# GlassyWing/yolo_deepsort

Hardware: AMD Instinct MI355X
Metric: end-to-end frames/sec (detect+ReID+assoc), 608x608 (higher is better)
Workload: dtype f16x3

## Files before the change

include/ydsort.h:

```cpp
#ifndef YDSORT_H
#define YDSORT_H

#include <stddef.h>
#include <stdint.h>

#ifdef __cplusplus
extern "C" {
#endif

typedef struct yds_net yds_net;
typedef struct yds_reid yds_reid;
typedef struct yds_trk yds_trk;
typedef struct yds_pipe yds_pipe;
typedef struct yds_zones yds_zones;
typedef struct yds_act yds_act;
typedef struct yds_ident yds_ident;
typedef struct yds_comm yds_comm;

int yds_init(int device_id);
int yds_current_device(void);
int yds_device_pci_bus_id(char *buf, int len);
const char *yds_last_error(void);
int yds_device_count(void);
const char *yds_build_info(void);
void *yds_host_alloc(size_t nbytes);
int yds_host_free(void *host);
void *yds_dev_alloc(size_t nbytes);
int yds_dev_free(void *dev);
int yds_memcpy_h2d(void *dst_dev, const void *src_host, size_t nbytes);
int yds_memcpy_d2h(void *dst_host, const void *src_dev, size_t nbytes);
int yds_memcpy_d2d(void *dst_dev, const void *src_dev, size_t nbytes);
int yds_device_sync(void);

yds_net *yds_darknet_create(const char *cfg_text, int img_h, int img_w, int batch_max);
void yds_darknet_destroy(yds_net *);
int yds_darknet_load_weights(yds_net *, const void *blob_host, size_t nbytes, int cutoff);
int yds_darknet_set_batch_max(yds_net *, int batch_max);
int yds_darknet_batch_max(const yds_net *);
int yds_darknet_set_half(yds_net *, int on);
int yds_darknet_layer_format(const yds_net *, int layer);
int yds_darknet_num_boxes(const yds_net *);
int yds_darknet_num_attrs(const yds_net *);
int yds_darknet_num_layers(const yds_net *);
int yds_darknet_layer_shape(const yds_net *, int layer, int *c, int *h, int *w);
int64_t yds_darknet_conv_flops(const yds_net *);
int yds_darknet_forward_f32(yds_net *, const float *nchw_host, int batch, float *out_host);
int yds_darknet_forward_u8(yds_net *, const uint8_t *rgb_hwc_host, int h, int w, int batch,
                           float *out_host_or_null);
int yds_darknet_forward_u8_dev(yds_net *, const uint8_t *rgb_hwc_dev, int h, int w, int batch);
int yds_darknet_forward_u8_mixed_dev(yds_net *, const uint8_t *rgb_hwc_dev, const uint64_t *frame_off, const int32_t *frame_hw ,
                                     size_t frames_bytes, int batch);
const uint8_t *yds_darknet_last_frames_dev(yds_net *, int *h, int *w, int *batch);
int yds_darknet_layer_output(yds_net *, int layer, int batch, float *nchw_host);
int yds_darknet_get_input(yds_net *, int batch, float *nchw_host);

int yds_nms(yds_net *, int image, float conf_thres, float iou_thres, int frame_h, int frame_w,
            float *out6_host, int cap, int *n_out);
int yds_nms_pred(const float *pred_host, int n_boxes, int attrs, float conf_thres, float iou_thres,
                 float *out6_host, int cap, int *n_out);

int yds_detect_tiled(yds_net *, const uint8_t *rgb_hwc_host, int h, int w, const int32_t *tiles_xyhw, int n_tiles,
                     float conf_thres, float iou_thres, float *out6_host, int cap, int *n_out);
int yds_nms_merge_pred(const float *pred_host, int n_boxes, int attrs, float conf_thres, float iou_thres,
                       float *out6_host, int cap, int *n_out);
int yds_nms_merge_pred_batched(const float *pred_host, int n_frames, int n_boxes, int attrs, float conf_thres, float iou_thres,
                               float *out6_host, int cap, int *n_out);
int yds_nms_ragged_pred(const float *pred_host, size_t total_rows, int attrs, int n_frames, const uint64_t *row0, const int32_t *n_rows,
                        const int32_t *corner_merge, const float *scale, float conf_thres, float iou_thres, float *out6_host, int cap,
                        int *n_out);

yds_reid *yds_reid_create(int max_crops);
void yds_reid_destroy(yds_reid *);
int yds_reid_load_tensor(yds_reid *, const char *name, const float *data_host, const int64_t *shape, int ndim);
int yds_reid_finalize(yds_reid *);
int64_t yds_reid_flops_per_crop(void);
int yds_reid_embed(yds_reid *, const uint8_t *frame_rgb_host, int h, int w, const float *tlwh_host,
                   int D, float *out_host);
int yds_reid_embed_dev(yds_reid *, const uint8_t *frame_rgb_dev, int h, int w, const float *tlwh_host,
                       int D, float *out_host_or_null);
const float *yds_reid_features_dev(yds_reid *);
int yds_reid_preprocess(yds_reid *, const uint8_t *frame_rgb_host, int h, int w, const float *tlwh_host,
                        int D, float *nchw_host);
int yds_reid_preprocess_mixed(yds_reid *, const uint8_t *frames_rgb_dev, const uint64_t *frame_off, const int32_t *frame_hw ,
                              int n_frames, size_t frames_bytes, const float *tlwh_host, const int32_t *frame_of_host, int D, float *nchw_host);
int yds_reid_embed_mixed(yds_reid *, const uint8_t *frames_dev, const uint64_t *frame_off, const int32_t *frame_hw ,
                         int n_frames, size_t frames_bytes, const float *tlwh_host, const int32_t *frame_of_host, int D, int bgr,
                         float *out_host);
int yds_reid_front_fused(yds_reid *);
int yds_reid_front_grid_crops(void);
int yds_reid_forward_f32(yds_reid *, const float *nchw_host, int D, float *out_host);

yds_trk *yds_tracker_create(double max_dist, double max_iou_distance, int max_age, int n_init, int nn_budget);
yds_trk *yds_tracker_create_ex(double max_dist, double max_iou_distance, int max_age, int n_init, int nn_budget, int metric);
void yds_tracker_destroy(yds_trk *);
int yds_tracker_step(yds_trk *, const float *tlwh_host, const float *feats_host, const float *payload_host,
                     int D, int32_t *out6_host, int cap, int *m_out,
                     int32_t *dbg_matches_host, int dbg_cap, int *n_matches);
int yds_tracker_step_dev(yds_trk *, const float *tlwh_host, const float *feats_dev, const float *payload_host,
                         int D, int32_t *out6_host, int cap, int *m_out);
int yds_tracker_step_sel(yds_trk *, const float *tlwh_host, const float *feats, int feats_on_device, const int32_t *feat_rows_host,
                         const float *payload_host, int D, int32_t *out6_host, int cap, int *m_out,
                         int32_t *dbg_matches_host, int dbg_cap, int *n_matches);
int yds_tracker_nms(const float *tlwh_host, const int32_t *order_host, int D, double max_overlap, int32_t *pick_host, int *n_pick);
int yds_tracker_num_tracks(const yds_trk *);
int yds_tracker_get_state(yds_trk *, int32_t *ids, int32_t *state, int32_t *tsu, int32_t *hits,
                          float *mean8, float *cov64, int cap, int *T);
int yds_tracker_gallery_rows(const yds_trk *);
int yds_tracker_get_payload(yds_trk *, float *payload, int cap);
int yds_tracker_get_age(yds_trk *, int32_t *age, int cap);
int yds_tracker_last_unmatched(yds_trk *, int32_t *um_tracks, int cap_t, int *n_t,
                               int32_t *um_dets, int cap_d, int *n_d);
int yds_lsap(const float *cost_host, int nr, int nc, int32_t *rows, int32_t *cols, int *n_out);
int yds_lsap_bench(const float *cost_host, int nr, int nc, int iters, double *avg_us);
int yds_kalman_predict(float *mean_host, float *cov_host, int T);
int yds_kalman_update(float *mean_host, float *cov_host, const float *xyah_host, int M);
int yds_kalman_gating(const float *mean_host, const float *cov_host, int T, const float *xyah_host, int D,
                      float *out_TxD_host);
int yds_kalman_gating_ex(const float *mean_host, const float *cov_host, int T, const float *xyah_host, int D, int only_position,
                         float *out_TxD_host);
int yds_kalman_initiate(const float *xyah_host, int n, float *mean_host, float *cov_host);
int yds_kalman_project(const float *mean_host, const float *cov_host, int n, float *mean4_host, float *cov16_host);
int yds_iou_cost(const float *track_tlwh_host, int T, const float *det_tlwh_host, int D, float *out_TxD_host);
int yds_cosine_min_cost(const float *gallery_host, const int32_t *seg_offsets_host, int T,
                        const float *feats_host, int D, int dim, float *out_TxD_host);
int yds_euclidean_min_cost(const float *gallery_host, const int32_t *seg_offsets_host, int T,
                           const float *feats_host, int D, int dim, float *out_TxD_host);

int yds_gallery_search(yds_trk *const *trks, int n_streams, const float *queries, int queries_on_device, int Q, int state_mask, float max_dist,
                       int top_k, int32_t *n_hits, int32_t *hit_stream, int32_t *hit_id, float *hit_dist);
int yds_gallery_search_dense(yds_trk *const *trks, int n_streams, const float *queries, int queries_on_device, int Q, float *dist_out,
                             int32_t *stream_of, int32_t *track_id, int32_t *state, int cap, int *n_tracks);
int yds_gallery_link(yds_trk *const *trks, int n_streams, int stream, int track_id, int exclude_stream , int state_mask,
                     float max_dist, int top_k, int32_t *n_hits, int32_t *hit_stream, int32_t *hit_id, float *hit_dist);
int yds_tracker_get_gallery(yds_trk *, int track_index, float *rows_out, int cap, int *n_rows);
int yds_tracker_get_slots(yds_trk *, int32_t *slots, int cap);

yds_pipe *yds_pipeline_create(yds_net *, yds_reid *, yds_trk *, float conf_thres, float nms_thres,
                              const int32_t *class_mask, int n_mask);
void yds_pipeline_destroy(yds_pipe *);
int yds_pipeline_step(yds_pipe *, const uint8_t *frames_dev, const uint8_t *next_frames_dev, int h, int w,
                      int batch, int32_t *out6_host, int cap, int32_t *counts_host);
int yds_pipeline_step_host(yds_pipe *, const uint8_t *frames_host, const uint8_t *next_frames_host, int h, int w,
                           int batch, int32_t *out6_host, int cap, int32_t *counts_host);
yds_pipe *yds_pipeline_create_multi(yds_net *, yds_reid *, yds_trk *const *trks, int n_streams, float conf_thres, float nms_thres,
                                    const int32_t *class_mask, int n_mask);
int yds_pipeline_step_multi(yds_pipe *, const uint8_t *frames_dev, const uint8_t *next_frames_dev, int h, int w, int n_frames,
                            const int32_t *stream_of_frame, int32_t *out6_host, int cap, int32_t *counts_host);
int yds_pipeline_step_multi_host(yds_pipe *, const uint8_t *frames_host, const uint8_t *next_frames_host, int h, int w, int n_frames,
                                 const int32_t *stream_of_frame, int32_t *out6_host, int cap, int32_t *counts_host);
int yds_pipeline_step_multi_mixed(yds_pipe *, const uint8_t *frames_dev, const uint8_t *next_frames_dev, const uint64_t *frame_off,
                                  const int32_t *frame_hw , size_t frames_bytes, int n_frames,
                                  const int32_t *stream_of_frame, int32_t *out6_host, int cap, int32_t *counts_host);
int yds_pipeline_step_multi_mixed_host(yds_pipe *, const uint8_t *frames_host, const uint8_t *next_frames_host, const uint64_t *frame_off,
                                       const int32_t *frame_hw , size_t frames_bytes, int n_frames,
                                       const int32_t *stream_of_frame, int32_t *out6_host, int cap, int32_t *counts_host);
int yds_pipeline_prefetch_host(yds_pipe *, const uint8_t *frames_host, int h, int w, int batch);
int yds_pipeline_set_schedule(yds_pipe *, int min_crops);
int yds_pipeline_set_frame_order(yds_pipe *, int bgr);
int yds_pipeline_set_windows(yds_pipe *, int win_w, int win_h, double overlap);
int yds_pipeline_set_stream_windows(yds_pipe *, int stream, int win_w, int win_h, double overlap);
int yds_pipeline_last_schedule(yds_pipe *);
int yds_pipeline_schedule_trial(yds_pipe *, int uploaded, int *decided, double *serialized_s, double *two_stream_s);
int yds_pipeline_stage_us(yds_pipe *, float *us5);
int yds_overlay_tracks(const uint8_t *frames_dev, const int32_t *src_slot_host, int n_out, int h, int w, const int32_t *boxes_host,
                       const int32_t *box_ptr_host, const uint8_t *text_host, int n_text, const int32_t *fps_host,
                       const uint8_t *font_host, int n_glyphs, int thickness, int scale, uint8_t *out_dev, uint8_t *out_host);
int yds_swap_rb(uint8_t *frames_dev, size_t pixels);
int yds_overlay_tracks_bgr(uint8_t *frames_bgr_dev, int n_src, const int32_t *src_slot_host, int n_out, int h, int w, const int32_t *boxes_host,
                           const int32_t *box_ptr_host, const uint8_t *text_host, int n_text, const int32_t *fps_host,
                           const uint8_t *font_host, int n_glyphs, int thickness, int scale, uint8_t *out_host);
int yds_conv_timing(yds_net *, int mode, double *total_us, int64_t *launches, double *flops);
int yds_conv_timing_ex(yds_net *, int mode, double *total_us, int64_t *launches, double *flops, double *bytes, double *attainable_us);
int yds_conv_num_variants(void);
int yds_set_conv_math(int mode);
int yds_get_conv_math(void);
const char *yds_conv_variant_name(int variant);
int yds_conv_bench(int n, int h, int w, int cin, int cout, int ksize, int stride, int act, int with_residual,
                   int iters, double *avg_us, int *variant);
int yds_conv_clock(double *ghz, double *sampled_ms, int reset);
int yds_conv_run(int variant, int n, int h, int w, int cin, int cout, int ksize, int stride, int act, int res_mode,
                 const float *x_nhwc, const float *w_okkc, const float *bias, const float *res_nhwc, float *y_nchw);
int yds_conv_run_view(int variant, int n, int h, int w, int cin, int cout, int ksize, int stride, int act, int res_mode,
                      const int *view, const float *x_nhwc, const float *w_okkc, const float *bias, const float *res_nhwc,
                      float sentinel, float *y_nchw, float *y2_nchw);
int yds_conv_run_half(int variant, int n, int h, int w, int cin, int cout, int ksize, int stride, int act, int res_mode,
                      const int *view, int fmt_x, int fmt_y, const float *x_nhwc, const float *w_okkc, const float *bias,
                      const float *res_nhwc, float sentinel, float *y_nchw, float *y2_nchw);
int yds_conv_run_fused(int kind, int n, int h, int w, int act, int half, int fmt, const float *x_nhwc, const float *w_a,
                       const float *bias_a, const float *w_b, const float *bias_b, float *y_nchw);

enum { YDS_ACT_TAKEOFF = 0, YDS_ACT_LANDING = 1, YDS_ACT_GLIDE = 2, YDS_ACT_FAST_CROSSING = 3, YDS_ACT_BREAK_INTO = 4 };
#define YDS_ACT_MAX_SIZE 16
#define YDS_ACT_MAX_ACTIONS 32
yds_act *yds_actions_create(int n_streams, const int32_t *kind, const int32_t *class_id, const double *param, int n_actions, int max_age,
                            int max_size);
void yds_actions_destroy(yds_act *);
int yds_actions_reset(yds_act *, int stream);
int yds_actions_update(yds_act *, const int32_t *rows6_host, const int32_t *first, const int32_t *stream_of, const double *row_time,
                       int n_frames, int32_t *out4_host, int cap, int *n_out);
int yds_actions_get_orbits(yds_act *, int stream, int32_t *ids, int32_t *ages, int32_t *lens, int cap, int *n);
int yds_actions_set_timing(yds_act *, int on);
int yds_actions_last_us(yds_act *, float *us);
int yds_pipeline_set_actions(yds_pipe *, yds_act *);
int yds_pipeline_set_frame_times(yds_pipe *, const double *t_host, int n);
int yds_pipeline_last_actions(yds_pipe *, int32_t *out4_host, int cap, int *n_out);

enum { YDS_ZONE_ENTER = 0, YDS_ZONE_EXIT = 1, YDS_ZONE_LOST = 2, YDS_ZONE_CROSS_FWD = 3, YDS_ZONE_CROSS_BACK = 4 };
#define YDS_ZONE_MAX_ZONES 32
#define YDS_ZONE_MAX_LINES 32
#define YDS_ZONE_MAX_VERTICES 16
#define YDS_ZONE_COORD_LIMIT (1 << 20)
yds_zones *yds_zones_create(int n_streams, int max_age);
void yds_zones_destroy(yds_zones *);
int yds_zones_set_stream(yds_zones *, int stream, const int32_t *zone_ptr, const int32_t *zone_xy, const int32_t *zone_class,
                         const int32_t *zone_min_sightings, int n_zones, const int32_t *line_xy, const int32_t *line_class, int n_lines);
int yds_zones_reset(yds_zones *, int stream);
int yds_zones_update(yds_zones *, const int32_t *rows6_host, const int32_t *first, const int32_t *stream_of, const double *frame_time,
                     int n_frames, int32_t *ev6_host, double *evt2_host, int cap, int *n_out);
int yds_zones_get_counts(yds_zones *, int stream, int32_t *zone4, int32_t *line2);
int yds_zones_get_tracks(yds_zones *, int stream, int32_t *ids, int32_t *ages, int32_t *inside_mask, int cap, int *n);
int yds_zones_set_timing(yds_zones *, int on);
int yds_zones_last_us(yds_zones *, float *us);
int yds_pipeline_set_zones(yds_pipe *, yds_zones *);
int yds_pipeline_last_zone_events(yds_pipe *, int32_t *ev6_host, double *evt2_host, int cap, int *n_out);

yds_ident *yds_identity_create(yds_trk *const *trks, int n_streams, float max_dist, int max_rows);
void yds_identity_destroy(yds_ident *);
int yds_identity_reset(yds_ident *);
int yds_identity_update(yds_ident *, int *n_linked, int *n_fresh, int *n_deferred);
int yds_identity_get(yds_ident *, int stream, int32_t *track_id, int32_t *global_id, int cap, int *n);
int yds_identity_last_links(yds_ident *, int32_t *stream, int32_t *track_id, int32_t *global_id, float *cost, int cap, int *n);
int yds_identity_last_counts(yds_ident *, int *n_linked, int *n_fresh, int *n_deferred);
int yds_identity_set_timing(yds_ident *, int on);
int yds_identity_last_us(yds_ident *, float *us);
int yds_identity_set_memory(yds_ident *, int max_ids, int rows_per_id, int ttl);
int yds_identity_enrol(yds_ident *, const float *rows, const int32_t *n_rows, int n_arrays, int32_t *global_id_out);
int yds_identity_get_memory(yds_ident *, int32_t *global_id, int32_t *n_rows, int32_t *last_held, int cap, int *n);
int yds_identity_get_memory_rows(yds_ident *, int global_id, float *rows_out, int cap, int *n_rows);
int yds_identity_memory_distances(yds_ident *, const float *queries, int queries_on_device, int Q, float *dist_out, int32_t *global_id_out,
                                  int cap, int *n_entries);
int yds_identity_memory_bench(yds_ident *, const float *queries_dev, int Q, int strip_len, int iters, float *us_out);
int yds_identity_last_relinked(yds_ident *, int32_t *stream, int32_t *track_id, int32_t *global_id, float *cost, int cap, int *n);
int yds_identity_last_memory_counts(yds_ident *, int32_t *counts7);
int yds_pipeline_set_identities(yds_pipe *, yds_ident *);
int yds_pipeline_last_identities(yds_pipe *, int stream, int32_t *track_id, int32_t *global_id, int cap, int *n);

#define YDS_COMM_ID_BYTES 128
#define YDS_COMM_MIN_ROWS 64
int yds_comm_preflight(void);
int yds_comm_unique_id(void *id128_out);
yds_comm *yds_comm_create(const void *id128, int world, int rank);
void yds_comm_destroy(yds_comm *);
int yds_comm_world(const yds_comm *);
int yds_comm_rank(const yds_comm *);
int yds_comm_rccl_version(void);
int yds_comm_allgather(yds_comm *, const void *send_host, size_t bytes, void *recv_host);
int yds_comm_allgather_dev(yds_comm *, const void *send_dev, size_t bytes, void *recv_dev);
int yds_comm_allgather_rows(yds_comm *, const int32_t *out6_host, int cap, const int32_t *counts_host, int batch, int rows_per_block,
                            int32_t *all_host, int *rows_needed);
int yds_comm_allreduce_f64(yds_comm *, double *vals_host, int n, int op);
int yds_comm_barrier(yds_comm *);

int yds_darknet_set_injection(yds_net *, int image, const float *rows_host, int n, float logit);
int yds_darknet_load_injection_sets(yds_net *, const float *rows_host, const int32_t *offsets_host, int n_sets, float logit);
int yds_darknet_select_injection_set(yds_net *, int set);
int yds_pipeline_set_next_injection(yds_pipe *, int set);
int yds_pipeline_slot_pred(yds_pipe *, float *pred_host, size_t cap_rows, size_t *n_rows);
int yds_gallery_search_bench(yds_trk *const *trks, int n_streams, const float *queries_dev, int Q, int state_mask, float max_dist, int top_k,
                             int iters, float *us_out);

#ifdef __cplusplus
}
#endif
#endif
```

yolo_deepsort_amd/_lib.py:

```python

from __future__ import annotations

import ctypes as C
import os

import numpy as np

HERE = os.path.dirname(os.path.abspath(__file__))
_TAG = os.environ.get("YDS_BUILD_TAG", "")
LIB_PATH = os.path.join(HERE, "libydsort" + ("_" + _TAG if _TAG else "") + ".so")


class YdsError(RuntimeError):
    pass


_P = C.c_void_p
_I = C.c_int
_F = C.c_float
_SZ = C.c_size_t
_I64 = C.c_int64

SIGNATURES = {
    "yds_init": (_I, [_I]),
    "yds_last_error": (C.c_char_p, []),
    "yds_device_count": (_I, []),
    "yds_current_device": (_I, []),
    "yds_device_pci_bus_id": (_I, [C.c_char_p, _I]),
    "yds_build_info": (C.c_char_p, []),
    "yds_host_alloc": (_P, [_SZ]),
    "yds_host_free": (_I, [_P]),
    "yds_dev_alloc": (_P, [_SZ]),
    "yds_dev_free": (_I, [_P]),
    "yds_memcpy_h2d": (_I, [_P, _P, _SZ]),
    "yds_memcpy_d2h": (_I, [_P, _P, _SZ]),
    "yds_memcpy_d2d": (_I, [_P, _P, _SZ]),
    "yds_device_sync": (_I, []),
    "yds_darknet_create": (_P, [C.c_char_p, _I, _I, _I]),
    "yds_darknet_destroy": (None, [_P]),
    "yds_darknet_load_weights": (_I, [_P, _P, _SZ, _I]),
    "yds_darknet_set_batch_max": (_I, [_P, _I]),
    "yds_darknet_batch_max": (_I, [_P]),
    "yds_darknet_set_half": (_I, [_P, _I]),
    "yds_darknet_layer_format": (_I, [_P, _I]),
    "yds_darknet_num_boxes": (_I, [_P]),
    "yds_darknet_num_attrs": (_I, [_P]),
    "yds_darknet_num_layers": (_I, [_P]),
    "yds_darknet_layer_shape": (_I, [_P, _I, _P, _P, _P]),
    "yds_darknet_conv_flops": (_I64, [_P]),
    "yds_darknet_forward_f32": (_I, [_P, _P, _I, _P]),
    "yds_darknet_forward_u8": (_I, [_P, _P, _I, _I, _I, _P]),
    "yds_darknet_forward_u8_dev": (_I, [_P, _P, _I, _I, _I]),
    "yds_darknet_last_frames_dev": (_P, [_P, _P, _P, _P]),
    "yds_darknet_layer_output": (_I, [_P, _I, _I, _P]),
    "yds_darknet_get_input": (_I, [_P, _I, _P]),
    "yds_darknet_set_injection": (_I, [_P, _I, _P, _I, _F]),
    "yds_darknet_load_injection_sets": (_I, [_P, _P, _P, _I, _F]),
    "yds_darknet_select_injection_set": (_I, [_P, _I]),
    "yds_conv_variant_name": (C.c_char_p, [_I]),
    "yds_conv_timing_ex": (_I, [_P, _I, _P, _P, _P, _P, _P]),
    "yds_conv_num_variants": (_I, []),
    "yds_conv_clock": (_I, [_P, _P, _I]),
    "yds_set_conv_math": (_I, [_I]),
    "yds_get_conv_math": (_I, []),
    "yds_conv_bench": (_I, [_I, _I, _I, _I, _I, _I, _I, _I, _I, _I, _P, _P]),
    "yds_conv_run": (_I, [_I, _I, _I, _I, _I, _I, _I, _I, _I, _I, _P, _P, _P, _P, _P]),
    "yds_conv_run_view": (_I, [_I, _I, _I, _I, _I, _I, _I, _I, _I, _I, _P, _P, _P, _P, _P, _F, _P, _P]),
    "yds_conv_run_half": (_I, [_I, _I, _I, _I, _I, _I, _I, _I, _I, _I, _P, _I, _I, _P, _P, _P, _P, _F, _P, _P]),
    "yds_conv_run_fused": (_I, [_I, _I, _I, _I, _I, _I, _I, _P, _P, _P, _P, _P, _P]),
    "yds_nms": (_I, [_P, _I, _F, _F, _I, _I, _P, _I, _P]),
    "yds_nms_pred": (_I, [_P, _I, _I, _F, _F, _P, _I, _P]),
    "yds_nms_merge_pred": (_I, [_P, _I, _I, _F, _F, _P, _I, _P]),
    "yds_nms_merge_pred_batched": (_I, [_P, _I, _I, _I, _F, _F, _P, _I, _P]),
    "yds_detect_tiled": (_I, [_P, _P, _I, _I, _P, _I, _F, _F, _P, _I, _P]),
    "yds_reid_create": (_P, [_I]),
    "yds_reid_destroy": (None, [_P]),
    "yds_reid_load_tensor": (_I, [_P, C.c_char_p, _P, _P, _I]),
    "yds_reid_finalize": (_I, [_P]),
    "yds_reid_flops_per_crop": (_I64, []),
    "yds_reid_embed": (_I, [_P, _P, _I, _I, _P, _I, _P]),
    "yds_reid_embed_dev": (_I, [_P, _P, _I, _I, _P, _I, _P]),
    "yds_reid_features_dev": (_P, [_P]),
    "yds_reid_preprocess": (_I, [_P, _P, _I, _I, _P, _I, _P]),
    "yds_reid_forward_f32": (_I, [_P, _P, _I, _P]),
    "yds_tracker_create": (_P, [C.c_double, C.c_double, _I, _I, _I]),
    "yds_tracker_create_ex": (_P, [C.c_double, C.c_double, _I, _I, _I, _I]),
    "yds_tracker_step_sel": (_I, [_P, _P, _P, _I, _P, _P, _I, _P, _I, _P, _P, _I, _P]),
    "yds_tracker_nms": (_I, [_P, _P, _I, C.c_double, _P, _P]),
    "yds_euclidean_min_cost": (_I, [_P, _P, _I, _P, _I, _I, _P]),
    "yds_tracker_destroy": (None, [_P]),
    "yds_tracker_step": (_I, [_P, _P, _P, _P, _I, _P, _I, _P, _P, _I, _P]),
    "yds_tracker_step_dev": (_I, [_P, _P, _P, _P, _I, _P, _I, _P]),
    "yds_tracker_num_tracks": (_I, [_P]),
    "yds_tracker_get_state": (_I, [_P, _P, _P, _P, _P, _P, _P, _I, _P]),
    "yds_comm_unique_id": (_I, [_P]),
    "yds_comm_create": (_P, [_P, _I, _I]),
    "yds_comm_destroy": (None, [_P]),
    "yds_comm_world": (_I, [_P]),
    "yds_comm_rank": (_I, [_P]),
    "yds_comm_rccl_version": (_I, []),
    "yds_comm_allgather": (_I, [_P, _P, _SZ, _P]),
    "yds_comm_allgather_dev": (_I, [_P, _P, _SZ, _P]),
    "yds_comm_allgather_rows": (_I, [_P, _P, _I, _P, _I, _I, _P, _P]),
    "yds_comm_preflight": (_I, []),
    "yds_comm_allreduce_f64": (_I, [_P, _P, _I, _I]),
    "yds_comm_barrier": (_I, [_P]),
    "yds_tracker_get_payload": (_I, [_P, _P, _I]),
    "yds_tracker_get_age": (_I, [_P, _P, _I]),
    "yds_tracker_gallery_rows": (_I, [_P]),
    "yds_kalman_gating_ex": (_I, [_P, _P, _I, _P, _I, _I, _P]),
    "yds_kalman_initiate": (_I, [_P, _I, _P, _P]),
    "yds_kalman_project": (_I, [_P, _P, _I, _P, _P]),
    "yds_tracker_last_unmatched": (_I, [_P, _P, _I, _P, _P, _I, _P]),
    "yds_lsap": (_I, [_P, _I, _I, _P, _P, _P]),
    "yds_lsap_bench": (_I, [_P, _I, _I, _I, _P]),
    "yds_kalman_predict": (_I, [_P, _P, _I]),
    "yds_kalman_update": (_I, [_P, _P, _P, _I]),
    "yds_kalman_gating": (_I, [_P, _P, _I, _P, _I, _P]),
    "yds_iou_cost": (_I, [_P, _I, _P, _I, _P]),
    "yds_cosine_min_cost": (_I, [_P, _P, _I, _P, _I, _I, _P]),
    "yds_pipeline_create": (_P, [_P, _P, _P, _F, _F, _P, _I]),
    "yds_pipeline_destroy": (None, [_P]),
    "yds_pipeline_step": (_I, [_P, _P, _P, _I, _I, _I, _P, _I, _P]),
    "yds_pipeline_step_host": (_I, [_P, _P, _P, _I, _I, _I, _P, _I, _P]),
    "yds_pipeline_create_multi": (_P, [_P, _P, _P, _I, _F, _F, _P, _I]),
    "yds_pipeline_step_multi": (_I, [_P, _P, _P, _I, _I, _I, _P, _P, _I, _P]),
    "yds_pipeline_step_multi_host": (_I, [_P, _P, _P, _I, _I, _I, _P, _P, _I, _P]),
    "yds_pipeline_prefetch_host": (_I, [_P, _P, _I, _I, _I]),
    "yds_pipeline_set_next_injection": (_I, [_P, _I]),
    "yds_pipeline_stage_us": (_I, [_P, _P]),
    "yds_pipeline_set_schedule": (_I, [_P, _I]),
    "yds_pipeline_last_schedule": (_I, [_P]),
    "yds_pipeline_schedule_trial": (_I, [_P, _I, _P, _P, _P]),
    "yds_conv_timing": (_I, [_P, _I, _P, _P, _P]),
    "yds_overlay_tracks": (_I, [_P, _P, _I, _I, _I, _P, _P, _P, _I, _P, _P, _I, _I, _I, _P, _P]),
    "yds_swap_rb": (_I, [_P, _SZ]),
    "yds_overlay_tracks_bgr": (_I, [_P, _I, _P, _I, _I, _I, _P, _P, _P, _I, _P, _P, _I, _I, _I, _P]),
    "yds_pipeline_set_frame_order": (_I, [_P, _I]),
    "yds_pipeline_set_windows": (_I, [_P, _I, _I, C.c_double]),
    "yds_darknet_forward_u8_mixed_dev": (_I, [_P, _P, _P, _P, _SZ, _I]),
    "yds_reid_preprocess_mixed": (_I, [_P, _P, _P, _P, _I, _SZ, _P, _P, _I, _P]),
    "yds_reid_embed_mixed": (_I, [_P, _P, _P, _P, _I, _SZ, _P, _P, _I, _I, _P]),
    "yds_reid_front_fused": (_I, [_P]),
    "yds_reid_front_grid_crops": (_I, []),
    "yds_pipeline_step_multi_mixed": (_I, [_P, _P, _P, _P, _P, _SZ, _I, _P, _P, _I, _P]),
    "yds_pipeline_step_multi_mixed_host": (_I, [_P, _P, _P, _P, _P, _SZ, _I, _P, _P, _I, _P]),
    "yds_nms_ragged_pred": (_I, [_P, _SZ, _I, _I, _P, _P, _P, _P, _F, _F, _P, _I, _P]),
    "yds_pipeline_set_stream_windows": (_I, [_P, _I, _I, _I, C.c_double]),
    "yds_pipeline_slot_pred": (_I, [_P, _P, _SZ, _P]),
    "yds_gallery_search": (_I, [_P, _I, _P, _I, _I, _I, _F, _I, _P, _P, _P, _P]),
    "yds_gallery_search_dense": (_I, [_P, _I, _P, _I, _I, _P, _P, _P, _P, _I, _P]),
    "yds_gallery_link": (_I, [_P, _I, _I, _I, _I, _I, _F, _I, _P, _P, _P, _P]),
    "yds_tracker_get_gallery": (_I, [_P, _I, _P, _I, _P]),
    "yds_tracker_get_slots": (_I, [_P, _P, _I]),
    "yds_actions_create": (_P, [_I, _P, _P, _P, _I, _I, _I]),
    "yds_actions_destroy": (None, [_P]),
    "yds_actions_reset": (_I, [_P, _I]),
    "yds_actions_update": (_I, [_P, _P, _P, _P, _P, _I, _P, _I, _P]),
    "yds_actions_get_orbits": (_I, [_P, _I, _P, _P, _P, _I, _P]),
    "yds_actions_set_timing": (_I, [_P, _I]),
    "yds_actions_last_us": (_I, [_P, _P]),
    "yds_pipeline_set_actions": (_I, [_P, _P]),
    "yds_pipeline_set_frame_times": (_I, [_P, _P, _I]),
    "yds_pipeline_last_actions": (_I, [_P, _P, _I, _P]),
    "yds_gallery_search_bench": (_I, [_P, _I, _P, _I, _I, _F, _I, _I, _P]),
    "yds_identity_create": (_P, [_P, _I, _F, _I]),
    "yds_identity_destroy": (None, [_P]),
    "yds_identity_reset": (_I, [_P]),
    "yds_identity_update": (_I, [_P, _P, _P, _P]),
    "yds_identity_get": (_I, [_P, _I, _P, _P, _I, _P]),
    "yds_identity_last_links": (_I, [_P, _P, _P, _P, _P, _I, _P]),
    "yds_identity_last_counts": (_I, [_P, _P, _P, _P]),
    "yds_identity_set_timing": (_I, [_P, _I]),
    "yds_identity_last_us": (_I, [_P, _P]),
    "yds_identity_set_memory": (_I, [_P, _I, _I, _I]),
    "yds_identity_enrol": (_I, [_P, _P, _P, _I, _P]),
    "yds_identity_get_memory": (_I, [_P, _P, _P, _P, _I, _P]),
    "yds_identity_get_memory_rows": (_I, [_P, _I, _P, _I, _P]),
    "yds_identity_memory_distances": (_I, [_P, _P, _I, _I, _P, _P, _I, _P]),
    "yds_identity_memory_bench": (_I, [_P, _P, _I, _I, _I, _P]),
    "yds_identity_last_relinked": (_I, [_P, _P, _P, _P, _P, _I, _P]),
    "yds_identity_last_memory_counts": (_I, [_P, _P]),
    "yds_pipeline_set_identities": (_I, [_P, _P]),
    "yds_pipeline_last_identities": (_I, [_P, _I, _P, _P, _I, _P]),
    "yds_zones_create": (_P, [_I, _I]),
    "yds_zones_destroy": (None, [_P]),
    "yds_zones_set_stream": (_I, [_P, _I, _P, _P, _P, _P, _I, _P, _P, _I]),
    "yds_zones_reset": (_I, [_P, _I]),
    "yds_zones_update": (_I, [_P, _P, _P, _P, _P, _I, _P, _P, _I, _P]),
    "yds_zones_get_counts": (_I, [_P, _I, _P, _P]),
    "yds_zones_get_tracks": (_I, [_P, _I, _P, _P, _P, _I, _P]),
    "yds_zones_set_timing": (_I, [_P, _I]),
    "yds_zones_last_us": (_I, [_P, _P]),
    "yds_pipeline_set_zones": (_I, [_P, _P]),
    "yds_pipeline_last_zone_events": (_I, [_P, _P, _P, _I, _P]),
}

_lib = None
MISSING = []


def load():
    global _lib
    if _lib is not None:
        return _lib
    if not os.path.exists(LIB_PATH):
        raise YdsError(f"{LIB_PATH} not found: build it with `python -m yolo_deepsort_amd.build` "
                       "(the product has no CPU fallback)")
    lib = C.CDLL(LIB_PATH)
    for name, (res, args) in SIGNATURES.items():
        try:
            fn = getattr(lib, name)
        except AttributeError:
            MISSING.append(name)
            continue
        fn.restype = res
        fn.argtypes = args
    _lib = lib
    return lib


def last_error():
    return load().yds_last_error().decode("utf-8", "replace")


def check(rc):
    if rc != 0:
        raise YdsError(last_error())


def check_ptr(p):
    if not p:
        raise YdsError(last_error())
    return p


_bound = None


VISIBILITY_MASKS = ("HIP_VISIBLE_DEVICES", "ROCR_VISIBLE_DEVICES", "CUDA_VISIBLE_DEVICES", "GPU_DEVICE_ORDINAL")


def default_device(n_visible=None):
    v = os.environ.get("YDS_DEVICE")
    if v not in (None, ""):
        return int(v)
    v = os.environ.get("LOCAL_RANK")
    if v in (None, ""):
        return 0
    masked = any(os.environ.get(k) not in (None, "") for k in VISIBILITY_MASKS)
    if masked:
        n = load().yds_device_count() if n_visible is None else n_visible
        if n == 1:
            return 0
    return int(v)


def init(device=None):
    global _bound
    if _bound is not None:
        if device is not None and int(device) != _bound:
            raise YdsError(f"this process is bound to device {_bound}; one process drives one GPU (requested {int(device)})")
        return _bound
    dev = default_device() if device is None else int(device)
    check(load().yds_init(dev))
    _bound = dev
    return dev


def current_device():
    return _bound


def pci_bus_id():
    buf = C.create_string_buffer(64)
    check(load().yds_device_pci_bus_id(buf, 64))
    return buf.value.decode()


def ptr(a):
    if a is None:
        return None
    assert a.flags["C_CONTIGUOUS"], "array must be C-contiguous"
    return a.ctypes.data_as(C.c_void_p)


def as_f32(a):
    return np.ascontiguousarray(a, dtype=np.float32)


class PinnedArray:

    def __init__(self, shape, dtype=np.uint8):
        self.shape, self.dtype = tuple(int(v) for v in shape), np.dtype(dtype)
        self.nbytes = int(np.prod(self.shape)) * self.dtype.itemsize
        self.ptr = check_ptr(load().yds_host_alloc(self.nbytes))
        buf = (C.c_uint8 * self.nbytes).from_address(self.ptr)
        self.array = np.frombuffer(buf, dtype=self.dtype).reshape(self.shape)

    @classmethod
    def from_array(cls, a):
        a = np.asarray(a)
        p = cls(a.shape, a.dtype)
        np.copyto(p.array, a)
        return p

    def free(self):
        if self.ptr:
            self.array = None
            load().yds_host_free(self.ptr)
            self.ptr = None

    def __del__(self):
        try:
            self.free()
        except Exception:
            pass


class DeviceBuffer:

    def __init__(self, nbytes):
        self.nbytes = int(nbytes)
        self.ptr = check_ptr(load().yds_dev_alloc(self.nbytes))

    @classmethod
    def from_array(cls, a):
        a = np.ascontiguousarray(a)
        buf = cls(a.nbytes)
        check(load().yds_memcpy_h2d(buf.ptr, ptr(a), a.nbytes))
        return buf

    def offset(self, nbytes):
        return C.c_void_p(self.ptr + int(nbytes))

    def free(self):
        if self.ptr:
            load().yds_dev_free(self.ptr)
            self.ptr = None

    def __del__(self):
        try:
            self.free()
        except Exception:
            pass
```

yolo_deepsort_amd/csrc/common.h:

```cpp
#pragma once
#include <hip/hip_runtime.h>
#include <stdint.h>
#include <stdio.h>
#include <string>
#include <vector>
#include <stdexcept>

#include "slot_plan.h"

namespace yds {

void set_error(const std::string &msg);
struct Error : std::runtime_error {
    explicit Error(const std::string &m) : std::runtime_error(m) {}
};
[[noreturn]] void fail(const char *fmt, ...);
int bound_device();
void bind_thread();
hipStream_t make_stream(bool latency_role);

#define YDS_HIP(expr)                                                                          \
    do {                                                                                       \
        hipError_t _e = (expr);                                                                \
        if (_e != hipSuccess)                                                                  \
            ::yds::fail("%s failed: %s (%s:%d)", #expr, hipGetErrorString(_e), __FILE__, __LINE__); \
    } while (0)

#define YDS_API_BEGIN try { ::yds::bind_thread();
#define YDS_API_END                                                                            \
    }                                                                                          \
    catch (const std::exception &e) {                                                          \
        ::yds::set_error(e.what());                                                            \
        return -1;                                                                             \
    }                                                                                          \
    return 0;
#define YDS_API_END_PTR                                                                        \
    }                                                                                          \
    catch (const std::exception &e) {                                                          \
        ::yds::set_error(e.what());                                                            \
        return nullptr;                                                                        \
    }

template <typename T> struct DevBuf {
    T *p = nullptr;
    size_t n = 0;
    DevBuf() = default;
    explicit DevBuf(size_t count) { alloc(count); }
    DevBuf(const DevBuf &) = delete;
    DevBuf &operator=(const DevBuf &) = delete;
    DevBuf(DevBuf &&o) noexcept : p(o.p), n(o.n) { o.p = nullptr; o.n = 0; }
    DevBuf &operator=(DevBuf &&o) noexcept {
        if (this != &o) { release(); p = o.p; n = o.n; o.p = nullptr; o.n = 0; }
        return *this;
    }
    ~DevBuf() { release(); }
    void alloc(size_t count) {
        release();
        if (count == 0) return;
        YDS_HIP(hipMalloc((void **)&p, count * sizeof(T)));
        n = count;
    }
    void ensure(size_t count) { if (count > n) alloc(count); }
    void release() { if (p) { (void)hipFree(p); p = nullptr; n = 0; } }
    void upload(const T *src, size_t count, hipStream_t s = nullptr) {
        ensure(count);
        if (count) YDS_HIP(hipMemcpyAsync(p, src, count * sizeof(T), hipMemcpyHostToDevice, s));
    }
};

struct View {
    float *p = nullptr;
    int n = 0, h = 0, w = 0, c = 0, ld = 0;
    int fmt = 0;
    size_t pixels() const { return (size_t)n * h * w; }
};

enum Act { ACT_LINEAR = 0, ACT_LEAKY = 1, ACT_MISH = 2, ACT_RELU = 3 };
enum ResMode { RES_NONE = 0, RES_AFTER_ACT = 1, RES_BEFORE_ACT = 2 };

struct ConvArgs {
    View x, y;
    const float *w = nullptr, *bias = nullptr;
    const void *w16 = nullptr;
    View res;
    int ksize = 1, stride = 1, pad = 0, kpad = 0;
    int act = ACT_LINEAR, res_mode = RES_NONE;
    int terms = 3;
    View y2;
    int n_split = 0;
    int tile_gn = 0;
};
enum ConvVariant {
    VAR_F32_128x128_K32, VAR_F32_128x64_K32, VAR_F32_64x64_K32, VAR_F32_128x32_K32, VAR_F32_128x128_K16, VAR_F32_128x64_K16, VAR_F32_64x128_K16,
    VAR_STAGED_128x128, VAR_STAGED_64x128, VAR_STAGED_128x64, VAR_STAGED_64x64,
    VAR_DMA_128x128_NS2, VAR_DMA_256x128_NS3, VAR_DMA_128x256_NS3, VAR_DMA_128x128_NS3, VAR_WIN_256x128, VAR_WIN_256x64, VAR_WIN_128x64,
    VAR_DMA_128x64_NS2, VAR_DMA_64x128_NS2, VAR_WIN2_128x128, VAR_SPLITK_64x128, VAR_SPLITK_128x128, VAR_DIRECT_RGB, kConvVariants
};
static_assert(VAR_STAGED_128x128 == 7 && VAR_WIN_256x128 == 15 && VAR_SPLITK_64x128 == 21 && kConvVariants == 24, "variant ids are fixed");
int launch_conv(const ConvArgs &a, hipStream_t s, int variant = -1);
constexpr int kVariantMask = 0xff, kTileGnShift = 8;
bool conv_presplit_input(const ConvArgs &a);
bool launch_conv_maxpool3s2(const ConvArgs &a, hipStream_t s);
int conv_autotune(const ConvArgs &a, hipStream_t s, float *best_us);
std::vector<int> conv_candidates(const ConvArgs &a);
enum ConvMath { MATH_F32 = 0, MATH_F16X3 = 1 };
int conv_math();
void set_conv_math(int m);
void pack_weights_f16x3(const float *w, int cout, int kpad, std::vector<uint16_t> &out);
const char *conv_variant_name(int v);
double conv_flops(const ConvArgs &a);
double conv_bytes_io(const View &v);
double conv_bytes(const ConvArgs &a);

void launch_maxpool(const View &x, const View &y, int k, int stride, int pad, bool zero_pad_br, hipStream_t s);
void launch_upsample(const View &x, const View &y, int stride, hipStream_t s);
void launch_copy(const View &x, const View &y, hipStream_t s);
void launch_add(const View &a, const View &b, const View &y, hipStream_t s);
void launch_nchw_to_nhwc(const float *src_nchw, const View &y, int c_src, hipStream_t s);
void launch_nhwc_to_nchw(const View &x, float *dst_nchw, hipStream_t s);
void nhwc_to_host(const View &x, float *dst_nchw_host, hipStream_t s);
void launch_pack_h16(const float *src_f32, const View &y, hipStream_t s);
void launch_yolo_decode(const View &head, float *out, int total_boxes, int box_off, int num_classes,
                        const float *anchors_wh , int A, int img_h, int img_w, hipStream_t s);
void launch_inject(const View &head, int image, const float *rows_dev, int n, int head_index, int num_classes,
                   float logit, hipStream_t s);
void launch_inject_batch(const View &head, int batch, const float *table_dev, const int *offsets_dev, int max_rows, int head_index,
                         int num_classes, float logit, hipStream_t s);
void launch_resize_u8(const uint8_t *frames, int n, int h, int w, const View &y, hipStream_t s, bool bgr = false);
std::vector<FrameGeom> checked_layout(const uint64_t *frame_off, const int32_t *frame_hw, int n, size_t frames_bytes);
void launch_slot_resize(const uint8_t *frames, const SlotRec *slots, int n, const View &y, hipStream_t s, bool bgr);
void launch_slot_boxes(const float *pred, int n_boxes, int attrs, const SlotRec *slots, int n, float *dst, hipStream_t s);
struct ReidFront {
    const uint8_t *frames = nullptr;
    const FrameGeom *geom = nullptr;
    const int *boxes = nullptr;
    int h = 0, w = 0, bgr = 0;
};
void launch_crop_resize(const ReidFront &f, int D, const View &y, hipStream_t s);
void launch_reid_stem(const ReidFront &f, int D, const float *w, int kpad, const float *bias, const View &pooled, hipStream_t s);
constexpr int kReidStemUnitsPerCrop = 4;
int reid_stem_grid();
void launch_avgpool_l2norm(const View &x, float *out, hipStream_t s);

}
```

yolo_deepsort_amd/csrc/conv_common.h:

```cpp
#pragma once
#include "common.h"
#include "h16.h"

#include <algorithm>
#include <stdlib.h>
#include <type_traits>

namespace yds {

typedef float f32x16 __attribute__((ext_vector_type(16)));
typedef float f32x4 __attribute__((ext_vector_type(4)));

typedef _Float16 h8 __attribute__((ext_vector_type(8)));
typedef _Float16 h4 __attribute__((ext_vector_type(4)));
constexpr float A_SCALE = 1.f / 256.f, LO_SCALE = 2048.f;
typedef __attribute__((address_space(3))) void lds_void_t;
typedef __attribute__((address_space(1))) const void glb_void_t;
template <int N> __device__ __forceinline__ void wait_vmcnt() { asm volatile("s_waitcnt vmcnt(%0)" ::"n"(N) : "memory"); }

struct ConvKernelArgs {
    const float *x, *w, *bias, *res;
    float *y;
    int H, W, Cin, ldx;
    int Ho, Wo, Cout, ldy, ldr;
    int ksize, stride, pad;
    int K, Kpad, M;
    int act, res_mode;
    int fmt_x, fmt_y, fmt_r;
    int terms;
    int ksplit = 1;
    float *y2 = nullptr;
    int ldy2 = 0, n_split = 0;
    int tiles_m, tiles_n, xm, rm, rn;
    int gn = 1;
    int gn_req = 0;
};

constexpr int KALIGN = 32;
constexpr int STAGGER = 24;

template <int ACT> __device__ __forceinline__ float apply_act(float v) {
    if (ACT == ACT_LEAKY) return v > 0.f ? v : v * 0.1f;
    if (ACT == ACT_RELU) return v > 0.f ? v : 0.f;
    if (ACT == ACT_MISH) {
        const float e = __builtin_amdgcn_exp2f(fminf(v, 20.f) * 1.44269504088896341f);
        const float n = e * (e + 2.f);
        const float m = v * (n * __builtin_amdgcn_rcpf(n + 2.f));
        return v > 20.f ? v : m;
    }
    return v;
}

__device__ __forceinline__ bool tile_of_block(const ConvKernelArgs &p, int &tm, int &tn) {
    const int b = blockIdx.x, xcd = b & 7, idx = b >> 3;
    int lm, ln;
    if (p.gn <= 1) {
        lm = idx % p.rm;
        ln = idx / p.rm;
    } else {
        const int per = p.rm * p.gn, grp = idx / per, w = idx - grp * per;
        const int g = min(p.gn, p.rn - grp * p.gn);
        lm = w / g;
        ln = grp * p.gn + (w - lm * g);
    }
    tm = (xcd % p.xm) * p.rm + lm;
    tn = (xcd / p.xm) * p.rn + ln;
    return tm < p.tiles_m && tn < p.tiles_n;
}

inline int plan_tile_map(ConvKernelArgs &k, int BM, int BN) {
    k.tiles_m = (k.M + BM - 1) / BM;
    k.tiles_n = (k.Cout + BN - 1) / BN;
    long best = -1;
    for (int xm = 1; xm <= 8; xm *= 2) {
        int xn = 8 / xm;
        int rm = (k.tiles_m + xm - 1) / xm, rn = (k.tiles_n + xn - 1) / xn;
        long waste = (long)rm * rn * 8 - (long)k.tiles_m * k.tiles_n;
        long cost = ((long)rm * BM + (long)rn * BN) * 64 + waste * (BM + BN);
        if (best < 0 || cost < best) { best = cost; k.xm = xm; k.rm = rm; k.rn = rn; }
    }
    k.gn = std::max(1, std::min(k.gn_req, k.rn));
    return 8 * k.rm * k.rn;
}

struct FlatRows {
    int m0;
    __device__ __forceinline__ int operator()(int row) const { return m0 + row; }
};
template <int BM, int BN, int WM, int WN, int ACT, int RES, int NT, class RowMap, bool ONE_PASS, class Store>
__device__ __forceinline__ void conv_epilogue_core(const ConvKernelArgs &p, Store store, float *stage, RowMap rows, int n0, int tid) {
    constexpr int ROWS = BM / WM, LD = BN + 4, C4 = BN / 4;
    constexpr int RSTEP = NT / C4;
    static_assert(NT % C4 == 0 && C4 % 2 == 0 && ROWS % RSTEP == 0, "tile width must divide the workgroup; lane pairs share a row");
    const int wave = tid >> 6, wm = wave / WN;
    const int c4 = tid % C4, rr = tid / C4;
    const int n = n0 + c4 * 4;
    const bool n_vec = n + 3 < p.Cout;
    const bool second = p.n_split > 0 && n >= p.n_split;
    float *const y_base = second ? p.y2 : p.y;
    const int y_ld = second ? p.ldy2 : p.ldy, ny = second ? n - p.n_split : n;
    float4 bias4 = make_float4(0.f, 0.f, 0.f, 0.f);
    if (n_vec) bias4 = *reinterpret_cast<const float4 *>(p.bias + n);
    else {
        if (n < p.Cout) bias4.x = p.bias[n];
        if (n + 1 < p.Cout) bias4.y = p.bias[n + 1];
        if (n + 2 < p.Cout) bias4.z = p.bias[n + 2];
    }
    constexpr int PER_PASS = ROWS / RSTEP, NRES = RES != RES_NONE ? WM * PER_PASS : 1;
    auto sweep = [&](auto yf_c, auto rf_c) {
        constexpr int YF = decltype(yf_c)::value, RF = decltype(rf_c)::value;
        constexpr bool YH = YF == FMT_H16, RH = RF == FMT_H16, YS = YF == FMT_F16, RS = RF == FMT_F16;
        float4 rraw[NRES];
        if (RES != RES_NONE) {
#pragma unroll
            for (int q = 0; q < NRES; ++q) {
                const int m = rows((q / PER_PASS) * ROWS + rr + (q % PER_PASS) * RSTEP);
                rraw[q] = make_float4(0.f, 0.f, 0.f, 0.f);
                if (m >= 0 && m < p.M && n < p.Cout) {
                    const float *rp = p.res + (size_t)m * p.ldr;
                    if (RH) {
                        const char *g = reinterpret_cast<const char *>(rp + (n & ~31)) + (n & 31) * 2;
                        const float2 hi = *reinterpret_cast<const float2 *>(g), lo = *reinterpret_cast<const float2 *>(g + 64);
                        rraw[q] = make_float4(hi.x, hi.y, lo.x, lo.y);
                    } else if (RS) {
                        const float2 h = *reinterpret_cast<const float2 *>(reinterpret_cast<const char *>(rp) + n * 2);
                        rraw[q] = make_float4(h.x, h.y, 0.f, 0.f);
                    } else if (n_vec) {
                        rraw[q] = *reinterpret_cast<const float4 *>(rp + n);
                    } else {
                        rraw[q].x = rp[n];
                        if (n + 1 < p.Cout) rraw[q].y = rp[n + 1];
                        if (n + 2 < p.Cout) rraw[q].z = rp[n + 2];
                    }
                }
            }
        }
#pragma unroll
        for (int pass = 0; pass < WM; ++pass) {
            if (ONE_PASS ? pass == 0 : wm == pass) store(stage + (ONE_PASS ? wm * ROWS * LD : 0));
            if (!ONE_PASS || pass == 0) __syncthreads();
#pragma unroll
            for (int k2 = 0; k2 < PER_PASS; ++k2) {
                const int r = rr + k2 * RSTEP;
                const int m = rows(pass * ROWS + r);
                const bool live = m >= 0 && m < p.M && n < p.Cout;
                float4 v = *reinterpret_cast<const float4 *>(stage + (ONE_PASS ? pass * ROWS * LD : 0) + r * LD + c4 * 4);
                float rs[4] = {0.f, 0.f, 0.f, 0.f};
                if (RES != RES_NONE) {
                    const float4 t = rraw[RES != RES_NONE ? pass * PER_PASS + k2 : 0];
                    if (RH) {
                        union { float2 f; h16x4 h; } uh, ul;
                        uh.f = make_float2(t.x, t.y);
                        ul.f = make_float2(t.z, t.w);
                        h16_decode4(uh.h, ul.h, rs);
                    } else if (RS) {
                        union { float2 f; h16x4 h; } uh;
                        uh.f = make_float2(t.x, t.y);
#pragma unroll
                        for (int k = 0; k < 4; ++k) rs[k] = (float)uh.h[k] * (1.f / H16_A_SCALE);
                    } else { rs[0] = t.x; rs[1] = t.y; rs[2] = t.z; rs[3] = t.w; }
                }
                float o[4] = {v.x + bias4.x, v.y + bias4.y, v.z + bias4.z, v.w + bias4.w};
#pragma unroll
                for (int k = 0; k < 4; ++k) {
                    if (RES == RES_BEFORE_ACT) o[k] += rs[k];
                    o[k] = apply_act<ACT>(o[k]);
                    if (RES == RES_AFTER_ACT) o[k] += rs[k];
                }
                float *yp = y_base + (size_t)m * y_ld;
                if (YH) {
                    h16x4 hi, lo;
                    h16_encode4(o, hi, lo);
                    const bool odd = c4 & 1;
                    union { h16x4 h; int i[2]; } send, recv;
                    send.h = odd ? hi : lo;
                    recv.i[0] = __builtin_amdgcn_update_dpp(send.i[0], send.i[0], 0xB1, 0xF, 0xF, false);
                    recv.i[1] = __builtin_amdgcn_update_dpp(send.i[1], send.i[1], 0xB1, 0xF, 0xF, false);
                    union { h16x4 h[2]; float4 f; } out;
                    out.h[0] = odd ? recv.h : hi;
                    out.h[1] = odd ? lo : recv.h;
                    const int nq = ny & ~7;
                    char *g = reinterpret_cast<char *>(yp + (nq & ~31)) + (nq & 31) * 2 + (odd ? 64 : 0);
                    if (live) *reinterpret_cast<float4 *>(g) = out.f;
                } else if (YS) {
                    union { h16x4 h; int i[2]; } mine, other;
#pragma unroll
                    for (int k = 0; k < 4; ++k) mine.h[k] = (_Float16)(o[k] * H16_A_SCALE);
                    other.i[0] = __builtin_amdgcn_update_dpp(mine.i[0], mine.i[0], 0xB1, 0xF, 0xF, false);
                    other.i[1] = __builtin_amdgcn_update_dpp(mine.i[1], mine.i[1], 0xB1, 0xF, 0xF, false);
                    union { h16x4 h[2]; float4 f; } out;
                    out.h[0] = mine.h;
                    out.h[1] = other.h;
                    if (live && !(c4 & 1)) *reinterpret_cast<float4 *>(reinterpret_cast<char *>(yp) + ny * 2) = out.f;
                } else if (live) {
                    if (n_vec) *reinterpret_cast<float4 *>(yp + ny) = make_float4(o[0], o[1], o[2], o[3]);
                    else { yp[ny] = o[0]; if (n + 1 < p.Cout) yp[ny + 1] = o[1]; if (n + 2 < p.Cout) yp[ny + 2] = o[2]; }
                }
            }
            if (!ONE_PASS && pass + 1 < WM) __syncthreads();
        }
    };
    using F32c = std::integral_constant<int, FMT_F32>;
    using H16c = std::integral_constant<int, FMT_H16>;
    using F16c = std::integral_constant<int, FMT_F16>;
    const bool yh = p.fmt_y == FMT_H16, rh = RES != RES_NONE && p.fmt_r == FMT_H16;
    if (p.fmt_y == FMT_F16) {
        sweep(F16c{}, F16c{});
    } else if (yh) {
        if (rh) sweep(H16c{}, H16c{});
        else sweep(H16c{}, F32c{});
    } else {
        if (rh) sweep(F32c{}, H16c{});
        else sweep(F32c{}, F32c{});
    }
}
constexpr size_t conv_stage_bytes(int BM, int BN) { return (size_t)BM * (BN + 4) * sizeof(float); }

template <int BM, int BN, int WM, int WN, int ACT, int RES, int TM, int TN, int NT = 256, class RowMap = FlatRows, bool ONE_PASS = false>
__device__ __forceinline__ void conv_epilogue_rows(const ConvKernelArgs &p, f32x16 (&acc)[TM][TN], float *stage, RowMap rows, int n0, int tid) {
    constexpr int LD = BN + 4;
    const int lane = tid & 63, wn = (tid >> 6) % WN;
    const int col = lane & 31, rsel = (lane >> 5) * 4;
    auto store = [&](float *st) {
#pragma unroll
        for (int i = 0; i < TM; ++i)
#pragma unroll
            for (int j = 0; j < TN; ++j)
#pragma unroll
                for (int e = 0; e < 16; ++e)
                    st[(i * 32 + rsel + (e & 3) + 8 * (e >> 2)) * LD + wn * (BN / WN) + j * 32 + col] = acc[i][j][e];
    };
    conv_epilogue_core<BM, BN, WM, WN, ACT, RES, NT, RowMap, ONE_PASS>(p, store, stage, rows, n0, tid);
}

template <int BM, int BN, int WM, int WN, int ACT, int RES, int TM, int TN, int NT = 256, class RowMap = FlatRows, bool ONE_PASS = false>
__device__ __forceinline__ void conv_epilogue16_rows(const ConvKernelArgs &p, f32x4 (&acc)[TM][TN], float *stage, RowMap rows, int n0, int tid) {
    constexpr int LD = BN + 4;
    const int lane = tid & 63, wn = (tid >> 6) % WN;
    const int col = lane & 15, rsel = (lane >> 4) * 4;
    auto store = [&](float *st) {
#pragma unroll
        for (int i = 0; i < TM; ++i)
#pragma unroll
            for (int j = 0; j < TN; ++j)
#pragma unroll
                for (int e = 0; e < 4; ++e)
                    st[(i * 16 + rsel + e) * LD + wn * (BN / WN) + j * 16 + col] = acc[i][j][e];
    };
    conv_epilogue_core<BM, BN, WM, WN, ACT, RES, NT, RowMap, ONE_PASS>(p, store, stage, rows, n0, tid);
}
template <int BM, int BN, int WM, int WN, int ACT, int RES, int TM, int TN, int NT = 256, bool ONE_PASS = false>
__device__ __forceinline__ void conv_epilogue16(const ConvKernelArgs &p, f32x4 (&acc)[TM][TN], float *stage, int m0, int n0, int tid) {
    conv_epilogue16_rows<BM, BN, WM, WN, ACT, RES, TM, TN, NT, FlatRows, ONE_PASS>(p, acc, stage, FlatRows{m0}, n0, tid);
}

template <int BM, int BN, int WM, int WN, int ACT, int RES, int TM, int TN, int NT = 256, bool ONE_PASS = false>
__device__ __forceinline__ void conv_epilogue(const ConvKernelArgs &p, f32x16 (&acc)[TM][TN], float *stage, int m0, int n0, int tid) {
    conv_epilogue_rows<BM, BN, WM, WN, ACT, RES, TM, TN, NT, FlatRows, ONE_PASS>(p, acc, stage, FlatRows{m0}, n0, tid);
}

ConvKernelArgs make_conv_args(const ConvArgs &a);
bool conv_stem2_applicable(const ConvKernelArgs &k0, const ConvKernelArgs &k1);
void launch_conv_stem2(const ConvKernelArgs &k0, const ConvKernelArgs &k1, hipStream_t s);
bool conv_block1_applicable(const ConvKernelArgs &k2, const ConvKernelArgs &k3);
void launch_conv_block1(const ConvKernelArgs &k2, const ConvKernelArgs &k3, hipStream_t s);

template <class F> void dispatch_act_res(const ConvKernelArgs &k, F f) {
    using Linear = std::integral_constant<int, ACT_LINEAR>;
    using Leaky = std::integral_constant<int, ACT_LEAKY>;
    using Mish = std::integral_constant<int, ACT_MISH>;
    using Relu = std::integral_constant<int, ACT_RELU>;
    using None = std::integral_constant<int, RES_NONE>;
    using After = std::integral_constant<int, RES_AFTER_ACT>;
    using Before = std::integral_constant<int, RES_BEFORE_ACT>;
    switch (k.act * 4 + k.res_mode) {
        case ACT_LINEAR * 4 + RES_NONE: f(Linear{}, None{}); break;
        case ACT_LEAKY * 4 + RES_NONE: f(Leaky{}, None{}); break;
        case ACT_LEAKY * 4 + RES_AFTER_ACT: f(Leaky{}, After{}); break;
        case ACT_MISH * 4 + RES_NONE: f(Mish{}, None{}); break;
        case ACT_MISH * 4 + RES_AFTER_ACT: f(Mish{}, After{}); break;
        case ACT_RELU * 4 + RES_NONE: f(Relu{}, None{}); break;
        case ACT_RELU * 4 + RES_BEFORE_ACT: f(Relu{}, Before{}); break;
        default: fail("conv: unsupported activation/residual combination (%d, %d)", k.act, k.res_mode);
    }
}

template <auto KERN, class... Args>
void launch_conv_tiles(ConvKernelArgs k, int BM, int BN, int grid_y, int threads, size_t smem, hipStream_t s, Args... args) {
    static size_t attr_set = 0;
    if (smem > attr_set) {
        YDS_HIP(hipFuncSetAttribute(reinterpret_cast<const void *>(KERN), hipFuncAttributeMaxDynamicSharedMemorySize, (int)smem));
        attr_set = smem;
    }
    dim3 grid(plan_tile_map(k, BM, BN), grid_y);
    hipLaunchKernelGGL(KERN, grid, dim3(threads), smem, s, k, args...);
    YDS_HIP(hipGetLastError());
}

bool conv_direct_applicable(const ConvKernelArgs &k);
void launch_conv_direct(const ConvKernelArgs &k, hipStream_t s);
bool conv_pool_applicable(const ConvKernelArgs &k);
void launch_conv_pool(const ConvKernelArgs &k, hipStream_t s);

void launch_conv_f16x3_staged(ConvKernelArgs k, int tile, hipStream_t s);
void launch_conv_f16x3_dma(ConvKernelArgs k, int tile, hipStream_t s);
void launch_conv_f16x3_win(ConvKernelArgs k, int tile, hipStream_t s);
void launch_conv_f16x3_splitk(ConvKernelArgs k, int tile, hipStream_t s);
bool conv_splitk_applicable(const ConvKernelArgs &k, int tile);
bool conv_splitk_preferred(const ConvKernelArgs &k);
bool conv_win2_applicable(const ConvKernelArgs &k);
void launch_conv_win2(ConvKernelArgs k, hipStream_t s);
bool conv_win_applicable(const ConvKernelArgs &k);
void launch_conv_win(ConvKernelArgs k, int shape, hipStream_t s);
void conv_win_clock(unsigned long long *cycles_ticks, bool reset);
void conv_win16_clock(unsigned long long *cycles_ticks, bool reset);
bool conv_win16_small_applicable(const ConvKernelArgs &k);
void launch_conv_win16(ConvKernelArgs k, int shape, hipStream_t s);
void conv_win2_clock(unsigned long long *cycles_ticks, bool reset);

}
```

yolo_deepsort_amd/csrc/conv_stem2.hip:

```cpp
#include "conv_common.h"

#include <algorithm>


namespace yds {

namespace {

typedef float f32x2 __attribute__((ext_vector_type(2)));

constexpr int TH = 8, TW = 16;
constexpr int BM = TH * TW, BN = 64, WM = 4, WN = 2, NW = 8, NT = NW * 64;
constexpr int PR = 2 * TH + 1, PC = 2 * TW + 1;
constexpr int EVEN_COLS = TW + 1, ODD_COLS = TW;
constexpr int ODD_BASE = PR * EVEN_COLS;
constexpr int PATCH_ROWS = PR * PC;
constexpr int RR = PR + 2, RC = PC + 2;
constexpr int W_BYTES = 9 * BN * 128, PATCH_BYTES = PATCH_ROWS * 128, RGB_BYTES = RR * RC * 16;
constexpr int SMEM = W_BYTES + PATCH_BYTES + RGB_BYTES;

struct StemRows {
    int img, oy0, ox0, Ho, Wo;
    __device__ __forceinline__ int operator()(int row) const {
        const int oy = oy0 + row / TW, ox = ox0 + row % TW;
        return oy < Ho && ox < Wo ? (img * Ho + oy) * Wo + ox : -1;
    }
};

__device__ __forceinline__ int patch_row(int ry, int rc) {
    return (rc & 1) ? ODD_BASE + ry * ODD_COLS + (rc >> 1) : ry * EVEN_COLS + (rc >> 1);
}

template <int ACT0, int ACT1, bool HALF>
__global__ __launch_bounds__(NT, 1) void conv_stem2_f16x3(ConvKernelArgs p0, ConvKernelArgs p1, int tiles_y, int tiles_x, int n_tiles) {
    fp16_saturate_on();
    extern __shared__ __attribute__((aligned(16))) char smem[];
    char *wreg = smem, *patch = smem + W_BYTES;
    float4 *rgb = reinterpret_cast<float4 *>(smem + W_BYTES + PATCH_BYTES);
    const int tid = threadIdx.x, lane = tid & 63, wave = tid >> 6, wm = wave / WN, wn = wave % WN;

    for (int i = tid; i < 9 * BN * 8; i += NT) {
        const int row = i >> 3, pos = i & 7, tap = row / BN, co = row - tap * BN;
        const int c = pos ^ ((row >> 1) & 7);
        const f32x4 v = *reinterpret_cast<const f32x4 *>(reinterpret_cast<const char *>(p1.w) + ((size_t)min(co, p1.Cout - 1) * 9 + tap) * 128 + c * 16);
        *reinterpret_cast<f32x4 *>(wreg + row * 128 + pos * 16) = v;
    }
    const int kb0 = lane >> 5;
    h8 w0h[3], w0l[3];
#pragma unroll
    for (int sb = 0; sb < 3; ++sb)
#pragma unroll
        for (int e = 0; e < 8; ++e) {
            const int t = 4 * sb + 2 * kb0 + (e >> 2), c = e & 3;
            const float x = (t < 9 && c < 3) ? p0.w[(size_t)(lane & 31) * p0.Kpad + t * 4 + c] : (t == 4 && c == 3 ? p0.bias[lane & 31] : 0.f);
            const _Float16 h = (_Float16)x;
            w0h[sb][e] = h;
            w0l[sb][e] = (_Float16)((x - (float)h) * LO_SCALE);
        }
    const int kb = lane >> 5, r = wm * 32 + (lane & 31), py = r / TW, px = r - py * TW;
    const int brow = wn * 32 + (lane & 31);

    constexpr int LOADS = (RR * RC + NT - 1) / NT;
    float4 nxt[LOADS];
    auto fetch = [&](int tl) {
        const int img = tl / (tiles_y * tiles_x), rem = tl - img * (tiles_y * tiles_x);
        const int iy0 = 2 * ((rem / tiles_x) * TH) - 2, ix0 = 2 * ((rem % tiles_x) * TW) - 2;
#pragma unroll
        for (int l = 0; l < LOADS; ++l) {
            const int i = tid + l * NT, rr = i / RC, cc = i - rr * RC;
            const int iy = iy0 + rr, ix = ix0 + cc;
            nxt[l] = make_float4(0.f, 0.f, 0.f, 0.f);
            if (i < RR * RC && tl < n_tiles && (unsigned)iy < (unsigned)p0.H && (unsigned)ix < (unsigned)p0.W) {
                nxt[l] = *reinterpret_cast<const float4 *>(p0.x + ((size_t)(img * p0.H + iy) * p0.W + ix) * p0.ldx);
                nxt[l].w = 1.f;
            }
        }
    };
    fetch(blockIdx.x);
    for (int tl = blockIdx.x; tl < n_tiles; tl += gridDim.x) {
        const int img = tl / (tiles_y * tiles_x), rem = tl - img * (tiles_y * tiles_x);
        const int oy0 = (rem / tiles_x) * TH, ox0 = (rem % tiles_x) * TW;
        const int ly0 = 2 * oy0 - 1, lx0 = 2 * ox0 - 1;
        __syncthreads();
#pragma unroll
        for (int l = 0; l < LOADS; ++l) {
            const int i = tid + l * NT;
            if (i < RR * RC) {
                const float v[4] = {nxt[l].x, nxt[l].y, nxt[l].z, nxt[l].w};
                union { h16x4 h[2]; float4 f; } sp;
                h16_encode4(v, sp.h[0], sp.h[1]);
                rgb[i] = sp.f;
            }
        }
        __syncthreads();
        fetch(tl + gridDim.x);
#pragma unroll 1
        for (int fr = wave; fr < (PATCH_ROWS + 31) / 32; fr += NW) {
            const int pix = fr * 32 + (lane & 31), pc = min(pix, PATCH_ROWS - 1);
            const int ry = pc / PC, rc = pc - ry * PC;
            f32x16 c1, c2;
#pragma unroll
            for (int e = 0; e < 16; ++e) { c1[e] = 0.f; c2[e] = 0.f; }
#pragma unroll
            for (int sb = 0; sb < 3; ++sb) {
                union { h16x4 q[2]; h8 v; } xh, xl;
#pragma unroll
                for (int u = 0; u < 2; ++u) {
                    const int t = 4 * sb + 2 * kb0 + u;
                    union { float4 f; h16x4 h[2]; } px4;
                    px4.f = make_float4(0.f, 0.f, 0.f, 0.f);
                    if (t < 9) px4.f = rgb[(ry + t / 3) * RC + rc + t % 3];
                    xh.q[u] = px4.h[0];
                    xl.q[u] = px4.h[1];
                }
                c1 = __builtin_amdgcn_mfma_f32_32x32x16_f16(w0h[sb], xh.v, c1, 0, 0, 0);
                if (!HALF) {
                    c2 = __builtin_amdgcn_mfma_f32_32x32x16_f16(w0h[sb], xl.v, c2, 0, 0, 0);
                    c2 = __builtin_amdgcn_mfma_f32_32x32x16_f16(w0l[sb], xh.v, c2, 0, 0, 0);
                }
            }
            const bool inside = (unsigned)(ly0 + ry) < (unsigned)p0.H && (unsigned)(lx0 + rc) < (unsigned)p0.W;
            const int j = patch_row(ry, rc), jsw = (j >> 1) & 7;
            if (pix < PATCH_ROWS) {
                if (inside) {
#pragma unroll
                    for (int g = 0; g < 4; ++g) {
                        float v[4];
#pragma unroll
                        for (int c = 0; c < 4; ++c) {
                            const int e = g * 4 + c;
                            const float os = HALF ? c1[e] : c1[e] + c2[e] * (1.f / LO_SCALE);
                            v[c] = ACT0 == ACT_LEAKY ? fmaxf(os, os * 0.1f) : apply_act<ACT0>(os * (1.f / A_SCALE)) * A_SCALE;
                        }
                        h16x4 hi, lo;
                        if (HALF) {
#pragma unroll
                            for (int c = 0; c < 4; ++c) hi[c] = (_Float16)v[c];
                        } else {
                            h16_encode4_scaled(v, hi, lo);
                        }
                        *reinterpret_cast<h16x4 *>(patch + j * 128 + ((g ^ jsw) << 4) + kb0 * 8) = hi;
                        if (!HALF) *reinterpret_cast<h16x4 *>(patch + j * 128 + (((4 + g) ^ jsw) << 4) + kb0 * 8) = lo;
                    }
                } else {
                    const h16x4 z = {(_Float16)0.f, (_Float16)0.f, (_Float16)0.f, (_Float16)0.f};
#pragma unroll
                    for (int g = 0; g < (HALF ? 4 : 8); ++g) *reinterpret_cast<h16x4 *>(patch + j * 128 + ((g ^ jsw) << 4) + kb0 * 8) = z;
                }
            }
        }
        __syncthreads();
        f32x16 acc1[1][1], acc2[1][1];
#pragma unroll
        for (int e = 0; e < 16; ++e) { acc1[0][0][e] = 0.f; acc2[0][0][e] = 0.f; }
#pragma unroll
        for (int t = 0; t < 9; ++t) {
            const int dy = t / 3, dx = t % 3;
            const int j = (dx & 1) ? ODD_BASE + (2 * py + dy) * ODD_COLS + px : (2 * py + dy) * EVEN_COLS + px + (dx >> 1);
            const int jsw = (j >> 1) & 7, wrow = t * BN + brow, wsw = (wrow >> 1) & 7;
            const char *ap = patch + j * 128, *bp = wreg + wrow * 128;
#pragma unroll
            for (int s = 0; s < 2; ++s) {
                const h8 ah = *reinterpret_cast<const h8 *>(ap + (((2 * s + kb) ^ jsw) << 4));
                const h8 bh = *reinterpret_cast<const h8 *>(bp + (((2 * s + kb) ^ wsw) << 4));
                acc1[0][0] = __builtin_amdgcn_mfma_f32_32x32x16_f16(ah, bh, acc1[0][0], 0, 0, 0);
                if (!HALF) {
                    const h8 al = *reinterpret_cast<const h8 *>(ap + (((4 + 2 * s + kb) ^ jsw) << 4));
                    const h8 bl = *reinterpret_cast<const h8 *>(bp + (((4 + 2 * s + kb) ^ wsw) << 4));
                    acc2[0][0] = __builtin_amdgcn_mfma_f32_32x32x16_f16(ah, bl, acc2[0][0], 0, 0, 0);
                    acc2[0][0] = __builtin_amdgcn_mfma_f32_32x32x16_f16(al, bh, acc2[0][0], 0, 0, 0);
                }
            }
        }
#pragma unroll
        for (int e = 0; e < 16; ++e) acc1[0][0][e] = (HALF ? acc1[0][0][e] : acc1[0][0][e] + acc2[0][0][e] * (1.f / LO_SCALE)) * (1.f / A_SCALE);
        __syncthreads();
        conv_epilogue_rows<BM, BN, WM, WN, ACT1, RES_NONE, 1, 1, NT, StemRows, true>(p1, acc1, reinterpret_cast<float *>(patch),
                                                                                       StemRows{img, oy0, ox0, p1.Ho, p1.Wo}, 0, tid);
    }
}

template <int ACT0, int ACT1, bool HALF> void launch_inst(const ConvKernelArgs &k0, const ConvKernelArgs &k1, hipStream_t s) {
    static_assert(BM * (BN + 4) * 4 <= PATCH_BYTES, "whole-tile epilogue staging must fit the layer-0 patch");
    const int n_img = k0.M / (k0.H * k0.W);
    const int tiles_y = (k1.Ho + TH - 1) / TH, tiles_x = (k1.Wo + TW - 1) / TW, n_tiles = n_img * tiles_y * tiles_x;
    static bool attr_set = false;
    auto kern = conv_stem2_f16x3<ACT0, ACT1, HALF>;
    if (!attr_set) {
        YDS_HIP(hipFuncSetAttribute(reinterpret_cast<const void *>(kern), hipFuncAttributeMaxDynamicSharedMemorySize, SMEM));
        attr_set = true;
    }
    hipLaunchKernelGGL(kern, dim3(std::min(n_tiles, 256)), dim3(NT), SMEM, s, k0, k1, tiles_y, tiles_x, n_tiles);
    YDS_HIP(hipGetLastError());
}

}

bool conv_stem2_applicable(const ConvKernelArgs &k0, const ConvKernelArgs &k1) {
    return k0.Cin == 4 && k0.ksize == 3 && k0.stride == 1 && k0.pad == 1 && k0.Cout == 32 && k0.res_mode == RES_NONE && k0.fmt_x == FMT_F32 &&
           k1.Cin == 32 && k1.ksize == 3 && k1.stride == 2 && k1.pad == 1 && k1.Cout == 64 && k1.res_mode == RES_NONE && k1.K == 288 &&
           k1.H == k0.Ho && k1.W == k0.Wo && k0.act == k1.act && (k0.act == ACT_LEAKY || k0.act == ACT_MISH);
}

void launch_conv_stem2(const ConvKernelArgs &k0, const ConvKernelArgs &k1, hipStream_t s) {
    if (!conv_stem2_applicable(k0, k1)) fail("conv: the fused stem takes a 3x3/s1 RGB->32 conv followed by a 3x3/s2 32->64 conv");
    const bool half = k1.terms == 1;
    if (k0.act == ACT_LEAKY) { if (half) launch_inst<ACT_LEAKY, ACT_LEAKY, true>(k0, k1, s); else launch_inst<ACT_LEAKY, ACT_LEAKY, false>(k0, k1, s); }
    else { if (half) launch_inst<ACT_MISH, ACT_MISH, true>(k0, k1, s); else launch_inst<ACT_MISH, ACT_MISH, false>(k0, k1, s); }
}

}
```

yolo_deepsort_amd/csrc/darknet.cpp:

```cpp
#include "engine.h"
#include "h16.h"
#include "conv_common.h"

#include <math.h>
#include <stdlib.h>
#include <string.h>
#include <map>
#include <sstream>

namespace yds {

std::vector<CfgBlock> parse_cfg(const std::string &text) {
    std::vector<CfgBlock> blocks;
    std::istringstream in(text);
    std::string line;
    auto strip = [](std::string s) {
        size_t a = s.find_first_not_of(" \t\r\n"), b = s.find_last_not_of(" \t\r\n");
        return a == std::string::npos ? std::string() : s.substr(a, b - a + 1);
    };
    while (std::getline(in, line)) {
        if (line.empty() || line[0] == '#') continue;
        line = strip(line);
        if (line.empty()) fail("cfg: whitespace-only line (the reference parser rejects it too)");
        if (line[0] == '[') {
// ... 178 lines not shown
                storage[r].into = i;
                storage[r].coff = off;
            } else {
                l.copies.push_back({j, off});
            }
            off += s.c;
        }
        if (l.groups) fail("cfg: grouped multi-source routes are not supported");
    }
    math = conv_math();
    std::vector<char> h16_ok(L, math == MATH_F16X3 ? 1 : 0);
    for (int j = 0; j < L; ++j) {
        if (layers[j].type == L_YOLO) continue;
        int off = 0, o = owner_of(j, off);
        if (off % 32 || layers[j].c % 32) h16_ok[o] = 0;
    }
    for (int pass = 0; pass < 2; ++pass)
        for (int i = 0; i < L; ++i)
            for (auto &cp : layers[i].copies) {
                int off = 0, o = owner_of(cp.first, off);
                if (o >= 0 && h16_ok[o] != h16_ok[i]) h16_ok[o] = h16_ok[i] = 0;
            }
    for (int i = 0; i < L; ++i) {
        Layer &l = layers[i];
        bool owns = (is_producer(i) && !storage[i].redirected) || l.concat();
        if (!owns) continue;
        if (storage[i].ld == 0) storage[i].ld = (l.c + 3) / 4 * 4;
        storage[i].fmt = (h16_ok[i] && storage[i].ld % 32 == 0) ? FMT_H16 : FMT_F32;
        storage[i].owns = true;
    }
    const bool no_merge = getenv("YDS_NO_CSP_MERGE") != nullptr;
    for (int i = 1; i + 2 < L && !no_merge; ++i) {
        Layer &a = layers[i];
        const Layer &r = layers[i + 1];
        Layer &b = layers[i + 2];
        if (a.type != L_CONV || b.type != L_CONV || r.type != L_ROUTE || r.refs.size() != 1 || r.groups) continue;
        if (a.src < 0 || r.refs[0] != a.src || b.src != i + 1) continue;
        if (a.cw.ksize != 1 || b.cw.ksize != 1 || a.cw.stride != 1 || b.cw.stride != 1 || a.act != b.act || a.fused_res >= 0 || b.fused_res >= 0) continue;
        if (a.merged_into >= 0 || a.merge_next >= 0 || a.cw.cin != b.cw.cin) continue;
        if ((int)i == block1_at || (int)i + 2 == block1_at || i + 2 == (int)block1_at + 1) continue;
        int oa = 0, ob = 0;
        const int sa = owner_of(i, oa), sb = owner_of(i + 2, ob);
        if (storage[sa].fmt != storage[sb].fmt || a.c % 4 || b.c % 4) continue;
        if (storage[sa].fmt == FMT_H16 && (a.c % 32 || b.c % 32)) continue;
        a.merge_next = i + 2;
        b.merged_into = i;
    }
    plan_half_formats();
    allocate_buffers();
}

int Darknet::owner_of(int j, int &off) const {
    const Layer &l = layers[j];
    if (l.concat()) { off = 0; return j; }
    int r = l.root;
    if (storage[r].redirected) { off = storage[r].coff + l.coff; return storage[r].into; }
    off = l.coff;
    return r;
}

void Darknet::plan_half_formats() {
    const int L = (int)layers.size();
    for (Storage &st : storage) st.fmt_half = st.fmt;
    const bool off = getenv("YDS_HALF_H16") != nullptr;
    if (!half_mode || off || math != MATH_F16X3) return;
    std::vector<char> ok(L, 0);
    for (int i = 0; i < L; ++i) ok[i] = storage[i].owns && storage[i].fmt == FMT_H16 && storage[i].ld % 64 == 0;
    auto own = [&](int j) { int off = 0; return owner_of(j, off); };
    for (int j = 0; j < L; ++j) {
        if (layers[j].type == L_YOLO) continue;
        int off = 0, o = owner_of(j, off);
        if (o >= 0 && (off % 64 || layers[j].c % 64)) ok[o] = 0;
    }
    if (block1_at >= 0) ok[own(block1_at)] = 0;
    for (int pass = 0; pass < L; ++pass) {
        bool changed = false;
        auto tie = [&](int a, int b) {
            if (a >= 0 && b >= 0 && ok[a] != ok[b]) { ok[a] = ok[b] = 0; changed = true; }
        };
        for (int i = 0; i < L; ++i) {
            const Layer &l = layers[i];
            for (auto &cp : l.copies) tie(own(cp.first), i);
            if (l.type == L_CONV && l.fused_res >= 0) tie(own(i), own(l.fused_res));
            if (l.type == L_CONV && l.merge_next >= 0) tie(own(i), own(l.merge_next));
            if (l.type == L_UPSAMPLE) tie(own(i), own(l.src));
            if (i == block1_at && l.src >= 0) tie(own(l.src), own(i + 1));
        }
        if (!changed) break;
    }
    for (int i = 0; i < L; ++i)
        if (ok[i]) storage[i].fmt_half = FMT_F16;
}

void Darknet::set_half(bool on) {
    if (on == half_mode) return;
    YDS_HIP(hipStreamSynchronize(stream));
    half_mode = on;
    plan_half_formats();
    ++plan_epoch;
}

void Darknet::allocate_buffers() {
    for (size_t i = 0; i < layers.size(); ++i) {
        if (!storage[i].owns) continue;
        const Layer &l = layers[i];
        size_t n = (size_t)batch_max * l.h * l.w * storage[i].ld;
        storage[i].buf.alloc(n);
        YDS_HIP(hipMemsetAsync(storage[i].buf.p, 0, n * sizeof(float), stream));
    }
    input.alloc((size_t)batch_max * img_h * img_w * 4);
    out.alloc((size_t)batch_max * total_boxes * attrs);
    stage_f32.alloc((size_t)batch_max * img_h * img_w * 4);
    YDS_HIP(hipStreamSynchronize(stream));
    inject_rows.clear();
    inject_rows.resize(batch_max);
    inject_n.assign(batch_max, 0);
    inject_active = false;
    inject_offsets.clear();
    inject_set = -1;
    ++plan_epoch;
    stage_n = 0;
}

void Darknet::set_batch_max(int b) {
    if (b < 1) fail("set_batch_max: %d", b);
    if (b == batch_max) return;
    YDS_HIP(hipStreamSynchronize(stream));
    batch_max = b;
    allocate_buffers();
}

Darknet::~Darknet() {
    for (const ConvTimeRec &r : conv_pending) { (void)hipEventDestroy(r.e0); (void)hipEventDestroy(r.e1); }
    for (hipEvent_t e : ev_pool) (void)hipEventDestroy(e);
    if (stream) (void)hipStreamDestroy(stream);
}

View Darknet::view(int i, int batch, int first) const {
    const Layer &l = layers[i];
    int r = l.root;
    View v;
    v.n = batch; v.h = l.h; v.w = l.w; v.c = l.c;
    if (l.concat()) {
        v.fmt = half_mode ? storage[i].fmt_half : storage[i].fmt;
        v.p = storage[i].buf.p; v.ld = fmt_slots(v.fmt, storage[i].ld);
        v.p += (size_t)first * l.h * l.w * v.ld;
        return v;
    }
    const Storage &st = storage[r];
    if (st.redirected) {
        const Storage &dst = storage[st.into];
        v.fmt = half_mode ? dst.fmt_half : dst.fmt;
        v.p = dst.buf.p + fmt_slots(v.fmt, st.coff + l.coff);
        v.ld = fmt_slots(v.fmt, dst.ld);
    } else {
        v.fmt = half_mode ? st.fmt_half : st.fmt;
        v.p = st.buf.p + fmt_slots(v.fmt, l.coff);
        v.ld = fmt_slots(v.fmt, st.ld);
    }
    v.p += (size_t)first * l.h * l.w * v.ld;
    return v;
}

View Darknet::input_view(int batch, int first) const {
    View v;
    v.p = input.p + (size_t)first * img_h * img_w * 4; v.n = batch; v.h = img_h; v.w = img_w; v.c = 4; v.ld = 4;
    return v;
}

void Darknet::load_weights(const void *blob, size_t nbytes, int cutoff) {
    if (nbytes < 20) fail("weights: blob shorter than the 20-byte header");
    const float *w = reinterpret_cast<const float *>(static_cast<const char *>(blob) + 20);
    size_t avail = (nbytes - 20) / 4, ptr = 0;
    ++plan_epoch;
    for (Layer &l : layers) l.cw_merged.release();
    for (int i = 0; i < (int)layers.size(); ++i) {
        Layer &l = layers[i];
        if (l.type != L_CONV) continue;
        if (cutoff >= 0 && i >= cutoff) { l.cw.release(); continue; }
        const int co = l.c;
        const size_t nw = (size_t)co * l.cw.cin_file * l.cw.ksize * l.cw.ksize, need = (size_t)(l.bn ? 4 : 1) * co + nw;
        if (ptr + need > avail) fail("weights: file too short at layer %d (need %zu more floats, have %zu)", i, need, avail - ptr);
        std::vector<double> scale(co, 1.0);
        std::vector<float> bias(co);
        if (l.bn) {
            const float *beta = w + ptr, *gamma = beta + co, *mean = gamma + co, *var = mean + co;
            for (int o = 0; o < co; ++o) {
                scale[o] = (double)gamma[o] / sqrt((double)var[o] + 1e-5);
                bias[o] = (float)((double)beta[o] - (double)mean[o] * scale[o]);
            }
        } else {
            for (int o = 0; o < co; ++o) bias[o] = w[ptr + o];
        }
        ptr += (size_t)(l.bn ? 4 : 1) * co;
        l.cw.upload(w + ptr, scale.data(), bias.data(), stream);
        ptr += nw;
    }
    for (Layer &a : layers) {
        if (a.merge_next < 0) continue;
        const Layer &b = layers[a.merge_next];
        if (a.cw.loaded() && b.cw.loaded()) a.cw_merged = ConvWeights::concat(a.cw, b.cw, stream);
    }
}

ConvArgs Darknet::conv_args(int i, int batch, int first, bool merged) const {
    const Layer &l = layers[i];
    ConvArgs a;
    a.x = l.src < 0 ? input_view(batch, first) : view(l.src, batch, first);
    a.y = view(i, batch, first);
    l.cw.fill(a);
    a.act = l.act;
    if (l.fused_res >= 0) { a.res = view(l.fused_res, batch, first); a.res_mode = RES_AFTER_ACT; }
    a.terms = half_mode ? 1 : 3;
    if (merged) {
        a.y2 = view(l.merge_next, batch, first);
        a.n_split = a.y.c;
        a.y.c = a.y.c + a.y2.c;
        l.cw_merged.fill(a);
    }
    return a;
}

const LaunchPlan &Darknet::plan(int batch) {
    LaunchPlan &p = plan_;
    if (p.batch == batch && p.math == conv_math() && p.epoch == plan_epoch) return p;
    p.batch = batch; p.math = conv_math(); p.epoch = plan_epoch;
    p.steps.clear();
    p.produced_by.assign(layers.size(), -1);
    static const bool no_stem = getenv("YDS_NO_STEM_FUSE") != nullptr, no_block = getenv("YDS_NO_BLOCK_FUSE") != nullptr;
    const bool f16x3 = p.math == MATH_F16X3;
    auto has_w = [&](int i) { return layers[i].cw.loaded(); };
    auto kargs = [&](int i) { return make_conv_args(conv_args(i, batch)); };
    const bool stem = !no_stem && stem_fusable && f16x3 && has_w(0) && has_w(1) && view(1, batch).fmt != FMT_F32 &&
                      conv_stem2_applicable(kargs(0), kargs(1));
    const bool block1 = !no_block && block1_at >= 0 && f16x3 && has_w(block1_at) && has_w(block1_at + 1) &&
                        conv_block1_applicable(kargs(block1_at), kargs(block1_at + 1));
    int heads = 0;
    auto add = [&](Step::Kind kind, int layer) -> Step & {
        p.produced_by[layer] = (int)p.steps.size();
        p.steps.push_back(Step{kind, layer});
        return p.steps.back();
    };
    for (int i = 0; i < (int)layers.size(); ++i) {
        const Layer &l = layers[i];
        switch (l.type) {
        case L_CONV:
            if (l.merged_into >= 0 && layers[l.merged_into].cw_merged.loaded()) p.produced_by[i] = p.produced_by[l.merged_into];
            else if ((i == 0 && stem) || (i == block1_at && block1)) break;
            else if (i == 1 && stem) add(Step::CONV_STEM2, i);
            else if (i == block1_at + 1 && block1) add(Step::CONV_BLOCK1, i);
            else add(l.cw_merged.loaded() ? Step::CONV_MERGED : Step::CONV, i);
            break;
        case L_MAXPOOL: {
            Step &st = add(Step::MAXPOOL, i);
            st.src = l.src; st.ksize = l.ksize; st.stride = l.stride; st.pad = l.pad; st.zero_br = l.zero_br;
            if (l.stride != 1 || l.zero_br || l.ksize < 9 || l.pad != (l.ksize - 1) / 2) break;
            for (int j = i - 1; j >= 0; --j) {
                const Layer &q = layers[j];
                if (q.type == L_MAXPOOL && q.stride == 1 && !q.zero_br && q.ksize == l.ksize - 4 && q.pad == (q.ksize - 1) / 2 && q.c == l.c &&
                    layers[q.src].root == layers[l.src].root && layers[q.src].coff == layers[l.src].coff) {
                    st.src = j; st.ksize = 5; st.pad = 2;
                    break;
                }
            }
            break;
        }
        case L_UPSAMPLE: add(Step::UPSAMPLE, i); break;
        case L_ROUTE:
            for (auto &cp : l.copies) {
                Step &st = add(Step::COPY, i);
                st.src = cp.first; st.arg = cp.second;
            }
            break;
        case L_SHORTCUT:
            if (!l.fused) add(Step::ADD, i);
            break;
        case L_YOLO: add(Step::YOLO, i).arg = heads++; break;
        }
    }
    return p;
}

void Darknet::autotune(int batch) {
    const int mode = conv_math() + (half_mode ? 10 : 0);
    auto tune = [&](int i, bool merged) {
        Layer &l = layers[i];
        if (!l.cw.loaded() || (l.tuned_batch == batch && l.tuned_math == mode)) return;
        l.variant = conv_autotune(conv_args(i, batch, 0, merged), stream, nullptr);
        l.tuned_batch = batch;
        l.tuned_math = mode;
    };
    for (const Step &st : plan(batch).steps) {
        if (st.kind > Step::CONV_BLOCK1) continue;
        if (st.kind == Step::CONV_STEM2 || st.kind == Step::CONV_BLOCK1) tune(st.layer - 1, false);
        tune(st.layer, st.kind == Step::CONV_MERGED);
    }
}

void Darknet::check_pass(int batch) const {
    if (batch < 1 || batch > batch_max) fail("forward: batch %d outside [1,%d]", batch, batch_max);
    if (math != conv_math()) fail("forward: this network was planned for conv math %d, current mode is %d (re-create it)", math, conv_math());
}

void Darknet::run_graph(int batch) {
    check_pass(batch);
    int lanes = getenv("YDS_DET_LANES") ? atoi(getenv("YDS_DET_LANES")) : 1;
    while (lanes > 1 && batch / lanes < 4) --lanes;
    if (lanes < 1) lanes = 1;
    if (lanes == 1) { run_lane(0, batch, stream); return; }
    while ((int)lane_streams.size() < lanes - 1) {
        hipStream_t st; hipEvent_t ev;
        YDS_HIP(hipStreamCreateWithFlags(&st, hipStreamNonBlocking));
        YDS_HIP(hipEventCreateWithFlags(&ev, hipEventDisableTiming));
        lane_streams.push_back(st); lane_done.push_back(ev);
    }
    if (!lane_fork) YDS_HIP(hipEventCreateWithFlags(&lane_fork, hipEventDisableTiming));
    const int per = (batch + lanes - 1) / lanes;
    YDS_HIP(hipEventRecord(lane_fork, stream));
    for (int k = 0; k < lanes; ++k) {
        const int first = k * per, cnt = std::min(per, batch - first);
        if (cnt <= 0) break;
        hipStream_t st = (k == 0 || time_convs) ? stream : lane_streams[k - 1];
        if (st != stream) YDS_HIP(hipStreamWaitEvent(st, lane_fork, 0));
        run_lane(first, cnt, st);
        if (st != stream) {
            YDS_HIP(hipEventRecord(lane_done[k - 1], st));
            YDS_HIP(hipStreamWaitEvent(stream, lane_done[k - 1], 0));
        }
    }
}

int Darknet::head_layers() const {
    double total = 0, acc = 0;
    for (int i = 0; i < (int)layers.size(); ++i)
        if (layers[i].type == L_CONV) total += conv_flops(conv_args(i, 1));
    for (int i = 0; i < (int)layers.size(); ++i) {
        if (layers[i].type != L_CONV) continue;
        acc += conv_flops(conv_args(i, 1));
        if (acc >= 0.06 * total) return i + 1;
    }
    return (int)layers.size();
}

bool Darknet::forward_resized_part(int batch, int part) {
    check_pass(batch);
    if (getenv("YDS_DET_LANES") && atoi(getenv("YDS_DET_LANES")) > 1) return false;
    const int cut = head_layers();
    if (part == 0) run_lane(0, batch, stream, 0, cut);
    else run_lane(0, batch, stream, cut, -1);
    return true;
}

void Darknet::enqueue_conv(const Step &st, int first, int batch, hipStream_t stream) {
    const int i = st.layer;
    const Layer &l = layers[i];
    if (!l.cw.loaded()) fail("forward: layer %d has no weights (call load_darknet_weights)", i);
    const ConvArgs a = conv_args(i, batch, first, st.kind == Step::CONV_MERGED);
    ConvTimeRec rec;
    if (time_convs) { rec.e0 = timing_event(); rec.e1 = timing_event(); YDS_HIP(hipEventRecord(rec.e0, stream)); }
    int variant;
    double extra_flops = 0, extra_bytes = 0;
    if (st.kind == Step::CONV_STEM2) {
        const ConvArgs a0 = conv_args(i - 1, batch, first);
        ConvKernelArgs k0 = make_conv_args(a0), k1 = make_conv_args(a);
        k1.w = reinterpret_cast<const float *>(a.w16);
        launch_conv_stem2(k0, k1, stream);
        variant = VAR_DIRECT_RGB;
        extra_flops = conv_flops(a0);
        extra_bytes = conv_bytes(a0) - conv_bytes_io(a0.y) - conv_bytes_io(a.x);
    } else if (st.kind == Step::CONV_BLOCK1) {
        const ConvArgs a2 = conv_args(i - 1, batch, first);
        ConvKernelArgs k2 = make_conv_args(a2), k3 = make_conv_args(a);
        k2.w = reinterpret_cast<const float *>(a2.w16);
        k3.w = reinterpret_cast<const float *>(a.w16);
        launch_conv_block1(k2, k3, stream);
        variant = VAR_WIN_256x128;
        extra_flops = conv_flops(a2);
        extra_bytes = conv_bytes(a2) - conv_bytes_io(a2.y) - conv_bytes_io(a.x) - (a.res.p ? conv_bytes_io(a.res) : 0.0);
    } else {
        variant = launch_conv(a, stream, l.variant);
    }
    if (time_convs) {
        YDS_HIP(hipEventRecord(rec.e1, stream));
        rec.variant = variant;
        rec.flops = conv_flops(a) + extra_flops;
        rec.bytes = conv_bytes(a) + extra_bytes;
        const double peak = conv_math() == MATH_F32 ? 157.3e12 : (a.terms == 1 ? 2500e12 : 2500e12 / 3);
        rec.attain_us = std::max(rec.flops / peak, rec.bytes / 6.29e12) * 1e6;
        conv_pending.push_back(rec);
    }
}

void Darknet::run_lane(int first, int batch, hipStream_t stream, int l0, int l1) {
    autotune(batch);
    if (l1 < 0) l1 = (int)layers.size();
    auto v = [&](int layer) { return view(layer, batch, first); };
    for (const Step &st : plan(batch).steps) {
        const int i = st.layer;
        if (i < l0) continue;
        if (i >= l1) break;
        const Layer &l = layers[i];
        switch (st.kind) {
        case Step::CONV: case Step::CONV_MERGED: case Step::CONV_STEM2: case Step::CONV_BLOCK1:
            enqueue_conv(st, first, batch, stream);
            break;
        case Step::MAXPOOL: launch_maxpool(v(st.src), v(i), st.ksize, st.stride, st.pad, st.zero_br, stream); break;
        case Step::UPSAMPLE: launch_upsample(v(l.src), v(i), l.stride, stream); break;
        case Step::COPY: {
            View d = v(i);
            d.p += fmt_slots(d.fmt, st.arg);
            launch_copy(v(st.src), d, stream);
            break;
        }
        case Step::ADD: launch_add(v(l.refs[0]), v(l.refs[1]), v(i), stream); break;
        case Step::YOLO: {
            const View head = v(l.src);
            const int hidx = st.arg;
            if (inject_active && inject_set >= 0) {
                launch_inject_batch(head, batch, inject_table.p, inject_offsets_dev.p + (size_t)inject_set * batch_max + first, inject_max_rows, hidx,
                                    l.classes, inject_logit, stream);
            } else {
                for (int b = 0; b < batch && inject_active; ++b)
                    launch_inject(head, b, inject_rows[first + b].p, inject_n[first + b], hidx, l.classes, inject_logit, stream);
            }
            launch_yolo_decode(head, out.p + (size_t)first * total_boxes * attrs, total_boxes, l.box_off, l.classes, l.anchors.data(), (int)l.anchors.size() / 2, img_h, img_w, stream);
            break;
        }
        }
    }
}

void Darknet::forward_f32_host(const float *nchw, int batch, float *out_host) {
    size_t n = (size_t)batch * in_channels * img_h * img_w;
    YDS_HIP(hipMemcpyAsync(stage_f32.p, nchw, n * sizeof(float), hipMemcpyHostToDevice, stream));
    launch_nchw_to_nhwc(stage_f32.p, input_view(batch), in_channels, stream);
    run_graph(batch);
    if (out_host) YDS_HIP(hipMemcpyAsync(out_host, out.p, (size_t)batch * total_boxes * attrs * sizeof(float), hipMemcpyDeviceToHost, stream));
    YDS_HIP(hipStreamSynchronize(stream));
}

void Darknet::forward_u8_dev(const uint8_t *frames_dev, int h, int w, int batch) {
    if (in_channels != 3) fail("forward_u8: network expects %d channels", in_channels);
    check_pass(batch);
    launch_resize_u8(frames_dev, batch, h, w, input_view(batch), stream);
    run_graph(batch);
}

void Darknet::forward_u8_frames_dev(const uint8_t *frames_dev, const std::vector<FrameGeom> &geom) {
    const int batch = (int)geom.size();
    if (in_channels != 3) fail("forward_u8: network expects %d channels", in_channels);
    check_pass(batch);
    std::vector<SlotRec> slots;
    for (const FrameGeom &g : geom) slots.push_back(plain_slot(g.off, g.h, g.w));
    slot_tab.upload(slots.data(), slots.size(), stream);
    YDS_HIP(hipStreamSynchronize(stream));
    launch_slot_resize(frames_dev, slot_tab.p, batch, input_view(batch), stream, false);
    run_graph(batch);
}

void Darknet::forward_u8_host(const uint8_t *frames, int h, int w, int batch, float *out_host) {
    size_t n = (size_t)batch * h * w * 3;
    stage_u8.ensure(n);
    YDS_HIP(hipMemcpyAsync(stage_u8.p, frames, n, hipMemcpyHostToDevice, stream));
    stage_h = h; stage_w = w; stage_n = batch;
    forward_u8_dev(stage_u8.p, h, w, batch);
    if (out_host) YDS_HIP(hipMemcpyAsync(out_host, out.p, (size_t)batch * total_boxes * attrs * sizeof(float), hipMemcpyDeviceToHost, stream));
    YDS_HIP(hipStreamSynchronize(stream));
}

void Darknet::forward_slots(const uint8_t *frames_dev, const SlotRec *slots, int n_slots, float *pred, bool bgr) {
    for (int slot0 = 0; slot0 < n_slots; slot0 += batch_max) {
        const int nb = std::min(batch_max, n_slots - slot0);
        launch_slot_resize(frames_dev, slots + slot0, nb, input_view(nb), stream, bgr);
        run_graph(nb);
        launch_slot_boxes(out.p, total_boxes, attrs, slots + slot0, nb, pred + (size_t)slot0 * total_boxes * attrs, stream);
    }
}

void Darknet::forward_tiles_host(const uint8_t *frame, int h, int w, const int *tiles_xyhw, int n_tiles) {
    if (in_channels != 3) fail("forward_tiles: network expects %d channels", in_channels);
    if (n_tiles < 1) fail("forward_tiles: no windows");
    for (int t = 0; t < n_tiles; ++t) {
        const int x = tiles_xyhw[t * 4], y = tiles_xyhw[t * 4 + 1], th = tiles_xyhw[t * 4 + 2], tw = tiles_xyhw[t * 4 + 3];
        if (x < 0 || y < 0 || th < 1 || tw < 1 || x + tw > w || y + th > h) fail("forward_tiles: window %d (%d,%d,%d,%d) outside the %dx%d frame", t, x, y, th, tw, w, h);
    }
    const size_t nbytes = (size_t)h * w * 3;
    stage_u8.ensure(nbytes);
    tiled_pred.ensure((size_t)n_tiles * total_boxes * attrs);
    YDS_HIP(hipMemcpyAsync(stage_u8.p, frame, nbytes, hipMemcpyHostToDevice, stream));
    stage_h = h; stage_w = w; stage_n = 1;
    std::vector<SlotRec> slots;
    for (int t = 0; t < n_tiles; ++t)
        slots.push_back(window_slot(0, w, tiles_xyhw[t * 4], tiles_xyhw[t * 4 + 1], tiles_xyhw[t * 4 + 2], tiles_xyhw[t * 4 + 3], img_h, img_w));
    slot_tab.upload(slots.data(), slots.size(), stream);
    forward_slots(stage_u8.p, slot_tab.p, n_tiles, tiled_pred.p, false);
    YDS_HIP(hipStreamSynchronize(stream));
}

void Darknet::layer_output_host(int i, int batch, float *nchw) {
    if (i < 0 || i >= (int)layers.size()) fail("layer_output: no layer %d", i);
    const Layer &l = layers[i];
    if (l.type == L_CONV && l.cw.loaded() && plan(batch).produced_by[i] < 0) (void)launch_conv(conv_args(i, batch), stream, l.variant);
    if (l.type == L_YOLO) fail("layer_output: yolo layers are read through the forward output");
    if (l.fused_res >= 0) fail("layer_output: layer %d is fused with the following shortcut", i);
    nhwc_to_host(view(i, batch), nchw, stream);
}

void Darknet::get_input_host(int batch, float *nchw) {
    View v = input_view(batch);
    v.c = in_channels;
    nhwc_to_host(v, nchw, stream);
}

void Darknet::set_injection(int image, const float *rows, int n, float logit) {
    if (image < 0 || image >= batch_max) fail("inject: image %d outside batch", image);
    inject_n[image] = n;
    if (n > 0) inject_rows[image].upload(rows, (size_t)n * 9, stream);
    YDS_HIP(hipStreamSynchronize(stream));
    inject_logit = logit;
    inject_active = false;
    for (int b = 0; b < batch_max; ++b) inject_active |= inject_n[b] > 0;
}

void Darknet::load_injection_sets(const float *rows, const int *offsets, int n_sets, float logit) {
    if (n_sets <= 0) { inject_set = -1; inject_active = false; inject_offsets.clear(); return; }
    inject_offsets.assign(offsets, offsets + (size_t)n_sets * batch_max + 1);
    inject_table.ensure((size_t)inject_offsets.back() * 9 + 9);
    inject_table.upload(rows, (size_t)inject_offsets.back() * 9, stream);
    inject_offsets_dev.ensure(inject_offsets.size());
    inject_offsets_dev.upload(inject_offsets.data(), inject_offsets.size(), stream);
    inject_max_rows = 0;
    for (size_t i = 0; i + 1 < inject_offsets.size(); ++i) inject_max_rows = std::max(inject_max_rows, inject_offsets[i + 1] - inject_offsets[i]);
    YDS_HIP(hipStreamSynchronize(stream));
    inject_logit = logit;
    inject_set = 0;
    inject_active = true;
}

void Darknet::select_injection_set(int set) {
    if (inject_offsets.empty()) fail("inject: no sets loaded");
    int n_sets = (int)(inject_offsets.size() - 1) / batch_max;
    if (set < 0 || set >= n_sets) fail("inject: set %d outside [0,%d)", set, n_sets);
    inject_set = set;
}

int64_t Darknet::flops_per_image() const {
    int64_t f = 0;
    for (const Layer &l : layers)
        if (l.type == L_CONV) f += 2ll * l.h * l.w * l.c * l.cw.ksize * l.cw.ksize * l.cw.cin_file;
    return f;
}

void Darknet::enable_conv_timing(bool on) {
    if (!on) resolve_conv_timing();
    time_convs = on;
}

hipEvent_t Darknet::timing_event() {
    if (!ev_pool.empty()) { hipEvent_t e = ev_pool.back(); ev_pool.pop_back(); return e; }
    hipEvent_t e;
    YDS_HIP(hipEventCreate(&e));
    return e;
}

void Darknet::resolve_conv_timing() {
    if (conv_pending.empty()) return;
    YDS_HIP(hipStreamSynchronize(stream));
    for (const ConvTimeRec &r : conv_pending) {
        float ms = 0;
        YDS_HIP(hipEventElapsedTime(&ms, r.e0, r.e1));
        conv_us[r.variant] += ms * 1e3;
        conv_launches[r.variant]++;
        conv_flops_acc[r.variant] += r.flops;
        conv_bytes_acc[r.variant] += r.bytes;
        conv_attain_us[r.variant] += r.attain_us;
        ev_pool.push_back(r.e0);
        ev_pool.push_back(r.e1);
    }
    conv_pending.clear();
}

}

using yds::Darknet;

extern "C" {

yds_net *yds_darknet_create(const char *cfg_text, int img_h, int img_w, int batch_max) {
    YDS_API_BEGIN
    if (!cfg_text) yds::fail("cfg_text is NULL");
    if (img_h <= 0 || img_w <= 0 || batch_max <= 0) yds::fail("bad geometry %dx%d batch %d", img_h, img_w, batch_max);
    auto *n = new yds_net{new Darknet(cfg_text, img_h, img_w, batch_max)};
    return n;
    YDS_API_END_PTR
}
void yds_darknet_destroy(yds_net *n) {
    if (n) { delete n->d; delete n; }
}
int yds_darknet_load_weights(yds_net *n, const void *blob, size_t nbytes, int cutoff) {
    YDS_API_BEGIN
    n->d->load_weights(blob, nbytes, cutoff);
    YDS_API_END
}
int yds_darknet_set_batch_max(yds_net *n, int batch_max) {
    YDS_API_BEGIN
    n->d->set_batch_max(batch_max);
    YDS_API_END
}
int yds_darknet_batch_max(const yds_net *n) { return n->d->batch_max; }
int yds_darknet_set_half(yds_net *n, int on) {
    YDS_API_BEGIN
    if (on && n->d->math != yds::MATH_F16X3) yds::fail("half mode needs the split-fp16 tensor formats (conv math f16x3)");
    n->d->set_half(on != 0);
    YDS_API_END
}
int yds_darknet_layer_format(const yds_net *n, int layer) {
    if (!n || layer < 0 || layer >= (int)n->d->layers.size() || n->d->layers[layer].type == yds::L_YOLO) return -1;
    return n->d->view(layer, 1).fmt;
}
int yds_darknet_num_boxes(const yds_net *n) { return n->d->total_boxes; }
int yds_darknet_num_attrs(const yds_net *n) { return n->d->attrs; }
int yds_darknet_num_layers(const yds_net *n) { return (int)n->d->layers.size(); }
int yds_darknet_layer_shape(const yds_net *n, int layer, int *c, int *h, int *w) {
    YDS_API_BEGIN
    if (layer < 0 || layer >= (int)n->d->layers.size()) yds::fail("no layer %d", layer);
    const auto &l = n->d->layers[layer];
    *c = l.c; *h = l.h; *w = l.w;
    YDS_API_END
}
int64_t yds_darknet_conv_flops(const yds_net *n) { return n->d->flops_per_image(); }
int yds_darknet_forward_f32(yds_net *n, const float *nchw_host, int batch, float *out_host) {
    YDS_API_BEGIN
    n->d->forward_f32_host(nchw_host, batch, out_host);
    YDS_API_END
}
int yds_darknet_forward_u8(yds_net *n, const uint8_t *rgb, int h, int w, int batch, float *out_host) {
    YDS_API_BEGIN
    n->d->forward_u8_host(rgb, h, w, batch, out_host);
    YDS_API_END
}
const uint8_t *yds_darknet_last_frames_dev(yds_net *n, int *h, int *w, int *batch) {
    if (!n || !n->d->stage_n) return nullptr;
    *h = n->d->stage_h; *w = n->d->stage_w; *batch = n->d->stage_n;
    return n->d->stage_u8.p;
}
int yds_darknet_forward_u8_dev(yds_net *n, const uint8_t *rgb_dev, int h, int w, int batch) {
    YDS_API_BEGIN
    n->d->forward_u8_dev(rgb_dev, h, w, batch);
    YDS_API_END
}
int yds_darknet_forward_u8_mixed_dev(yds_net *n, const uint8_t *rgb_dev, const uint64_t *frame_off, const int32_t *frame_hw, size_t frames_bytes,
                                     int batch) {
    YDS_API_BEGIN
    if (!rgb_dev) yds::fail("forward_u8: NULL frames");
    n->d->forward_u8_frames_dev(rgb_dev, yds::checked_layout(frame_off, frame_hw, batch, frames_bytes));
    YDS_API_END
}
int yds_darknet_layer_output(yds_net *n, int layer, int batch, float *nchw_host) {
    YDS_API_BEGIN
    n->d->layer_output_host(layer, batch, nchw_host);
    YDS_API_END
}
int yds_darknet_get_input(yds_net *n, int batch, float *nchw_host) {
    YDS_API_BEGIN
    n->d->get_input_host(batch, nchw_host);
    YDS_API_END
}
int yds_darknet_set_injection(yds_net *n, int image, const float *rows, int cnt, float logit) {
    YDS_API_BEGIN
    n->d->set_injection(image, rows, cnt, logit);
    YDS_API_END
}
int yds_conv_timing_ex(yds_net *n, int mode, double *total_us, int64_t *launches, double *flops, double *bytes, double *attainable_us) {
    YDS_API_BEGIN
    Darknet *d = n->d;
    if (mode == 2) d->enable_conv_timing(false);
    else d->resolve_conv_timing();
    for (int v = 0; v < yds::kConvVariants; ++v) {
        if (total_us) total_us[v] = d->conv_us[v];
        if (launches) launches[v] = d->conv_launches[v];
        if (flops) flops[v] = d->conv_flops_acc[v];
        if (bytes) bytes[v] = d->conv_bytes_acc[v];
        if (attainable_us) attainable_us[v] = d->conv_attain_us[v];
    }
    if (mode == 1) {
        for (int v = 0; v < yds::kConvVariants; ++v) {
            d->conv_us[v] = 0; d->conv_launches[v] = 0; d->conv_flops_acc[v] = 0; d->conv_bytes_acc[v] = 0; d->conv_attain_us[v] = 0;
        }
        d->enable_conv_timing(true);
    }
    YDS_API_END
}
int yds_conv_timing(yds_net *n, int mode, double *total_us4, int64_t *launches4, double *flops4) {
    return yds_conv_timing_ex(n, mode, total_us4, launches4, flops4, nullptr, nullptr);
}
const char *yds_conv_variant_name(int v) { return yds::conv_variant_name(v); }
int yds_conv_num_variants(void) { return yds::kConvVariants; }
int yds_set_conv_math(int mode) { yds::set_conv_math(mode); return 0; }
int yds_get_conv_math(void) { return yds::conv_math(); }
int yds_conv_clock(double *ghz, double *sampled_ms, int reset) {
    YDS_API_BEGIN
    double g = 0, ms = 0;
#ifdef YDS_CLOCK_PROBE
    YDS_HIP(hipDeviceSynchronize());
    unsigned long long a[2], b[2], c[2];
    yds::conv_win_clock(a, reset != 0);
    yds::conv_win2_clock(b, reset != 0);
    yds::conv_win16_clock(c, reset != 0);
    const double cycles = (double)a[0] + (double)b[0] + (double)c[0], ticks = (double)a[1] + (double)b[1] + (double)c[1];
    g = ticks > 0 ? cycles / ticks * 0.1 : 0.0;
    ms = ticks * 1e-5;
#else
    (void)reset;
#endif
    if (ghz) *ghz = g;
    if (sampled_ms) *sampled_ms = ms;
    YDS_API_END
}
int yds_darknet_load_injection_sets(yds_net *n, const float *rows_host, const int32_t *offsets_host, int n_sets, float logit) {
    YDS_API_BEGIN
    n->d->load_injection_sets(rows_host, offsets_host, n_sets, logit);
    YDS_API_END
}
int yds_darknet_select_injection_set(yds_net *n, int set) {
    YDS_API_BEGIN
    n->d->select_injection_set(set);
    YDS_API_END
}

}
```

yolo_deepsort_amd/csrc/engine.h:

```cpp
#pragma once
#include "common.h"
#include "conv_weights.h"

#include <map>
#include <memory>
#include <string>
#include <utility>
#include <vector>

namespace yds {

struct CfgBlock {
    std::string type;
    std::map<std::string, std::string> kv;
};
std::vector<CfgBlock> parse_cfg(const std::string &text);

enum LayerType { L_CONV, L_MAXPOOL, L_UPSAMPLE, L_ROUTE, L_SHORTCUT, L_YOLO };

struct Layer {
    LayerType type = L_CONV;
    int c = 0, h = 0, w = 0;
    int root = -1, coff = 0;
    int src = -1;
    std::vector<int> refs;
    std::vector<std::pair<int, int>> copies;
    bool concat() const { return type == L_ROUTE && refs.size() > 1; }
    int bn = 0, act = ACT_LINEAR;
    ConvWeights cw;
    int fused_res = -1;
    int variant = -1, tuned_batch = 0, tuned_math = -1;
    int merge_next = -1, merged_into = -1;
    ConvWeights cw_merged;
    int ksize = 1, stride = 1, pad = 0;
    bool fused = false, zero_br = false;
    int groups = 0, group_id = 0;
    std::vector<float> anchors;
    int classes = 0, box_off = 0;
};

struct Step {
    enum Kind { CONV, CONV_MERGED, CONV_STEM2, CONV_BLOCK1, MAXPOOL, UPSAMPLE, COPY, ADD, YOLO };
    Kind kind;
    int layer;
    int src = -1;
    int arg = 0;
    int ksize = 1, stride = 1, pad = 0;
    bool zero_br = false;
};
struct LaunchPlan {
    std::vector<Step> steps;
    std::vector<int> produced_by;
    int batch = -1, math = -1, epoch = -1;
};

struct Storage {
    DevBuf<float> buf;
    int ld = 0;
    int fmt = 0;
    int fmt_half = 0;
    bool owns = false;
    bool redirected = false;
    int into = -1, coff = 0;
};

class Darknet {
public:
    Darknet(const std::string &cfg_text, int img_h, int img_w, int batch_max);
    ~Darknet();
    void load_weights(const void *blob, size_t nbytes, int cutoff);
    void set_batch_max(int b);
    void forward_f32_host(const float *nchw, int batch, float *out_host);
    void forward_u8_host(const uint8_t *frames, int h, int w, int batch, float *out_host);
    void forward_u8_dev(const uint8_t *frames_dev, int h, int w, int batch);
    void forward_u8_frames_dev(const uint8_t *frames_dev, const std::vector<FrameGeom> &geom);
    void forward_resized(int batch) { run_graph(batch); }
    bool forward_resized_part(int batch, int part);
    int head_layers() const;
    void forward_tiles_host(const uint8_t *frame, int h, int w, const int *tiles_xyhw, int n_tiles);
    void forward_slots(const uint8_t *frames_dev, const SlotRec *slots, int n_slots, float *pred, bool bgr);
    void layer_output_host(int layer, int batch, float *nchw);
    void get_input_host(int batch, float *nchw);
    void set_injection(int image, const float *rows, int n, float logit);
    void load_injection_sets(const float *rows, const int *offsets, int n_sets, float logit);
    void select_injection_set(int set);
    void enable_conv_timing(bool on);
    void autotune(int batch);
    int64_t flops_per_image() const;
    View view(int layer, int batch, int first = 0) const;
    View input_view(int batch, int first = 0) const;
    ConvArgs conv_args(int layer, int batch, int first = 0, bool merged = false) const;

    int img_h, img_w, batch_max, in_channels = 3;
    int math = 0;
    bool half_mode = false;
    void set_half(bool on);
    void plan_half_formats();
    int owner_of(int layer, int &off) const;
    int total_boxes = 0, attrs = 0;
    std::vector<Layer> layers;
    std::vector<Storage> storage;
    std::vector<int> yolo_layers;
    DevBuf<float> input, out, stage_f32;
    DevBuf<uint8_t> stage_u8;
    DevBuf<SlotRec> slot_tab;
    int stage_h = 0, stage_w = 0, stage_n = 0;
    DevBuf<float> tiled_pred;
    hipStream_t stream = nullptr;
    std::vector<DevBuf<float>> inject_rows;
    std::vector<int> inject_n;
    bool inject_active = false;
    DevBuf<float> inject_table;
    std::vector<int> inject_offsets;
    DevBuf<int> inject_offsets_dev;
    int inject_max_rows = 0;
    int inject_set = -1;
    float inject_logit = 6.f;
    struct ConvTimeRec { hipEvent_t e0 = nullptr, e1 = nullptr; int variant = 0; double flops = 0, bytes = 0, attain_us = 0; };
    bool time_convs = false;
    std::vector<ConvTimeRec> conv_pending;
    std::vector<hipEvent_t> ev_pool;
    hipEvent_t timing_event();
    void resolve_conv_timing();
    double conv_us[kConvVariants] = {}, conv_flops_acc[kConvVariants] = {}, conv_bytes_acc[kConvVariants] = {}, conv_attain_us[kConvVariants] = {};
    int64_t conv_launches[kConvVariants] = {};

private:
    void allocate_buffers();
    void check_pass(int batch) const;
    void run_graph(int batch);
    void run_lane(int first, int batch, hipStream_t st, int l0 = 0, int l1 = -1);
    void enqueue_conv(const Step &st, int first, int batch, hipStream_t s);
    const LaunchPlan &plan(int batch);
    LaunchPlan plan_;
    int plan_epoch = 0;
    bool stem_fusable = false;
    int block1_at = -1;
    std::vector<hipStream_t> lane_streams;
    std::vector<hipEvent_t> lane_done;
    hipEvent_t lane_fork = nullptr;
};

struct NmsUniform { int32_t n_boxes, corner, merge; float sx, sy; };
class NmsWorkspace {
public:
    explicit NmsWorkspace(int max_candidates = 16384, int frames = 1);
    ~NmsWorkspace();
    NmsWorkspace(const NmsWorkspace &) = delete;
    void launch(const float *pred_dev, const NmsUniform &u, int n_frames, int attrs, float conf_thres, float iou_thres, int cap, hipStream_t s);
    void launch(const float *pred_dev, const NmsFrame *fr, int n_frames, int max_rows, size_t total_rows, int attrs, float conf_thres,
                float iou_thres, int cap, hipStream_t s);
    int collect(int frame, float *out6_host, int cap);
    void resize(int max_candidates, int n_frames);
    int needed(int n_frames) const;
    static constexpr int kMaxCandidates = 1 << 18;
    int run(const float *pred_dev, int n_boxes, int attrs, float conf_thres, float iou_thres, float sx, float sy,
            float *out6_host, int cap, hipStream_t s);
    int run_merge(const float *pred_dev, int n_boxes, int attrs, float conf_thres, float iou_thres, float *out6_host, int cap, hipStream_t s);
    int max_cand, frames;
    DevBuf<float> cand;
    DevBuf<float> sorted;
    DevBuf<int> counts;
    DevBuf<int> box_count;
    DevBuf<unsigned long long> mask;
    DevBuf<float> kept;
    int *h_counts = nullptr;
    float *h_kept = nullptr;
};

class ReidNet {
public:
    explicit ReidNet(int max_crops);
    ~ReidNet();
    void load_tensor(const std::string &name, const float *data, const int64_t *shape, int ndim);
    void finalize();
    void embed_dev(const uint8_t *frame_dev, int h, int w, const float *tlwh_host, int D, float *out_host);
    void embed_multi_dev(const uint8_t *frames_dev, int h, int w, const float *tlwh_host, const int *frame_of, int D, bool bgr = false,
                         const FrameGeom *geom = nullptr, int n_geom = 0);
    void preprocess_frames_dev(const uint8_t *frames_dev, const std::vector<FrameGeom> &geom, const float *tlwh_host, const int *frame_of, int D,
                               float *nchw_host);
    void embed_host(const uint8_t *frame_host, int h, int w, const float *tlwh_host, int D, float *out_host);
    void preprocess_host(const uint8_t *frame_host, int h, int w, const float *tlwh_host, int D, float *nchw_host);
    void forward_f32_host(const float *nchw, int D, float *out_host);
    void forward(int D, const ReidFront *front = nullptr);
    void reserve(int D);
    float *in_buf();
    void crop_into_in(const ReidFront &f, int D);
    ReidFront stage_crops(const uint8_t *frames_dev, int h, int w, const float *tlwh_host, const int *frame_of, int D, bool bgr,
                          const FrameGeom *geom, int n_geom);
    void allocate_buffers();
    static int64_t flops_per_crop();

    int max_crops;
    std::map<std::string, std::vector<float>> raw;
    std::map<std::string, std::vector<int64_t>> raw_shape;
    bool ready = false;
    std::vector<ConvWeights> convs;
    std::vector<DevBuf<float>> bufs;
    DevBuf<float> in, feat, stage_f32;
    DevBuf<uint8_t> stage_u8;
    DevBuf<int> boxes_dev;
    std::vector<int> boxes_host;
    int *boxes_pin[2] = {nullptr, nullptr};
    size_t boxes_pin_cap[2] = {0, 0};
    int boxes_pin_turn = 0;
    hipStream_t sync_before_regrow = nullptr;
    std::map<int, std::pair<int, int>> tuned;
    int tuned_math = -1;
    hipStream_t stream = nullptr;
    double conv_flops_last = 0;
    bool front_fused_last = false;
};

struct ActFrame {
    const int32_t *rows6;
    const int32_t *n_rows_p;
    int n_rows, stream, tag;
    double t;
    const double *row_time;
};
struct ActionsIface {
    virtual ~ActionsIface() {}
    virtual int streams() const = 0;
    virtual void enqueue(const ActFrame *fr, int n, hipStream_t s) = 0;
    virtual void collect() = 0;
    std::vector<int32_t> rows4, first;
};

struct ZonesIface {
    virtual ~ZonesIface() {}
    virtual int streams() const = 0;
    virtual void enqueue(const ActFrame *fr, int n, hipStream_t s) = 0;
    virtual void collect() = 0;
    std::vector<int32_t> ev6, first;
    std::vector<double> evt2;
};

struct GalleryView {
    const float *gallery;
    const int *slot, *id, *state, *n_feat;
    int budget, n_tracks, metric;
    double max_dist;
    const int *n_tracks_dev;
    int capacity, unbounded;
    const int *hits;
};
struct TrackerIface {
    virtual ~TrackerIface() {}
    virtual GalleryView gallery_view() const = 0;
    virtual int step(const float *tlwh_host, const float *feats, bool feats_on_device, const float *payload_host, int D,
                     int32_t *out6_host, int cap) = 0;
    virtual int num_tracks() const = 0;
};
struct IdentityIface {
    virtual ~IdentityIface() {}
    virtual bool bound_to(TrackerIface *const *trk, int S) const = 0;
    virtual void enqueue_collect(hipStream_t s) = 0;
    virtual void finish(hipStream_t s) = 0;
    virtual void get(int stream, int32_t *track_id, int32_t *global_id, int cap, int *n) const = 0;
    std::shared_ptr<void *> user;
    bool (*user_busy)(void *) = nullptr;
};

struct TrackerGroupIface {
    virtual ~TrackerGroupIface() {}
    virtual void set_identities(IdentityIface *ident) = 0;
    virtual void set_actions(ActionsIface *act, const double *frame_times) = 0;
    virtual void set_zones(ZonesIface *zones, const double *frame_times) = 0;
    virtual void step_batch(TrackerIface *const *trk, int S, int n, const int *stream_of, const float *tlwh_host, const int *first,
                            const float *feats_dev, const float *payload_host, const char *skip, int32_t *out6_host, int cap, int32_t *counts) = 0;
    virtual void wait_for(hipEvent_t ev) = 0;
};
TrackerGroupIface *make_tracker_group();

}

struct yds_net { yds::Darknet *d; };
struct yds_reid { yds::ReidNet *r; };
struct yds_trk { yds::TrackerIface *t; };
struct yds_act { yds::ActionsIface *a; };
struct yds_ident { yds::IdentityIface *i; };
struct yds_zones { yds::ZonesIface *z; };
```

yolo_deepsort_amd/csrc/layers.hip:

```cpp
#include "common.h"

#include <algorithm>
#include "h16.h"
#include "resize_dev.h"

namespace yds {

static inline int grid_for(size_t work, int block = 256) {
    size_t g = (work + block - 1) / block;
    if (g > 8192) g = 8192;
    if (g < 1) g = 1;
    return (int)g;
}

__global__ void maxpool_kernel(const float *x, float *y, int N, int H, int W, int C, int ldx, int Ho, int Wo, int ldy,
                               int k, int stride, int pad, int zero_br, int fmt_in, int fmt_out) {
    fp16_saturate_on();
    const int C4 = C >> 2;
    const size_t total = (size_t)N * Ho * Wo * C4;
    for (size_t idx = blockIdx.x * (size_t)blockDim.x + threadIdx.x; idx < total; idx += (size_t)gridDim.x * blockDim.x) {
        int c4 = idx % C4;
        size_t pix = idx / C4;
        int ox = pix % Wo;
        size_t t = pix / Wo;
        int oy = t % Ho;
        int n = t / Ho;
        float4 m = make_float4(-INFINITY, -INFINITY, -INFINITY, -INFINITY);
        for (int dy = 0; dy < k; ++dy) {
            int iy = oy * stride - pad + dy;
            for (int dx = 0; dx < k; ++dx) {
                int ix = ox * stride - pad + dx;
                float v[4] = {0.f, 0.f, 0.f, 0.f};
                if ((unsigned)iy < (unsigned)H && (unsigned)ix < (unsigned)W)
                    load4(x + ((size_t)(n * H + iy) * W + ix) * ldx, c4 * 4, fmt_in, v);
                else if (!zero_br)
                    continue;
                m.x = fmaxf(m.x, v[0]); m.y = fmaxf(m.y, v[1]); m.z = fmaxf(m.z, v[2]); m.w = fmaxf(m.w, v[3]);
            }
        }
        const float o[4] = {m.x, m.y, m.z, m.w};
        store4(y + pix * ldy, c4 * 4, fmt_out, o);
    }
}

void launch_maxpool(const View &x, const View &y, int k, int stride, int pad, bool zero_pad_br, hipStream_t s) {
    if (x.c % 4 || x.ld % 4 || y.ld % 4) fail("maxpool: channels must be a multiple of 4");
    size_t total = y.pixels() * (x.c / 4);
    hipLaunchKernelGGL(maxpool_kernel, dim3(grid_for(total)), dim3(256), 0, s, x.p, y.p, x.n, x.h, x.w, x.c, x.ld, y.h, y.w,
                       y.ld, k, stride, pad, zero_pad_br ? 1 : 0, x.fmt, y.fmt);
    YDS_HIP(hipGetLastError());
}

__global__ void upsample_kernel(const float *x, float *y, int N, int H, int W, int C, int ldx, int ldy, int s) {
    const int C4 = C >> 2, Ho = H * s, Wo = W * s;
    const size_t total = (size_t)N * Ho * Wo * C4;
    for (size_t idx = blockIdx.x * (size_t)blockDim.x + threadIdx.x; idx < total; idx += (size_t)gridDim.x * blockDim.x) {
        int c4 = idx % C4;
        size_t pix = idx / C4;
        int ox = pix % Wo;
        size_t t = pix / Wo;
        int oy = t % Ho;
        int n = t / Ho;
        *reinterpret_cast<float4 *>(y + pix * ldy + c4 * 4) =
            *reinterpret_cast<const float4 *>(x + ((size_t)(n * H + oy / s) * W + ox / s) * ldx + c4 * 4);
    }
}

void launch_upsample(const View &x, const View &y, int stride, hipStream_t s) {
    if (x.c % 4 || x.ld % 4 || y.ld % 4) fail("upsample: channels must be a multiple of 4");
    if (x.fmt != y.fmt) fail("upsample: source and destination formats differ");
    const int slots = fmt_slots(x.fmt, x.c);
    if (slots % 4) fail("upsample: channels must fill whole 16-byte pieces");
    size_t total = y.pixels() * (slots / 4);
    hipLaunchKernelGGL(upsample_kernel, dim3(grid_for(total)), dim3(256), 0, s, x.p, y.p, x.n, x.h, x.w, slots, x.ld, y.ld, stride);
    YDS_HIP(hipGetLastError());
}

__global__ void copy_kernel(const float *x, float *y, size_t pixels, int C, int ldx, int ldy) {
    const int C4 = C >> 2;
    const size_t total = pixels * C4;
    for (size_t idx = blockIdx.x * (size_t)blockDim.x + threadIdx.x; idx < total; idx += (size_t)gridDim.x * blockDim.x) {
        int c4 = idx % C4;
        size_t pix = idx / C4;
        *reinterpret_cast<float4 *>(y + pix * ldy + c4 * 4) = *reinterpret_cast<const float4 *>(x + pix * ldx + c4 * 4);
    }
}
__global__ void copy_scalar_kernel(const float *x, float *y, size_t pixels, int C, int ldx, int ldy) {
    const size_t total = pixels * C;
    for (size_t idx = blockIdx.x * (size_t)blockDim.x + threadIdx.x; idx < total; idx += (size_t)gridDim.x * blockDim.x) {
        int c = idx % C;
        size_t pix = idx / C;
        y[pix * ldy + c] = x[pix * ldx + c];
    }
}

void launch_copy(const View &x, const View &y, hipStream_t s) {
    if (x.fmt != y.fmt) fail("copy: source and destination formats differ");
    const int slots = fmt_slots(x.fmt, x.c);
    bool vec = !(slots % 4 || x.ld % 4 || y.ld % 4 || ((uintptr_t)x.p & 15) || ((uintptr_t)y.p & 15));
    if (vec)
        hipLaunchKernelGGL(copy_kernel, dim3(grid_for(x.pixels() * (slots / 4))), dim3(256), 0, s, x.p, y.p, x.pixels(), slots, x.ld, y.ld);
    else
        hipLaunchKernelGGL(copy_scalar_kernel, dim3(grid_for(x.pixels() * slots)), dim3(256), 0, s, x.p, y.p, x.pixels(), slots, x.ld, y.ld);
    YDS_HIP(hipGetLastError());
}

__global__ void add_kernel(const float *a, const float *b, float *y, size_t pixels, int C, int lda, int ldb, int ldy, int fa, int fb, int fy) {
    fp16_saturate_on();
    const int C4 = C >> 2;
    const size_t total = pixels * C4;
    for (size_t idx = blockIdx.x * (size_t)blockDim.x + threadIdx.x; idx < total; idx += (size_t)gridDim.x * blockDim.x) {
        int c4 = idx % C4;
        size_t pix = idx / C4;
        float u[4], v[4];
        load4(a + pix * lda, c4 * 4, fa, u);
        load4(b + pix * ldb, c4 * 4, fb, v);
        const float o[4] = {u[0] + v[0], u[1] + v[1], u[2] + v[2], u[3] + v[3]};
        store4(y + pix * ldy, c4 * 4, fy, o);
    }
}

void launch_add(const View &a, const View &b, const View &y, hipStream_t s) {
    if (a.c % 4 || a.ld % 4 || b.ld % 4 || y.ld % 4) fail("add: channels must be a multiple of 4");
    hipLaunchKernelGGL(add_kernel, dim3(grid_for(a.pixels() * (a.c / 4))), dim3(256), 0, s, a.p, b.p, y.p, a.pixels(), a.c, a.ld, b.ld, y.ld,
                       a.fmt, b.fmt, y.fmt);
    YDS_HIP(hipGetLastError());
}

__global__ void nchw_to_nhwc_kernel(const float *src, float *y, int N, int C, int H, int W, int ldy, int Cdst) {
    const size_t total = (size_t)N * H * W * Cdst;
    for (size_t idx = blockIdx.x * (size_t)blockDim.x + threadIdx.x; idx < total; idx += (size_t)gridDim.x * blockDim.x) {
        int c = idx % Cdst;
        size_t pix = idx / Cdst;
        int xw = pix % W;
        size_t t = pix / W;
        int yh = t % H;
        int n = t / H;
        y[pix * ldy + c] = c < C ? src[((size_t)(n * C + c) * H + yh) * W + xw] : 0.f;
    }
}
void launch_nchw_to_nhwc(const float *src_nchw, const View &y, int c_src, hipStream_t s) {
    hipLaunchKernelGGL(nchw_to_nhwc_kernel, dim3(grid_for(y.pixels() * y.c)), dim3(256), 0, s, src_nchw, y.p, y.n, c_src, y.h, y.w, y.ld, y.c);
    YDS_HIP(hipGetLastError());
}

__global__ void nhwc_to_nchw_kernel(const float *x, float *dst, int N, int C, int H, int W, int ldx, int fmt) {
    const size_t total = (size_t)N * C * H * W;
    for (size_t idx = blockIdx.x * (size_t)blockDim.x + threadIdx.x; idx < total; idx += (size_t)gridDim.x * blockDim.x) {
        int xw = idx % W;
        size_t t = idx / W;
        int yh = t % H;
        t /= H;
        int c = t % C;
        int n = t / C;
        const float *pixel = x + ((size_t)(n * H + yh) * W + xw) * ldx;
        if (fmt == FMT_H16 || fmt == FMT_F16) {
            float v[4];
            load4(pixel, c & ~3, fmt, v);
            dst[idx] = v[c & 3];
        } else {
            dst[idx] = pixel[c];
        }
    }
}
__global__ void pack_h16_kernel(const float *src, float *y, size_t pixels, int C, int ldy) {
    fp16_saturate_on();
    const int C4 = C >> 2;
    const size_t total = pixels * C4;
    for (size_t idx = blockIdx.x * (size_t)blockDim.x + threadIdx.x; idx < total; idx += (size_t)gridDim.x * blockDim.x) {
        int c4 = idx % C4;
        size_t pix = idx / C4;
        float4 t = *reinterpret_cast<const float4 *>(src + pix * C + c4 * 4);
        const float v[4] = {t.x, t.y, t.z, t.w};
        h16_store4(y + pix * ldy, c4 * 4, v);
    }
}
void launch_pack_h16(const float *src_f32, const View &y, hipStream_t s) {
    if (y.c % 32 || y.ld % 32) fail("pack_h16: channels must be a multiple of 32");
    hipLaunchKernelGGL(pack_h16_kernel, dim3(grid_for(y.pixels() * (y.c / 4))), dim3(256), 0, s, src_f32, y.p, y.pixels(), y.c, y.ld);
    YDS_HIP(hipGetLastError());
}

void launch_nhwc_to_nchw(const View &x, float *dst_nchw, hipStream_t s) {
    hipLaunchKernelGGL(nhwc_to_nchw_kernel, dim3(grid_for(x.pixels() * x.c)), dim3(256), 0, s, x.p, dst_nchw, x.n, x.c, x.h, x.w, x.ld, x.fmt);
    YDS_HIP(hipGetLastError());
}

struct YoloParams {
    float aw[8], ah[8];
    float s0, s1;
};

__global__ void yolo_decode_kernel(const float *head, float *out, int N, int H, int W, int ld, int A, int attrs, int total_boxes,
                                   int box_off, YoloParams yp) {
    const int HW = H * W, n = blockIdx.y, per_cell = A * attrs;
    (void)N;
    const int lane = threadIdx.x & 63;
    const int wave0 = __builtin_amdgcn_readfirstlane((int)((blockIdx.x * blockDim.x + threadIdx.x) >> 6));
    const int nwaves = (int)((gridDim.x * blockDim.x) >> 6);
    for (int cell = wave0; cell < HW; cell += nwaves) {
        const int gy = cell / W, gx = cell - gy * W;
        const float *src = head + ((size_t)(n * H + gy) * W + gx) * ld;
        float *dst = out + ((size_t)n * total_boxes + box_off + cell) * attrs;
        for (int i = lane; i < per_cell; i += 64) {
            int a = 0;
#pragma unroll
            for (int k = 1; k < 8; ++k) a += (k < A && i >= k * attrs) ? 1 : 0;
            const int t = i - a * attrs;
            const float v = src[i];
            float r;
            if (t == 0) r = __fmul_rn(__fadd_rn(1.f / (1.f + expf(-v)), (float)gx), yp.s0);
            else if (t == 1) r = __fmul_rn(__fadd_rn(1.f / (1.f + expf(-v)), (float)gy), yp.s1);
            else if (t == 2) r = __fmul_rn(__fmul_rn(expf(v), yp.aw[a]), yp.s0);
            else if (t == 3) r = __fmul_rn(__fmul_rn(expf(v), yp.ah[a]), yp.s1);
            else r = 1.f / (1.f + expf(-v));
            dst[(size_t)a * HW * attrs + t] = r;
        }
    }
}

void launch_yolo_decode(const View &head, float *out, int total_boxes, int box_off, int num_classes, const float *anchors_wh,
                        int A, int img_h, int img_w, hipStream_t s) {
    if (A > 8) fail("yolo: at most 8 anchors per head");
    YoloParams yp;
    yp.s0 = (float)((double)img_h / head.h);
    yp.s1 = (float)((double)img_w / head.w);
    for (int a = 0; a < A; ++a) {
        yp.aw[a] = anchors_wh[2 * a] / yp.s0;
        yp.ah[a] = anchors_wh[2 * a + 1] / yp.s1;
    }
    int attrs = num_classes + 5;
    if (head.c != A * attrs) fail("yolo: head has %d channels, expected %d", head.c, A * attrs);
    const size_t per_img = (size_t)A * head.h * head.w * attrs;
    if (per_img >= (1ull << 31)) fail("yolo: head too large for 32-bit indexing");
    const unsigned cells = (unsigned)head.h * head.w;
    hipLaunchKernelGGL(yolo_decode_kernel, dim3(std::min((cells + 3) / 4, 2048u), head.n), dim3(256), 0, s, head.p, out, head.n, head.h, head.w,
                       head.ld, A, attrs, total_boxes, box_off, yp);
    YDS_HIP(hipGetLastError());
}

__global__ void inject_clear_kernel(float *head, int image, int H, int W, int ld, int A, int attrs, float logit) {
    int total = H * W * A;
    for (int idx = blockIdx.x * blockDim.x + threadIdx.x; idx < total; idx += gridDim.x * blockDim.x) {
        int a = idx % A, cell = idx / A;
        head[((size_t)image * H * W + cell) * ld + a * attrs + 4] = -logit;
    }
}
__device__ __forceinline__ bool inject_row_superseded(const float *rows, int r, int n) {
    const float *row = rows + (size_t)r * 9;
    for (int j = r + 1; j < n; ++j) {
        const float *o = rows + (size_t)j * 9;
        if (o[0] == row[0] && o[1] == row[1] && o[2] == row[2] && o[3] == row[3]) return true;
    }
    return false;
}
__global__ void inject_rows_kernel(float *head, int image, int H, int W, int ld, int attrs, const float *rows, int n, int head_index,
                                   float logit) {
    int r = blockIdx.x;
    if (r >= n) return;
    const float *row = rows + r * 9;
    if ((int)row[0] != head_index) return;
    if (inject_row_superseded(rows, r, n)) return;
    int a = (int)row[1], gy = (int)row[2], gx = (int)row[3], cls = (int)row[8];
    float *cell = head + ((size_t)(image * H + gy) * W + gx) * ld + a * attrs;
    for (int t = threadIdx.x; t < attrs; t += blockDim.x) {
        float v;
        if (t < 4) v = row[4 + t];
        else if (t == 4) v = logit;
        else v = (t - 5 == cls) ? logit : -logit;
        cell[t] = v;
    }
}
void launch_inject(const View &head, int image, const float *rows_dev, int n, int head_index, int num_classes, float logit,
                   hipStream_t s) {
    int attrs = num_classes + 5, A = head.c / attrs;
    hipLaunchKernelGGL(inject_clear_kernel, dim3(grid_for((size_t)head.h * head.w * A)), dim3(256), 0, s, head.p, image, head.h, head.w,
                       head.ld, A, attrs, logit);
    if (n > 0)
        hipLaunchKernelGGL(inject_rows_kernel, dim3(n), dim3(128), 0, s, head.p, image, head.h, head.w, head.ld, attrs, rows_dev, n,
                           head_index, logit);
    YDS_HIP(hipGetLastError());
}

__global__ void inject_clear_batch_kernel(float *head, int H, int W, int ld, int A, int attrs, float logit) {
    const int total = H * W * A, image = blockIdx.y;
    for (int idx = blockIdx.x * blockDim.x + threadIdx.x; idx < total; idx += gridDim.x * blockDim.x) {
        int a = idx % A, cell = idx / A;
        head[((size_t)image * H * W + cell) * ld + a * attrs + 4] = -logit;
    }
}
__global__ void inject_rows_batch_kernel(float *head, int H, int W, int ld, int attrs, const float *table, const int *offsets, int head_index,
                                         float logit) {
    const int image = blockIdx.y, o0 = offsets[image], n = offsets[image + 1] - o0, r = blockIdx.x;
    if (r >= n) return;
    const float *row = table + (size_t)(o0 + r) * 9;
    if ((int)row[0] != head_index) return;
    if (inject_row_superseded(table + (size_t)o0 * 9, r, n)) return;
    int a = (int)row[1], gy = (int)row[2], gx = (int)row[3], cls = (int)row[8];
    float *cell = head + ((size_t)(image * H + gy) * W + gx) * ld + a * attrs;
    for (int t = threadIdx.x; t < attrs; t += blockDim.x) {
        float v;
        if (t < 4) v = row[4 + t];
        else if (t == 4) v = logit;
        else v = (t - 5 == cls) ? logit : -logit;
        cell[t] = v;
    }
}
void launch_inject_batch(const View &head, int batch, const float *table_dev, const int *offsets_dev, int max_rows, int head_index,
                         int num_classes, float logit, hipStream_t s) {
    int attrs = num_classes + 5, A = head.c / attrs;
    hipLaunchKernelGGL(inject_clear_batch_kernel, dim3(min(grid_for((size_t)head.h * head.w * A), 64), batch), dim3(256), 0, s, head.p, head.h,
                       head.w, head.ld, A, attrs, logit);
    if (max_rows > 0)
        hipLaunchKernelGGL(inject_rows_batch_kernel, dim3(max_rows, batch), dim3(128), 0, s, head.p, head.h, head.w, head.ld, attrs, table_dev,
                           offsets_dev, head_index, logit);
    YDS_HIP(hipGetLastError());
}


__global__ void resize_u8_kernel(const uint8_t *frames, int N, int H, int W, float *y, int Ho, int Wo, int ldy, int bgr) {
    const size_t total = (size_t)N * Ho * Wo;
    for (size_t idx = blockIdx.x * (size_t)blockDim.x + threadIdx.x; idx < total; idx += (size_t)gridDim.x * blockDim.x) {
        int ox = idx % Wo;
        size_t t = idx / Wo;
        int oy = t % Ho;
        int n = t / Ho;
        float o[3];
        resize_px(frames + (size_t)n * H * W * 3, (size_t)W * 3, H, W, Ho, Wo, oy, ox, o);
        if (bgr) { const float t = o[0]; o[0] = o[2]; o[2] = t; }
        *reinterpret_cast<float4 *>(y + idx * ldy) = make_float4(__fdiv_rn(o[0], 255.f), __fdiv_rn(o[1], 255.f), __fdiv_rn(o[2], 255.f), 0.f);
    }
}

void launch_resize_u8(const uint8_t *frames, int n, int h, int w, const View &y, hipStream_t s, bool bgr) {
    if (y.c != 4 || y.ld != 4) fail("resize: destination must be NHWC4");
    hipLaunchKernelGGL(resize_u8_kernel, dim3(grid_for((size_t)n * y.h * y.w)), dim3(256), 0, s, frames, n, h, w, y.p, y.h, y.w, y.ld, bgr ? 1 : 0);
    YDS_HIP(hipGetLastError());
}

__global__ void slot_resize_kernel(const uint8_t *frames, const SlotRec *slots, float *y, int Ho, int Wo, int bgr) {
    const SlotRec g = slots[blockIdx.y];
    const int per = Ho * Wo;
    float *dst = y + (size_t)blockIdx.y * per * 4;
    for (int idx = blockIdx.x * blockDim.x + threadIdx.x; idx < per; idx += gridDim.x * blockDim.x) {
        const int oy = idx / Wo, ox = idx - oy * Wo;
        float o[3];
        resize_px(frames + g.off, (size_t)g.stride, g.th, g.tw, Ho, Wo, oy, ox, o);
        if (bgr) { const float v = o[0]; o[0] = o[2]; o[2] = v; }
        *reinterpret_cast<float4 *>(dst + (size_t)idx * 4) = make_float4(__fdiv_rn(o[0], 255.f), __fdiv_rn(o[1], 255.f), __fdiv_rn(o[2], 255.f), 0.f);
    }
}

void launch_slot_resize(const uint8_t *frames, const SlotRec *slots, int n, const View &y, hipStream_t s, bool bgr) {
    if (y.c != 4 || y.ld != 4) fail("resize: destination must be NHWC4");
    if (n < 1 || n > 65535) fail("resize: %d slots", n);
    const int per_slot = grid_for((size_t)y.h * y.w), gx = std::min(per_slot, std::max(1, 8192 / n));
    hipLaunchKernelGGL(slot_resize_kernel, dim3(gx, n), dim3(256), 0, s, frames, slots, y.p, y.h, y.w, bgr ? 1 : 0);
    YDS_HIP(hipGetLastError());
}

__global__ void slot_boxes_kernel(const float *pred, int n_boxes, int attrs, const SlotRec *slots, int n, float *dst) {
    const size_t total = (size_t)n * n_boxes;
    for (size_t row = blockIdx.x * (size_t)(blockDim.x / 32) + threadIdx.x / 32; row < total; row += (size_t)gridDim.x * (blockDim.x / 32)) {
        const SlotRec &g = slots[row / n_boxes];
        const int lane = threadIdx.x % 32;
        const float *p = pred + row * attrs;
        float *d = dst + row * attrs;
        for (int j = 4 + lane; j < attrs; j += 32) d[j] = p[j];
        if (lane < 4) {
            float v = p[lane];
            if (g.window) {
                const float half = __fdiv_rn(p[2 + (lane & 1)], 2.f);
                v = lane < 2 ? __fsub_rn(p[lane & 1], half) : __fadd_rn(p[lane & 1], half);
                v = __fmul_rn(v, lane & 1 ? g.sy : g.sx);
                v = __fadd_rn(v, (float)(lane & 1 ? g.y0 : g.x0));
            }
            d[lane] = v;
        }
    }
}

void launch_slot_boxes(const float *pred, int n_boxes, int attrs, const SlotRec *slots, int n, float *dst, hipStream_t s) {
    hipLaunchKernelGGL(slot_boxes_kernel, dim3(grid_for((size_t)n * n_boxes * 32)), dim3(256), 0, s, pred, n_boxes, attrs, slots, n, dst);
    YDS_HIP(hipGetLastError());
}

__global__ void crop_resize_kernel(ReidFront f, int D, float *y, int Ho, int Wo) {
    const size_t total = (size_t)D * Ho * Wo;
    for (size_t idx = blockIdx.x * (size_t)blockDim.x + threadIdx.x; idx < total; idx += (size_t)gridDim.x * blockDim.x) {
        int ox = idx % Wo;
        size_t t = idx / Wo;
        int oy = t % Ho;
        int d = t / Ho;
        const int *b = f.boxes + (size_t)d * 5;
        int x1 = b[0], y1 = b[1], cw = b[2] - x1, ch = b[3] - y1, fi = b[4];
        size_t off = (size_t)fi * f.h * f.w * 3;
        int W = f.w;
        if (f.geom) { const FrameGeom g = f.geom[fi]; off = g.off; W = g.w; }
        const float mean[3] = {0.485f, 0.456f, 0.406f}, stdv[3] = {0.229f, 0.224f, 0.225f};
        float o[3];
        resize_px(f.frames + off + ((size_t)y1 * W + x1) * 3, (size_t)W * 3, ch, cw, Ho, Wo, oy, ox, o);
        if (f.bgr) { const float t = o[0]; o[0] = o[2]; o[2] = t; }
#pragma unroll
        for (int c = 0; c < 3; ++c) o[c] = __fdiv_rn(__fsub_rn(__fdiv_rn(o[c], 255.f), mean[c]), stdv[c]);
        *reinterpret_cast<float4 *>(y + idx * 4) = make_float4(o[0], o[1], o[2], 0.f);
    }
}

void launch_crop_resize(const ReidFront &f, int D, const View &y, hipStream_t s) {
    if (D == 0) return;
    hipLaunchKernelGGL(crop_resize_kernel, dim3(grid_for((size_t)D * y.h * y.w)), dim3(256), 0, s, f, D, y.p, y.h, y.w);
    YDS_HIP(hipGetLastError());
}

__global__ void avgpool_l2norm_kernel(const float *x, float *out, int P, int C, int ld, int fmt) {
    __shared__ float red[8];
    const int d = blockIdx.x;
    float v[2], ss = 0.f;
#pragma unroll
    for (int j = 0; j < 2; ++j) {
        int c = threadIdx.x + j * blockDim.x;
        float sum = 0.f;
        for (int p = 0; p < P; ++p) {
            const float *pixel = x + ((size_t)d * P + p) * ld;
            if (fmt == FMT_H16) {
                float q[4];
                h16_load4(pixel, c & ~3, q);
                sum += q[c & 3];
            } else {
                sum += pixel[c];
            }
        }
        v[j] = sum / (float)P;
        ss += v[j] * v[j];
    }
    for (int o = 32; o > 0; o >>= 1) ss += __shfl_down(ss, o, 64);
    if ((threadIdx.x & 63) == 0) red[threadIdx.x >> 6] = ss;
    __syncthreads();
    float tot = 0.f;
    for (int i = 0; i < (int)(blockDim.x >> 6); ++i) tot += red[i];
    float nrm = sqrtf(tot);
#pragma unroll
    for (int j = 0; j < 2; ++j) out[(size_t)d * C + threadIdx.x + j * blockDim.x] = v[j] / nrm;
}

void launch_avgpool_l2norm(const View &x, float *out, hipStream_t s) {
    if (x.n == 0) return;
    if (x.c != 512) fail("avgpool: expected 512 channels");
    hipLaunchKernelGGL(avgpool_l2norm_kernel, dim3(x.n), dim3(256), 0, s, x.p, out, x.h * x.w, x.c, x.ld, x.fmt);
    YDS_HIP(hipGetLastError());
}

}
```

yolo_deepsort_amd/csrc/pipeline.cpp:

```cpp
#include "engine.h"

#include <limits.h>
#include <stdlib.h>
#include <string.h>

#include <algorithm>
#include <chrono>
#include <utility>

namespace yds {

struct DetSlot {
    std::unique_ptr<NmsWorkspace> nms;
    hipEvent_t e0, e1, e2, e_nms;
    hipEvent_t e_r0, e_r1;
    bool reid_in_pass = false;
    DetSlot() { for (hipEvent_t *e : {&e0, &e1, &e2, &e_nms, &e_r0, &e_r1}) YDS_HIP(hipEventCreate(e)); }
    ~DetSlot() {
        for (hipEvent_t e : {e0, e1, e2, e_nms, e_r0, e_r1}) (void)hipEventDestroy(e);
        if (plan_tab) (void)hipHostFree(plan_tab);
    }
    void *plan_tab = nullptr;
    size_t plan_bytes = 0, plan_slots_n = 0;
    const SlotRec *plan_slots() const { return static_cast<const SlotRec *>(plan_tab); }
    const NmsFrame *plan_frames() const { return reinterpret_cast<const NmsFrame *>(plan_slots() + plan_slots_n); }
    void write_plan(const SlotPlan &pl) {
        YDS_HIP(hipEventSynchronize(e1));
        YDS_HIP(hipEventSynchronize(e_nms));
        const size_t need = pl.slots.size() * sizeof(SlotRec) + pl.frames.size() * sizeof(NmsFrame);
        if (plan_bytes < need) {
            if (plan_tab) (void)hipHostFree(plan_tab);
            plan_tab = nullptr;
            plan_bytes = 0;
            YDS_HIP(hipHostMalloc(&plan_tab, std::max<size_t>(need, 4096), hipHostMallocDefault));
            plan_bytes = std::max<size_t>(need, 4096);
        }
        plan_slots_n = pl.slots.size();
        memcpy(plan_tab, pl.slots.data(), pl.slots.size() * sizeof(SlotRec));
        memcpy(const_cast<NmsFrame *>(plan_frames()), pl.frames.data(), pl.frames.size() * sizeof(NmsFrame));
    }
};

struct Geometry {
    int h = 0, w = 0;
    std::vector<FrameGeom> frames;
    bool mixed() const { return !frames.empty(); }
    bool operator==(const Geometry &o) const {
        if (h != o.h || w != o.w || frames.size() != o.frames.size()) return false;
        for (size_t n = 0; n < frames.size(); ++n)
            if (frames[n].off != o.frames[n].off || frames[n].h != o.frames[n].h || frames[n].w != o.frames[n].w) return false;
        return true;
    }
};

struct Pass {
    const uint8_t *frames = nullptr;
    Geometry geo;
    SlotPlan plan;
    int batch = 0;
    int slot = 0;
    enum { NOTHING, HEAD, WHOLE } done = NOTHING;
    bool split = false;
    bool open() const { return frames && done != WHOLE; }
    bool is_whole(const uint8_t *f, int n, const Geometry &g, const SlotPlan &pl) const {
        return frames == f && batch == n && geo == g && plan == pl && done == WHOLE;
    }
};

class FrameStager {
public:
    enum Reader { DET, REID };
    FrameStager(hipStream_t det_stream, hipStream_t reid_stream) : det_stream(det_stream), reid_stream(reid_stream) {
        YDS_HIP(hipStreamCreateWithFlags(&copy_stream, hipStreamNonBlocking));
    }
    ~FrameStager() { (void)hipStreamDestroy(copy_stream); }
    int find(const uint8_t *host) const {
        for (int k = 0; k < N; ++k)
            if (host && slots[k].host == host) return k;
        return -1;
    }
    int slot_of(const uint8_t *dev) const {
        for (int k = 0; k < N; ++k)
            if (slots[k].dev.p && dev == slots[k].dev.p) return k;
        return -1;
    }
    const uint8_t *dev(int k) const { return slots[k].dev.p; }
    int upload(const uint8_t *host, size_t bytes, int ttl, int keep_a = -1, int keep_b = -1) {
        int k = -1;
        for (int pass = 0; pass < 2 && k < 0; ++pass)
            for (int t = 1; t <= N; ++t) {
                const int c = (turn + t) % N;
                if (c == keep_a || c == keep_b || (pass == 0 && slots[c].host)) continue;
                k = c;
                break;
            }
        if (k < 0) fail("pipeline: no staging buffer free");
        turn = k;
        Slot &s = slots[k];
        for (Read &r : s.rd)
            if (r.set) { YDS_HIP(hipStreamWaitEvent(copy_stream, r.ev, 0)); r.set = false; }
        if (s.dev.n < bytes) {
            YDS_HIP(hipStreamSynchronize(det_stream));
            YDS_HIP(hipStreamSynchronize(reid_stream));
        }
        s.dev.ensure(bytes);
        s.ttl = ttl;
        YDS_HIP(hipMemcpyAsync(s.dev.p, host, bytes, hipMemcpyHostToDevice, copy_stream));
        YDS_HIP(hipEventRecord(s.up_done, copy_stream));
        s.host = host;
        s.up_pending = true;
        return k;
    }
    void wait_uploaded(const uint8_t *dev, hipStream_t stream) {
        if (const int k = slot_of(dev); k >= 0 && hipEventQuery(slots[k].up_done) != hipSuccess)
            YDS_HIP(hipStreamWaitEvent(stream, slots[k].up_done, 0));
    }
    void mark_read(const uint8_t *dev, hipStream_t stream, Reader who) {
        if (const int k = slot_of(dev); k >= 0) { YDS_HIP(hipEventRecord(slots[k].rd[who].ev, stream)); slots[k].rd[who].set = true; }
    }
    void end_of_step(int consumed) {
        for (Slot &s : slots)
            if (s.up_pending) { YDS_HIP(hipEventSynchronize(s.up_done)); s.up_pending = false; }
        slots[consumed].host = nullptr;
        for (int k = 0; k < N; ++k)
            if (k != consumed && slots[k].host && --slots[k].ttl <= 0) slots[k].host = nullptr;
        cur = -1;
    }
    int cur = -1, next = -1;

private:
    static constexpr int N = 3;
    struct Read { hipEvent_t ev = nullptr; bool set = false; };
    struct Slot {
        DevBuf<uint8_t> dev;
        const uint8_t *host = nullptr;
        bool up_pending = false;
        int ttl = 0;
        hipEvent_t up_done = nullptr;
        Read rd[2];
        Slot() { for (hipEvent_t *e : {&up_done, &rd[DET].ev, &rd[REID].ev}) YDS_HIP(hipEventCreateWithFlags(e, hipEventDisableTiming)); }
        ~Slot() { for (hipEvent_t e : {up_done, rd[DET].ev, rd[REID].ev}) (void)hipEventDestroy(e); }
    };
    Slot slots[N];
    int turn = 0;
    hipStream_t copy_stream = nullptr, det_stream, reid_stream;
};

class Pipeline {
public:
    Pipeline(Darknet *net, ReidNet *reid, std::vector<TrackerIface *> trks, bool multi, float conf, float nms_iou, const int32_t *mask, int n_mask)
        : net(net), reid(reid), trks(std::move(trks)), group(make_tracker_group()), multi(multi), conf(conf), nms_thres(nms_iou),
          class_mask(mask, mask + n_mask), deep_min(getenv("YDS_PIPE_DEEP_MIN") ? atoi(getenv("YDS_PIPE_DEEP_MIN")) : 64),
          stager(net->stream, reid->stream) {
        for (DetSlot &s : det) s.nms.reset(new NmsWorkspace(4096, net->batch_max));
        YDS_HIP(hipEventCreateWithFlags(&ev_feat, hipEventDisableTiming));
        YDS_HIP(hipEventCreateWithFlags(&ev_reid_done, hipEventDisableTiming));
    }
    ~Pipeline() {
        *self = nullptr;
        (void)hipEventDestroy(ev_feat);
        (void)hipEventDestroy(ev_reid_done);
    }

    void prefetch_host(const uint8_t *frames_host, int h, int w, int batch) {
        if (stager.find(frames_host) >= 0) return;
        stager.upload(frames_host, (size_t)batch * h * w * 3, 3, stager.cur, stager.next);
    }
    void step_host(const uint8_t *frames_host, const uint8_t *next_host, const Geometry &geo, size_t bytes, int batch, int32_t *out6, int cap,
                   int32_t *counts) {
        check_step(geo, batch);
        stager.cur = stager.find(frames_host);
        if (stager.cur < 0) stager.cur = stager.upload(frames_host, bytes, 1, stager.find(next_host));
        stager.next = next_host ? stager.find(next_host) : -1;
        if (next_host && stager.next < 0) stager.next = stager.upload(next_host, bytes, 2, stager.cur);
        step(stager.dev(stager.cur), stager.next >= 0 ? stager.dev(stager.next) : nullptr, geo, batch, out6, cap, counts, true);
        stager.end_of_step(stager.cur);
    }

    void launch_detector(Pass &p, bool split = false) {
        if (p.done == Pass::NOTHING) launch_detector_head(p, split);
        if (p.done == Pass::HEAD) launch_detector_tail(p);
    }
    void launch_detector_head(Pass &p, bool split) {
        DetSlot &s = det[p.slot];
        s.reid_in_pass = false;
        stager.wait_uploaded(p.frames, net->stream);
        YDS_HIP(hipEventRecord(s.e0, net->stream));
        p.done = Pass::HEAD;
        p.split = false;
        if (!p.plan.empty()) s.write_plan(p.plan);
        if (p.plan.windowed) {
            YDS_HIP(hipEventRecord(s.e1, net->stream));
            return;
        }
        if (p.plan.direct()) launch_slot_resize(p.frames, s.plan_slots(), p.batch, net->input_view(p.batch), net->stream, frames_bgr);
        else launch_resize_u8(p.frames, p.batch, p.geo.h, p.geo.w, net->input_view(p.batch), net->stream, frames_bgr);
        YDS_HIP(hipEventRecord(s.e1, net->stream));
        stager.mark_read(p.frames, net->stream, FrameStager::DET);
        p.split = split && net->forward_resized_part(p.batch, 0);
    }
    void launch_detector_tail(Pass &p) {
        DetSlot &s = det[p.slot];
        const size_t per_slot = (size_t)net->total_boxes * net->attrs, n_slots = p.plan.slots.size();
        if (p.plan.windowed) {
            if (win_pred.n < n_slots * per_slot) {
                YDS_HIP(hipStreamSynchronize(net->stream));
                win_pred.alloc(n_slots * per_slot);
            }
            pred_rows = n_slots * net->total_boxes;
            net->forward_slots(p.frames, s.plan_slots(), (int)n_slots, win_pred.p, frames_bgr);
            stager.mark_read(p.frames, net->stream, FrameStager::DET);
        } else if (p.split) {
            (void)net->forward_resized_part(p.batch, 1);
        } else {
            net->forward_resized(p.batch);
        }
        YDS_HIP(hipEventRecord(s.e2, net->stream));
        if (p.plan.empty()) {
            const float sx = box_scale(p.geo.w, net->img_w), sy = box_scale(p.geo.h, net->img_h);
            s.nms->launch(net->out.p, NmsUniform{net->total_boxes, 0, 0, sx, sy}, p.batch, net->attrs, conf, nms_thres, 300, net->stream);
        } else {
            s.nms->launch(p.plan.windowed ? win_pred.p : net->out.p, s.plan_frames(), p.batch, p.plan.max_rows, n_slots * net->total_boxes,
                          net->attrs, conf, nms_thres, 300, net->stream);
        }
        YDS_HIP(hipEventRecord(s.e_nms, net->stream));
        p.done = Pass::WHOLE;
    }

    void set_windows(int ww, int wh, double overlap) {
        if (pending.frames || ahead.reid_in_flight) fail("pipeline: set_windows while a look-ahead pass is in flight (consume it with a step first)");
        if (ww > 0 && wh <= 0) fail("pipeline: window %d x %d", ww, wh);
        if (ww > 0 && !(overlap >= 0)) fail("pipeline: window overlap %g", overlap);
        if (ww > 0 && any_stream_windows()) fail("pipeline: set_windows while a stream holds a window setting of its own (set_stream_windows): one or the other");
        win_w = ww > 0 ? ww : 0; win_h = ww > 0 ? wh : 0; win_overlap = overlap;
    }
    bool any_stream_windows() const {
        for (const WindowSetting &sw : stream_win)
            if (sw.w > 0) return true;
        return false;
    }
    void set_stream_windows(int stream, int ww, int wh, double overlap) {
        if (!multi) fail("pipeline: created by yds_pipeline_create: it has no streams (window mode: yds_pipeline_set_windows)");
        if (stream < 0 || stream >= (int)trks.size()) fail("pipeline: stream %d outside [0,%zu)", stream, trks.size());
        if (ww > 0 && wh <= 0) fail("pipeline: window %d x %d", ww, wh);
        if (ww > 0 && !(overlap >= 0)) fail("pipeline: window overlap %g", overlap);
        if (pending.frames || ahead.reid_in_flight)
            fail("pipeline: set_stream_windows while a look-ahead pass is in flight (consume it with a step first)");
        if (win_w > 0) fail("pipeline: set_stream_windows while window mode is on for all streams (yds_pipeline_set_windows): one or the other");
        stream_win.resize(trks.size());
        stream_win[stream] = ww > 0 ? WindowSetting{ww, wh, overlap} : WindowSetting();
    }
    SlotPlan make_plan(const Geometry &geo, int batch) const {
        std::vector<WindowSetting> win;
        if (win_w > 0) win.push_back(WindowSetting{win_w, win_h, win_overlap});
        else if (multi && any_stream_windows())
            for (int b = 0; b < batch; ++b) win.push_back(stream_win[stream_of[b]]);
        return build_slot_plan(batch, geo.h, geo.w, geo.mixed() ? geo.frames.data() : nullptr, win, net->img_h, net->img_w, net->total_boxes);
    }

    struct Dets {
        std::vector<float> tlwh, payload;
        std::vector<int> frame_of, first, n_det;
        const uint8_t *frames = nullptr;
        Geometry geo;
        SlotPlan plan;
        int batch = 0;
        bool reid_in_flight = false;
        hipStream_t reid_on = nullptr;
    };

    void finish_detector(Dets &d, const Pass &p) {
        DetSlot &s = det[p.slot];
        const int batch = p.batch;
        YDS_HIP(hipEventSynchronize(s.e_nms));
        if (s.nms->needed(batch) > s.nms->max_cand) {
            YDS_HIP(hipStreamSynchronize(net->stream));
            s.nms->resize(s.nms->needed(batch), s.nms->frames);
            Pass redo{p.frames, p.geo, p.plan, batch, p.slot};
            launch_detector(redo);
            if (pending.done == Pass::HEAD) pending.done = Pass::NOTHING;
            YDS_HIP(hipEventSynchronize(s.e_nms));
        }
        float ms01 = 0, ms12 = 0;
        YDS_HIP(hipEventElapsedTime(&ms01, s.e0, s.e1));
        YDS_HIP(hipEventElapsedTime(&ms12, s.e1, s.e2));
        if (s.reid_in_pass) {
            float msr = 0;
            YDS_HIP(hipEventElapsedTime(&msr, s.e_r0, s.e_r1));
            ms12 -= msr;
            s.reid_in_pass = false;
        }
        stage_us[0] = ms01 * 1e3f; stage_us[1] = ms12 * 1e3f;
        std::vector<float> det_rows(300 * 6);
        d.tlwh.clear(); d.payload.clear(); d.frame_of.clear();
        d.first.assign(batch + 1, 0); d.n_det.assign(batch, 0);
        d.frames = p.frames; d.geo = p.geo; d.plan = p.plan; d.batch = batch; d.reid_in_flight = false;
        for (int b = 0; b < batch; ++b) {
            d.n_det[b] = s.nms->collect(b, det_rows.data(), 300);
            for (int i = 0; i < d.n_det[b]; ++i) {
                const float *r = &det_rows[i * 6];
                bool keep = class_mask.empty();
                for (int m : class_mask) keep |= (r[5] == (float)m);
                if (!keep) continue;
                d.tlwh.push_back(r[0]); d.tlwh.push_back(r[1]); d.tlwh.push_back(r[2] - r[0]); d.tlwh.push_back(r[3] - r[1]);
                d.payload.push_back(r[5]);
                d.frame_of.push_back(b);
            }
            d.first[b + 1] = (int)d.payload.size();
        }
    }
    void launch_reid(Dets &d, hipStream_t on = nullptr, const Pass *inside = nullptr) {
        d.reid_on = on ? on : reid->stream;
        if (!d.payload.empty()) {
            struct Swap { hipStream_t &s; hipStream_t keep; ~Swap() { s = keep; } } swap{reid->stream, reid->stream};
            if (reid_last_on && reid_last_on != d.reid_on) YDS_HIP(hipStreamWaitEvent(d.reid_on, ev_reid_done, 0));
            reid->stream = d.reid_on;
            if (reid_last_on && reid_last_on != d.reid_on) reid->sync_before_regrow = reid_last_on;
            if (inside) YDS_HIP(hipEventRecord(det[inside->slot].e_r0, d.reid_on));
            reid->embed_multi_dev(d.frames, d.geo.h, d.geo.w, d.tlwh.data(), d.frame_of.data(), (int)d.payload.size(), frames_bgr,
                                  d.geo.mixed() ? d.geo.frames.data() : nullptr, (int)d.geo.frames.size());
            reid->sync_before_regrow = nullptr;
            if (inside) { YDS_HIP(hipEventRecord(det[inside->slot].e_r1, d.reid_on)); det[inside->slot].reid_in_pass = true; }
            YDS_HIP(hipEventRecord(ev_reid_done, d.reid_on));
            reid_last_on = d.reid_on;
            stager.mark_read(d.frames, d.reid_on, FrameStager::REID);
        }
        d.reid_in_flight = true;
    }

    struct Trial {
        static constexpr int STEPS = 3, GROUPS = 4;
        static constexpr int SKIP = 2, LEN = SKIP + STEPS;
        int n = 0;
        double t0 = 0, t_serial = 0, t_two = 0;
        int decided = 0;
        bool wants_serial() const { return decided ? decided > 0 : (n / LEN) % 2 == 0; }
        void step_done() {
            if (decided) return;
            const double now = std::chrono::duration<double>(std::chrono::steady_clock::now().time_since_epoch()).count();
            const int group = n / LEN, k = n % LEN;
            if (k == SKIP - 1) t0 = now;
            if (k == LEN - 1) {
                double &best = group % 2 == 0 ? t_serial : t_two;
                best = best > 0 ? std::min(best, now - t0) : now - t0;
            }
            ++n;
            if (n == GROUPS * LEN) decided = t_serial <= t_two ? 1 : -1;
        }
    };

    void check_step(const Geometry &geo, int batch) {
        if (batch < 1 || batch > net->batch_max) fail("pipeline: batch %d outside [1,%d]", batch, net->batch_max);
        if (geo.mixed() && (int)geo.frames.size() != batch) fail("pipeline: a layout of %zu frames for a step of %d", geo.frames.size(), batch);
        if (geo.mixed() && win_w > 0)
            fail("pipeline: window mode takes frames of one size (yds_pipeline_step_multi); a mixed layout is refused while windows are set");
    }
    void step(const uint8_t *frames_dev, const uint8_t *next_frames_dev, const Geometry &geo, int batch, int32_t *out6, int cap, int32_t *counts,
              bool uploaded = false) {
        using clk = std::chrono::steady_clock;
        auto us = [](clk::time_point a, clk::time_point b) { return std::chrono::duration<float, std::micro>(b - a).count(); };
        check_step(geo, batch);
        auto t_begin = clk::now();
        const int inject_set = std::exchange(next_inject_set, -1);
        const SlotPlan plan = make_plan(geo, batch);
        const bool resumed = ahead.reid_in_flight && ahead.frames == frames_dev && ahead.batch == batch && ahead.geo == geo && ahead.plan == plan;
        const bool forced = schedule_min_crops != INT_MIN || getenv("YDS_PIPE_SERIAL");
        Trial &trial = trials[uploaded ? 1 : 0];
        const int serial_min = schedule_min_crops != INT_MIN ? schedule_min_crops
                               : getenv("YDS_PIPE_SERIAL")  ? atoi(getenv("YDS_PIPE_SERIAL"))
                               : (trial.wants_serial() ? 256 : -1);
        auto launch_next = [&](int this_slot, bool head_only) {
            pending = next_frames_dev ? Pass{next_frames_dev, geo, plan, batch, this_slot ^ 1} : Pass{nullptr, Geometry(), SlotPlan(), 0, this_slot};
            if (!next_frames_dev) return;
            if (inject_set >= 0) net->select_injection_set(inject_set);
            if (head_only) launch_detector_head(pending, true);
            else launch_detector(pending);
        };
        auto copy_feats = [&]() {
            if (cur.payload.empty()) return;
            feat_cur.ensure((size_t)reid->max_crops * 512);
            YDS_HIP(hipMemcpyAsync(feat_cur.p, reid->feat.p, cur.payload.size() * 512 * sizeof(float), hipMemcpyDeviceToDevice, cur.reid_on));
            YDS_HIP(hipEventRecord(ev_feat, cur.reid_on));
        };
        bool serial = false;
        if (resumed) {
            std::swap(cur, ahead);
            ahead.reid_in_flight = false;
            serial = cur.reid_on == net->stream;
            copy_feats();
            launch_next(pending.slot, false);
        } else {
            ahead.reid_in_flight = false;
            Pass now = pending.is_whole(frames_dev, batch, geo, plan) ? pending : Pass{frames_dev, geo, plan, batch, pending.slot ^ 1};
            launch_detector(now);
            launch_next(now.slot, serial_min >= 0);
            finish_detector(cur, now);
            serial = serial_min >= 0 && (int)cur.payload.size() >= std::max(serial_min, 1);
            if (serial) {
                launch_reid(cur, net->stream, pending.open() ? &pending : nullptr);
                copy_feats();
                if (pending.open()) launch_detector(pending, true);
            } else {
                if (pending.open()) launch_detector(pending, true);
                launch_reid(cur);
                copy_feats();
            }
        }
        last_serial = serial;
        auto t_nms = clk::now();
        const int D_all = (int)cur.payload.size();
        if (D_all) { if (batch == 1 && !next_frames_dev) group->wait_for(ev_feat); else YDS_HIP(hipEventSynchronize(ev_feat)); }
        auto t_reid = clk::now();
        if (next_frames_dev && D_all >= deep_min * batch) {
            finish_detector(ahead, pending);
            pending.frames = nullptr;
            launch_reid(ahead, serial ? net->stream : nullptr);
        }
        std::vector<char> skip(batch, 0);
        for (int b = 0; b < batch; ++b) skip[b] = cur.n_det[b] == 0;
        if (!multi) stream_of.assign(batch, 0);
        std::vector<double> times;
        if ((int)frames_seen.size() < (int)trks.size()) frames_seen.resize(trks.size(), 0);
        const std::vector<double> given = std::move(next_times);
        next_times.clear();
        if (actions || zones) {
            if (!given.empty() && (int)given.size() != batch)
                fail("pipeline: %zu frame times for a step of %d frames (yds_pipeline_set_frame_times)", given.size(), batch);
            times.resize(batch);
            std::vector<int64_t> seen(frames_seen);
            for (int b = 0; b < batch; ++b) times[b] = given.empty() ? (double)seen[stream_of[b]]++ / 25.0 : given[b];
            if (actions) group->set_actions(actions, times.data());
            if (zones) group->set_zones(zones, times.data());
        }
        for (int b = 0; b < batch; ++b) ++frames_seen[stream_of[b]];
        last_actions.clear();
        last_zone_ev6.clear();
        last_zone_evt2.clear();
        if (identities) group->set_identities(identities);
        group->step_batch(trks.data(), (int)trks.size(), batch, stream_of.data(), cur.tlwh.data(), cur.first.data(), feat_cur.p,
                          cur.payload.data(), skip.data(), out6, cap, counts);
        if (actions) last_actions = actions->rows4;
        if (zones) { last_zone_ev6 = zones->ev6; last_zone_evt2 = zones->evt2; }
        auto t_end = clk::now();
        stage_us[2] = us(t_begin, t_nms); stage_us[3] = us(t_nms, t_reid); stage_us[4] = us(t_reid, t_end);
        if (!forced && next_frames_dev && D_all >= 256) trial.step_done();
    }

    void set_streams(const int32_t *stream_of_frame, int n) {
        if (!multi) fail("pipeline: created by yds_pipeline_create: it has no streams (use yds_pipeline_step)");
        if (n < 1 || n > net->batch_max) fail("pipeline: batch %d outside [1,%d]", n, net->batch_max);
        for (int b = 0; b < n; ++b)
            if (stream_of_frame[b] < 0 || stream_of_frame[b] >= (int)trks.size())
                fail("pipeline: frame %d belongs to stream %d outside [0,%zu)", b, stream_of_frame[b], trks.size());
        stream_of.assign(stream_of_frame, stream_of_frame + n);
    }

    void set_actions(ActionsIface *a) {
        if (pending.frames || ahead.reid_in_flight) fail("pipeline: set_actions while a look-ahead pass is in flight (consume it with a step first)");
        if (a && a->streams() < (int)trks.size()) fail("pipeline: an action handle of %d streams for a pipeline of %zu", a->streams(), trks.size());
        actions = a;
        last_actions.clear();
    }
    void set_zones(ZonesIface *z) {
        if (pending.frames || ahead.reid_in_flight) fail("pipeline: set_zones while a look-ahead pass is in flight (consume it with a step first)");
        if (z && z->streams() < (int)trks.size()) fail("pipeline: a zones handle of %d streams for a pipeline of %zu", z->streams(), trks.size());
        zones = z;
        last_zone_ev6.clear();
        last_zone_evt2.clear();
    }
    ZonesIface *zones = nullptr;
    std::vector<int32_t> last_zone_ev6;
    std::vector<double> last_zone_evt2;
    void set_identities(IdentityIface *i) {
        if (pending.frames || ahead.reid_in_flight) fail("pipeline: set_identities while a look-ahead pass is in flight (consume it with a step first)");
        if (i && !i->bound_to(trks.data(), (int)trks.size()))
            fail("pipeline: the identity map was not created over this pipeline's %zu trackers in stream order", trks.size());
        if (identities) identities->user.reset();
        identities = i;
        if (i) {
            i->user = self;
            i->user_busy = [](void *p) { const Pipeline *me = static_cast<const Pipeline *>(p); return me->pending.frames || me->ahead.reid_in_flight; };
        }
    }
    IdentityIface *identities = nullptr;
    std::shared_ptr<void *> self = std::make_shared<void *>(this);
    ActionsIface *actions = nullptr;
    std::vector<double> next_times;
    std::vector<int64_t> frames_seen;
    std::vector<int32_t> last_actions;

    Darknet *net;
    ReidNet *reid;
    std::vector<TrackerIface *> trks;
    std::unique_ptr<TrackerGroupIface> group;
    const bool multi;
    std::vector<int32_t> stream_of;
    float conf, nms_thres;
    std::vector<int32_t> class_mask;
    const int deep_min;
    DetSlot det[2];
    Pass pending;
    FrameStager stager;
    Dets cur, ahead;
    DevBuf<float> feat_cur;
    int next_inject_set = -1;
    hipEvent_t ev_feat = nullptr;
    int schedule_min_crops = INT_MIN;
    Trial trials[2];
    hipEvent_t ev_reid_done = nullptr;
    hipStream_t reid_last_on = nullptr;
    bool last_serial = false;
    bool frames_bgr = false;
    float stage_us[5] = {0, 0, 0, 0, 0};
    int win_w = 0, win_h = 0;
    double win_overlap = 0;
    DevBuf<float> win_pred;
// ... 201 lines not shown
```

yolo_deepsort_amd/csrc/resize_dev.h:

```cpp
#pragma once
#include <hip/hip_runtime.h>
#include <stdint.h>

namespace yds {

struct Tap { int i0, i1, a0, a1; };
__device__ __forceinline__ double cv_scale(int dst, int src) { return __ddiv_rn(1.0, __ddiv_rn((double)dst, (double)src)); }
template <bool X_AXIS> __device__ __forceinline__ Tap axis_tap(int d, double scale, int src) {
    float f = __double2float_rn(__dsub_rn(__dmul_rn((double)d + 0.5, scale), 0.5));
    const float fl = floorf(f);
    int s = (int)fl;
    f = __fsub_rn(f, fl);
    if (X_AXIS) {
        if (s < 0) { s = 0; f = 0.f; }
        if (s >= src - 1) { s = src - 1; f = 0.f; }
    }
    Tap t;
    t.a0 = (int)rintf(__fmul_rn(__fsub_rn(1.f, f), 2048.f));
    t.a1 = (int)rintf(__fmul_rn(f, 2048.f));
    t.i0 = min(max(s, 0), src - 1);
    t.i1 = min(max(s + 1, 0), src - 1);
    return t;
}
enum { RESIZE_LINEAR = 0, RESIZE_AREA2 = 1, RESIZE_COPY = 2 };
__device__ __forceinline__ int resize_mode(int src_h, int src_w, int dst_h, int dst_w) {
    if (src_h == dst_h && src_w == dst_w) return RESIZE_COPY;
    if (src_h == 2 * dst_h && src_w == 2 * dst_w) return RESIZE_AREA2;
    return RESIZE_LINEAR;
}
__device__ __forceinline__ void resize_px(const uint8_t *base, size_t row_bytes, int src_h, int src_w, int dst_h, int dst_w, int oy, int ox,
                                          float o[3]) {
    const int mode = resize_mode(src_h, src_w, dst_h, dst_w);
    if (mode == RESIZE_COPY) {
        const uint8_t *p = base + (size_t)oy * row_bytes + ox * 3;
        o[0] = p[0]; o[1] = p[1]; o[2] = p[2];
        return;
    }
    if (mode == RESIZE_AREA2) {
        const uint8_t *p = base + (size_t)(2 * oy) * row_bytes + 2 * ox * 3, *q = p + row_bytes;
#pragma unroll
        for (int c = 0; c < 3; ++c) o[c] = (float)(((int)p[c] + (int)p[3 + c] + (int)q[c] + (int)q[3 + c] + 2) >> 2);
        return;
    }
    const Tap tx = axis_tap<true>(ox, cv_scale(dst_w, src_w), src_w), ty = axis_tap<false>(oy, cv_scale(dst_h, src_h), src_h);
    const uint8_t *r0 = base + (size_t)ty.i0 * row_bytes, *r1 = base + (size_t)ty.i1 * row_bytes;
#pragma unroll
    for (int c = 0; c < 3; ++c) {
        const int h0 = (int)r0[tx.i0 * 3 + c] * tx.a0 + (int)r0[tx.i1 * 3 + c] * tx.a1;
        const int h1 = (int)r1[tx.i0 * 3 + c] * tx.a0 + (int)r1[tx.i1 * 3 + c] * tx.a1;
        o[c] = (float)(((((ty.a0 * (h0 >> 4)) >> 16) + ((ty.a1 * (h1 >> 4)) >> 16) + 2) >> 2) & 0xff);
    }
}

}
```

yolo_deepsort_amd/models.py:

```python

from __future__ import annotations

import ctypes as C

import numpy as np

from . import _lib
from .loaders import parse_model_config


def _to_numpy(x):
    if hasattr(x, "detach"):
        x = x.detach().cpu().numpy()
    return np.ascontiguousarray(x, dtype=np.float32)


class _Param:

    def __init__(self, device):
        self.device = device


class Darknet:
    def __init__(self, config_path, img_size=416, batch_max=1, cfg_text=None):
        _lib.init()
        if cfg_text is None:
            with open(config_path, "r") as f:
                cfg_text = f.read()
        self.cfg_text = cfg_text
        defs = parse_model_config(config_path, text=cfg_text)
        self.hyperparams = defs.pop(0)
        self.module_defs = defs
        self.img_size = (img_size, img_size) if isinstance(img_size, int) else tuple(img_size)
        self.seen = 0
        self.header_info = np.array([0, 0, 0, self.seen, 0], dtype=np.int32)
        self.batch_max = int(batch_max)
        self.device = f"cuda:{_lib.current_device()}"
        self._half = False
        self._h = None
        self._create()

    def _create(self):
        lib = _lib.load()
        if self._h:
            lib.yds_darknet_destroy(self._h)
        self._h = _lib.check_ptr(lib.yds_darknet_create(self.cfg_text.encode(), self.img_size[0], self.img_size[1],
                                                        self.batch_max))
        self.num_boxes = lib.yds_darknet_num_boxes(self._h)
        self.num_attrs = lib.yds_darknet_num_attrs(self._h)
        blob = getattr(self, "_weights_blob", None)
        if blob is not None:
            _lib.check(lib.yds_darknet_load_weights(self._h, blob, len(blob), self._cutoff))

    def set_batch_max(self, batch_max):
        if batch_max != self.batch_max:
            _lib.check(_lib.load().yds_darknet_set_batch_max(self._h, int(batch_max)))
            self.batch_max = int(batch_max)

    def load_darknet_weights(self, weights_path, blob=None):
        if blob is None:
            with open(weights_path, "rb") as f:
                blob = f.read()
        self.header_info = np.frombuffer(blob[:20], dtype=np.int32).copy()
        self.seen = self.header_info[3]
        self._cutoff = 75 if (weights_path and "darknet53.conv.74" in str(weights_path)) else -1
        self._weights_blob = bytes(blob)
        _lib.check(_lib.load().yds_darknet_load_weights(self._h, self._weights_blob, len(blob), self._cutoff))

    def save_darknet_weights(self, path, cutoff=-1):
        blob = getattr(self, "_weights_blob", None)
        if blob is None:
            raise RuntimeError("no weights loaded")
        from .synth import conv_shapes
        n_blocks = len(self.module_defs)
        stop = n_blocks if cutoff == -1 else (cutoff if cutoff >= 0 else n_blocks + cutoff)
        header = np.array(self.header_info, dtype=np.int32).copy()
        header[3] = self.seen
        floats = 0
        for idx, cin, cout, k, bn, _, _ in conv_shapes(self.cfg_text):
            if idx >= stop:
                break
            floats += (4 if bn else 1) * cout + cout * cin * k * k
        with open(path, "wb") as f:
            f.write(header.tobytes())
            f.write(blob[20:20 + floats * 4])

    def to(self, device):
        self.device = str(device)
        return self

    def cuda(self):
        return self.to(f"cuda:{_lib.current_device()}")

    def eval(self):
        return self

    def half(self):
        _lib.check(_lib.load().yds_darknet_set_half(self._h, 1))
        self._half = True
        return self

    def float(self):
        _lib.check(_lib.load().yds_darknet_set_half(self._h, 0))
        self._half = False
        return self

    def parameters(self):
        yield _Param(self.device)

    def forward(self, x, targets=None):
        if targets is not None:
            raise NotImplementedError("training loss is out of scope (SURVEY 8a)")
        xn = _to_numpy(x)
        if xn.ndim != 4 or xn.shape[2:] != self.img_size:
            raise ValueError(f"expected [B,C,{self.img_size[0]},{self.img_size[1]}], got {xn.shape}")
        b = xn.shape[0]
        if b > self.batch_max:
            self.set_batch_max(b)
        out = np.empty((b, self.num_boxes, self.num_attrs), np.float32)
        _lib.check(_lib.load().yds_darknet_forward_f32(self._h, _lib.ptr(xn), b, _lib.ptr(out)))
        return _wrap_like(x, out)

    __call__ = forward

    def forward_u8(self, frames, want_output=True):
        self._last_frame_src = frames
        frames = np.ascontiguousarray(frames, dtype=np.uint8)
        if frames.ndim == 3:
            frames = frames[None]
        b, h, w, _ = frames.shape
        if b > self.batch_max:
            self.set_batch_max(b)
        out = np.empty((b, self.num_boxes, self.num_attrs), np.float32) if want_output else None
        _lib.check(_lib.load().yds_darknet_forward_u8(self._h, _lib.ptr(frames), h, w, b, _lib.ptr(out)))
        return out

    def forward_u8_mixed(self, frames):
        from .pipeline import pack_frames
        block, off, hw = pack_frames(frames)
        if len(off) > self.batch_max:
            self.set_batch_max(len(off))
        dev = _lib.DeviceBuffer.from_array(block)
        try:
            _lib.check(_lib.load().yds_darknet_forward_u8_mixed_dev(self._h, dev.ptr, _lib.ptr(off), _lib.ptr(hw), block.nbytes, len(off)))
            _lib.check(_lib.load().yds_device_sync())
        finally:
            dev.free()

    def last_frame_dev(self, frame):
        if getattr(self, "_last_frame_src", None) is not frame:
            return None
        h, w, b = C.c_int(), C.c_int(), C.c_int()
        p = _lib.load().yds_darknet_last_frames_dev(self._h, C.byref(h), C.byref(w), C.byref(b))
        if not p or b.value != 1 or (h.value, w.value) != tuple(frame.shape[:2]):
            return None
        return C.c_void_p(p)

    def nms(self, image, conf_thres, iou_thres, frame_hw=None, cap=300):
        out = np.empty((cap, 6), np.float32)
        n = C.c_int(0)
        fh, fw = frame_hw if frame_hw is not None else (0, 0)
        _lib.check(_lib.load().yds_nms(self._h, image, conf_thres, iou_thres, fh, fw, _lib.ptr(out), cap, C.byref(n)))
        return out[:n.value].copy()

    def detect_tiled(self, frame, tiles, conf_thres, iou_thres, cap=300):
        frame = np.ascontiguousarray(frame, dtype=np.uint8)
        h, w, _ = frame.shape
        rects = np.ascontiguousarray(tiles, dtype=np.int32).reshape(-1, 4)
        out = np.empty((cap, 6), np.float32)
        n = C.c_int(0)
        _lib.check(_lib.load().yds_detect_tiled(self._h, _lib.ptr(frame), h, w, _lib.ptr(rects), rects.shape[0], conf_thres, iou_thres,
                                                _lib.ptr(out), cap, C.byref(n)))
        return out[:n.value].copy()

    def layer_shape(self, i):
        c, h, w = C.c_int(), C.c_int(), C.c_int()
        _lib.check(_lib.load().yds_darknet_layer_shape(self._h, i, C.byref(c), C.byref(h), C.byref(w)))
        return c.value, h.value, w.value

    def layer_format(self, i):
        return int(_lib.load().yds_darknet_layer_format(self._h, i))

    def layer_output(self, i, batch=1):
        c, h, w = self.layer_shape(i)
        out = np.empty((batch, c, h, w), np.float32)
        _lib.check(_lib.load().yds_darknet_layer_output(self._h, i, batch, _lib.ptr(out)))
        return out

    def get_input(self, batch=1):
        out = np.empty((batch, int(self.hyperparams["channels"]), *self.img_size), np.float32)
        _lib.check(_lib.load().yds_darknet_get_input(self._h, batch, _lib.ptr(out)))
        return out

    def set_injection(self, image, rows, logit=6.0):
        rows = np.ascontiguousarray(rows, dtype=np.float32).reshape(-1, 9)
        _lib.check(_lib.load().yds_darknet_set_injection(self._h, image, _lib.ptr(rows), rows.shape[0], logit))

    def yolo_heads(self):
        heads = []
        for i, d in enumerate(self.module_defs):
            if d["type"] == "yolo":
                _, h, w = self.layer_shape(i)
                idx = [int(v) for v in d["mask"].split(",")]
                a = [int(v) for v in d["anchors"].split(",")]
                heads.append((h, w, [(a[2 * j], a[2 * j + 1]) for j in idx]))
        return heads

    def conv_flops(self):
        return int(_lib.load().yds_darknet_conv_flops(self._h))

    def __del__(self):
        try:
            if self._h:
                _lib.load().yds_darknet_destroy(self._h)
                self._h = None
        except Exception:
            pass


def _wrap_like(x, arr):
    if hasattr(x, "detach"):
        import torch
        return torch.from_numpy(arr)
    return arr
```

Before: 1616.

## Fuse u8 frame resize into the fused stem conv input fetch

The fused stem conv kernel gains a U8 path that reads raw u8 frames and does the bilinear, area or copy resize plus normalisation inline. This replaces the separate resize kernel and its write and read of the f32 input tensor. Resize logic is split into a load phase and a value phase so the gather can be prefetched across tiles. Paths that later need the input (get_input, layer_output) materialise it lazily. The diff also adds a new yolo decode kernel and keeps the old one as a reference behind an env var.

New measurement: 1614, median of 3. No clear change (-0.2%).

```diff
diff --git a/include/ydsort.h b/include/ydsort.h
--- a/include/ydsort.h
+++ b/include/ydsort.h
@@ -53,6 +53,7 @@
 const uint8_t *yds_darknet_last_frames_dev(yds_net *, int *h, int *w, int *batch);
 int yds_darknet_layer_output(yds_net *, int layer, int batch, float *nchw_host);
 int yds_darknet_get_input(yds_net *, int batch, float *nchw_host);
+int yds_darknet_stem_resize_fused(yds_net *, int64_t *resize_launches);
 
 int yds_nms(yds_net *, int image, float conf_thres, float iou_thres, int frame_h, int frame_w,
             float *out6_host, int cap, int *n_out);
diff --git a/yolo_deepsort_amd/_lib.py b/yolo_deepsort_amd/_lib.py
--- a/yolo_deepsort_amd/_lib.py
+++ b/yolo_deepsort_amd/_lib.py
@@ -54,6 +54,7 @@
     "yds_darknet_last_frames_dev": (_P, [_P, _P, _P, _P]),
     "yds_darknet_layer_output": (_I, [_P, _I, _I, _P]),
     "yds_darknet_get_input": (_I, [_P, _I, _P]),
+    "yds_darknet_stem_resize_fused": (_I, [_P, _P]),
     "yds_darknet_set_injection": (_I, [_P, _I, _P, _I, _F]),
     "yds_darknet_load_injection_sets": (_I, [_P, _P, _P, _I, _F]),
     "yds_darknet_select_injection_set": (_I, [_P, _I]),
diff --git a/yolo_deepsort_amd/csrc/common.h b/yolo_deepsort_amd/csrc/common.h
--- a/yolo_deepsort_amd/csrc/common.h
+++ b/yolo_deepsort_amd/csrc/common.h
@@ -126,6 +126,7 @@
                    float logit, hipStream_t s);
 void launch_inject_batch(const View &head, int batch, const float *table_dev, const int *offsets_dev, int max_rows, int head_index,
                          int num_classes, float logit, hipStream_t s);
+struct StemFrames { const uint8_t *p = nullptr; int h = 0, w = 0, bgr = 0; };
 void launch_resize_u8(const uint8_t *frames, int n, int h, int w, const View &y, hipStream_t s, bool bgr = false);
 std::vector<FrameGeom> checked_layout(const uint64_t *frame_off, const int32_t *frame_hw, int n, size_t frames_bytes);
 void launch_slot_resize(const uint8_t *frames, const SlotRec *slots, int n, const View &y, hipStream_t s, bool bgr);
diff --git a/yolo_deepsort_amd/csrc/conv_common.h b/yolo_deepsort_amd/csrc/conv_common.h
--- a/yolo_deepsort_amd/csrc/conv_common.h
+++ b/yolo_deepsort_amd/csrc/conv_common.h
@@ -261,7 +261,7 @@
 
 ConvKernelArgs make_conv_args(const ConvArgs &a);
 bool conv_stem2_applicable(const ConvKernelArgs &k0, const ConvKernelArgs &k1);
-void launch_conv_stem2(const ConvKernelArgs &k0, const ConvKernelArgs &k1, hipStream_t s);
+void launch_conv_stem2(const ConvKernelArgs &k0, const ConvKernelArgs &k1, hipStream_t s, const StemFrames *frames = nullptr);
 bool conv_block1_applicable(const ConvKernelArgs &k2, const ConvKernelArgs &k3);
 void launch_conv_block1(const ConvKernelArgs &k2, const ConvKernelArgs &k3, hipStream_t s);
 
diff --git a/yolo_deepsort_amd/csrc/conv_stem2.hip b/yolo_deepsort_amd/csrc/conv_stem2.hip
--- a/yolo_deepsort_amd/csrc/conv_stem2.hip
+++ b/yolo_deepsort_amd/csrc/conv_stem2.hip
@@ -1,4 +1,5 @@
 #include "conv_common.h"
+#include "resize_dev.h"
 
 #include <algorithm>
 
@@ -31,8 +32,9 @@
     return (rc & 1) ? ODD_BASE + ry * ODD_COLS + (rc >> 1) : ry * EVEN_COLS + (rc >> 1);
 }
 
-template <int ACT0, int ACT1, bool HALF>
-__global__ __launch_bounds__(NT, 1) void conv_stem2_f16x3(ConvKernelArgs p0, ConvKernelArgs p1, int tiles_y, int tiles_x, int n_tiles) {
+template <int ACT0, int ACT1, bool HALF, bool U8>
+__global__ __launch_bounds__(NT, 1) void conv_stem2_f16x3(ConvKernelArgs p0, ConvKernelArgs p1, int tiles_y, int tiles_x, int n_tiles,
+                                                          StemFrames fr) {
     fp16_saturate_on();
     extern __shared__ __attribute__((aligned(16))) char smem[];
     char *wreg = smem, *patch = smem + W_BYTES;
@@ -61,18 +63,29 @@
     const int brow = wn * 32 + (lane & 31);
 
     constexpr int LOADS = (RR * RC + NT - 1) / NT;
-    float4 nxt[LOADS];
-    auto fetch = [&](int tl) {
+    float4 nxt[U8 ? 1 : LOADS];
+    PxSrc nsrc[U8 ? LOADS : 1];
+    int nsrc_ok = 0;
+    auto fetch = [&](int tl) __attribute__((always_inline)) {
         const int img = tl / (tiles_y * tiles_x), rem = tl - img * (tiles_y * tiles_x);
         const int iy0 = 2 * ((rem / tiles_x) * TH) - 2, ix0 = 2 * ((rem % tiles_x) * TW) - 2;
 #pragma unroll
         for (int l = 0; l < LOADS; ++l) {
             const int i = tid + l * NT, rr = i / RC, cc = i - rr * RC;
             const int iy = iy0 + rr, ix = ix0 + cc;
-            nxt[l] = make_float4(0.f, 0.f, 0.f, 0.f);
-            if (i < RR * RC && tl < n_tiles && (unsigned)iy < (unsigned)p0.H && (unsigned)ix < (unsigned)p0.W) {
-                nxt[l] = *reinterpret_cast<const float4 *>(p0.x + ((size_t)(img * p0.H + iy) * p0.W + ix) * p0.ldx);
-                nxt[l].w = 1.f;
+            const bool in = i < RR * RC && tl < n_tiles && (unsigned)iy < (unsigned)p0.H && (unsigned)ix < (unsigned)p0.W;
+            if (U8) {
+                if (l == 0) nsrc_ok = 0;
+                if (in) {
+                    resize_px_load<unsigned>(fr.p + (size_t)img * fr.h * fr.w * 3, (unsigned)fr.w * 3u, fr.h, fr.w, p0.H, p0.W, iy, ix, nsrc[l]);
+                    nsrc_ok |= 1 << l;
+                }
+            } else {
+                nxt[l] = make_float4(0.f, 0.f, 0.f, 0.f);
+                if (in) {
+                    nxt[l] = *reinterpret_cast<const float4 *>(p0.x + ((size_t)(img * p0.H + iy) * p0.W + ix) * p0.ldx);
+                    nxt[l].w = 1.f;
+                }
             }
         }
     };
@@ -82,11 +95,20 @@
         const int oy0 = (rem / tiles_x) * TH, ox0 = (rem % tiles_x) * TW;
         const int ly0 = 2 * oy0 - 1, lx0 = 2 * ox0 - 1;
         __syncthreads();
+        if (U8) __builtin_amdgcn_s_waitcnt(0x0f70);
 #pragma unroll
         for (int l = 0; l < LOADS; ++l) {
             const int i = tid + l * NT;
             if (i < RR * RC) {
-                const float v[4] = {nxt[l].x, nxt[l].y, nxt[l].z, nxt[l].w};
+                float v[4] = {0.f, 0.f, 0.f, 0.f};
+                if (!U8) {
+                    v[0] = nxt[l].x; v[1] = nxt[l].y; v[2] = nxt[l].z; v[3] = nxt[l].w;
+                } else if (nsrc_ok >> l & 1) {
+                    float o[3];
+                    resize_px_value(nsrc[l], fr.h, fr.w, p0.H, p0.W, o);
+                    if (fr.bgr) { const float t = o[0]; o[0] = o[2]; o[2] = t; }
+                    v[0] = __fdiv_rn(o[0], 255.f); v[1] = __fdiv_rn(o[1], 255.f); v[2] = __fdiv_rn(o[2], 255.f); v[3] = 1.f;
+                }
                 union { h16x4 h[2]; float4 f; } sp;
                 h16_encode4(v, sp.h[0], sp.h[1]);
                 rgb[i] = sp.f;
@@ -180,17 +202,18 @@
     }
 }
 
-template <int ACT0, int ACT1, bool HALF> void launch_inst(const ConvKernelArgs &k0, const ConvKernelArgs &k1, hipStream_t s) {
+template <int ACT0, int ACT1, bool HALF, bool U8>
+void launch_inst(const ConvKernelArgs &k0, const ConvKernelArgs &k1, const StemFrames &fr, hipStream_t s) {
     static_assert(BM * (BN + 4) * 4 <= PATCH_BYTES, "whole-tile epilogue staging must fit the layer-0 patch");
     const int n_img = k0.M / (k0.H * k0.W);
     const int tiles_y = (k1.Ho + TH - 1) / TH, tiles_x = (k1.Wo + TW - 1) / TW, n_tiles = n_img * tiles_y * tiles_x;
     static bool attr_set = false;
-    auto kern = conv_stem2_f16x3<ACT0, ACT1, HALF>;
+    auto kern = conv_stem2_f16x3<ACT0, ACT1, HALF, U8>;
     if (!attr_set) {
         YDS_HIP(hipFuncSetAttribute(reinterpret_cast<const void *>(kern), hipFuncAttributeMaxDynamicSharedMemorySize, SMEM));
         attr_set = true;
     }
-    hipLaunchKernelGGL(kern, dim3(std::min(n_tiles, 256)), dim3(NT), SMEM, s, k0, k1, tiles_y, tiles_x, n_tiles);
+    hipLaunchKernelGGL(kern, dim3(std::min(n_tiles, 256)), dim3(NT), SMEM, s, k0, k1, tiles_y, tiles_x, n_tiles, fr);
     YDS_HIP(hipGetLastError());
 }
 
@@ -202,11 +225,20 @@
            k1.H == k0.Ho && k1.W == k0.Wo && k0.act == k1.act && (k0.act == ACT_LEAKY || k0.act == ACT_MISH);
 }
 
-void launch_conv_stem2(const ConvKernelArgs &k0, const ConvKernelArgs &k1, hipStream_t s) {
+namespace {
+template <int ACT, bool HALF> void launch_src(const ConvKernelArgs &k0, const ConvKernelArgs &k1, const StemFrames *frames, hipStream_t s) {
+    if (frames) launch_inst<ACT, ACT, HALF, true>(k0, k1, *frames, s);
+    else launch_inst<ACT, ACT, HALF, false>(k0, k1, StemFrames{}, s);
+}
+}
+
+void launch_conv_stem2(const ConvKernelArgs &k0, const ConvKernelArgs &k1, hipStream_t s, const StemFrames *frames) {
     if (!conv_stem2_applicable(k0, k1)) fail("conv: the fused stem takes a 3x3/s1 RGB->32 conv followed by a 3x3/s2 32->64 conv");
+    if (frames && (!frames->p || frames->h < 1 || frames->w < 1 || frames->h > (1 << 22) || frames->w > (1 << 22) || (size_t)frames->h * frames->w * 3 >= (1ull << 32)))
+        fail("conv: the fused stem cannot take %d x %d frames", frames->h, frames->w);
     const bool half = k1.terms == 1;
-    if (k0.act == ACT_LEAKY) { if (half) launch_inst<ACT_LEAKY, ACT_LEAKY, true>(k0, k1, s); else launch_inst<ACT_LEAKY, ACT_LEAKY, false>(k0, k1, s); }
-    else { if (half) launch_inst<ACT_MISH, ACT_MISH, true>(k0, k1, s); else launch_inst<ACT_MISH, ACT_MISH, false>(k0, k1, s); }
-}
-
-}
+    if (k0.act == ACT_LEAKY) { if (half) launch_src<ACT_LEAKY, true>(k0, k1, frames, s); else launch_src<ACT_LEAKY, false>(k0, k1, frames, s); }
+    else { if (half) launch_src<ACT_MISH, true>(k0, k1, frames, s); else launch_src<ACT_MISH, false>(k0, k1, frames, s); }
+}
+
+}
diff --git a/yolo_deepsort_amd/csrc/darknet.cpp b/yolo_deepsort_amd/csrc/darknet.cpp
--- a/yolo_deepsort_amd/csrc/darknet.cpp
+++ b/yolo_deepsort_amd/csrc/darknet.cpp
@@ -504,12 +504,13 @@
     if (math != conv_math()) fail("forward: this network was planned for conv math %d, current mode is %d (re-create it)", math, conv_math());
 }
 
-void Darknet::run_graph(int batch) {
+void Darknet::run_graph(int batch, const StemFrames *src) {
     check_pass(batch);
     int lanes = getenv("YDS_DET_LANES") ? atoi(getenv("YDS_DET_LANES")) : 1;
     while (lanes > 1 && batch / lanes < 4) --lanes;
     if (lanes < 1) lanes = 1;
-    if (lanes == 1) { run_lane(0, batch, stream); return; }
+    if (lanes == 1) { run_lane(0, batch, stream, 0, -1, src); return; }
+    if (src) fail("forward: a pass that starts from frames runs in one lane");
     while ((int)lane_streams.size() < lanes - 1) {
         hipStream_t st; hipEvent_t ev;
         YDS_HIP(hipStreamCreateWithFlags(&st, hipStreamNonBlocking));
@@ -544,16 +545,34 @@
     return (int)layers.size();
 }
 
-bool Darknet::forward_resized_part(int batch, int part) {
+bool Darknet::forward_resized_part(int batch, int part, const StemFrames *src) {
     check_pass(batch);
     if (getenv("YDS_DET_LANES") && atoi(getenv("YDS_DET_LANES")) > 1) return false;
     const int cut = head_layers();
-    if (part == 0) run_lane(0, batch, stream, 0, cut);
+    if (part == 0) run_lane(0, batch, stream, 0, cut, src);
     else run_lane(0, batch, stream, cut, -1);
     return true;
 }
 
-void Darknet::enqueue_conv(const Step &st, int first, int batch, hipStream_t stream) {
+bool Darknet::stem_takes_frames(int batch) {
+    if (getenv("YDS_STEM_RESIZE_UNFUSED") || in_channels != 3) return false;
+    if (getenv("YDS_DET_LANES") && atoi(getenv("YDS_DET_LANES")) > 1) return false;
+    const LaunchPlan &p = plan(batch);
+    return !p.steps.empty() && p.steps[0].kind == Step::CONV_STEM2;
+}
+
+void Darknet::resize_into_input(const uint8_t *frames_dev, int h, int w, int batch, bool bgr) {
+    launch_resize_u8(frames_dev, batch, h, w, input_view(batch), stream, bgr);
+    ++resize_launches;
+}
+
+void Darknet::materialise_input() {
+    if (!deferred_src.p) return;
+    resize_into_input(deferred_src.p, deferred_src.h, deferred_src.w, deferred_batch, deferred_src.bgr != 0);
+    deferred_src = StemFrames{};
+}
+
+void Darknet::enqueue_conv(const Step &st, int first, int batch, hipStream_t stream, const StemFrames *src) {
     const int i = st.layer;
     const Layer &l = layers[i];
     if (!l.cw.loaded()) fail("forward: layer %d has no weights (call load_darknet_weights)", i);
@@ -566,10 +585,11 @@
         const ConvArgs a0 = conv_args(i - 1, batch, first);
         ConvKernelArgs k0 = make_conv_args(a0), k1 = make_conv_args(a);
         k1.w = reinterpret_cast<const float *>(a.w16);
-        launch_conv_stem2(k0, k1, stream);
+        launch_conv_stem2(k0, k1, stream, src);
         variant = VAR_DIRECT_RGB;
         extra_flops = conv_flops(a0);
         extra_bytes = conv_bytes(a0) - conv_bytes_io(a0.y) - conv_bytes_io(a.x);
+        if (src) extra_bytes += (double)batch * src->h * src->w * 3 - conv_bytes_io(a0.x);
     } else if (st.kind == Step::CONV_BLOCK1) {
         const ConvArgs a2 = conv_args(i - 1, batch, first);
         ConvKernelArgs k2 = make_conv_args(a2), k3 = make_conv_args(a);
@@ -593,9 +613,16 @@
     }
 }
 
-void Darknet::run_lane(int first, int batch, hipStream_t stream, int l0, int l1) {
+void Darknet::run_lane(int first, int batch, hipStream_t stream, int l0, int l1, const StemFrames *src) {
     autotune(batch);
     if (l1 < 0) l1 = (int)layers.size();
+    if (src && (first != 0 || l0 != 0 || plan(batch).steps.empty() || plan(batch).steps[0].kind != Step::CONV_STEM2))
+        fail("forward: this pass cannot start from frames (ask stem_takes_frames first)");
+    if (l0 == 0 && first == 0) {
+        stem_resize_fused_last = src != nullptr;
+        deferred_src = src ? *src : StemFrames{};
+        deferred_batch = batch;
+    }
     auto v = [&](int layer) { return view(layer, batch, first); };
     for (const Step &st : plan(batch).steps) {
         const int i = st.layer;
@@ -604,7 +631,7 @@
         const Layer &l = layers[i];
         switch (st.kind) {
         case Step::CONV: case Step::CONV_MERGED: case Step::CONV_STEM2: case Step::CONV_BLOCK1:
-            enqueue_conv(st, first, batch, stream);
+            enqueue_conv(st, first, batch, stream, st.kind == Step::CONV_STEM2 ? src : nullptr);
             break;
         case Step::MAXPOOL: launch_maxpool(v(st.src), v(i), st.ksize, st.stride, st.pad, st.zero_br, stream); break;
         case Step::UPSAMPLE: launch_upsample(v(l.src), v(i), l.stride, stream); break;
@@ -644,7 +671,12 @@
 void Darknet::forward_u8_dev(const uint8_t *frames_dev, int h, int w, int batch) {
     if (in_channels != 3) fail("forward_u8: network expects %d channels", in_channels);
     check_pass(batch);
-    launch_resize_u8(frames_dev, batch, h, w, input_view(batch), stream);
+    if (stem_takes_frames(batch)) {
+        const StemFrames src{frames_dev, h, w, 0};
+        run_graph(batch, &src);
+        return;
+    }
+    resize_into_input(frames_dev, h, w, batch, false);
     run_graph(batch);
 }
 
@@ -702,13 +734,17 @@
 void Darknet::layer_output_host(int i, int batch, float *nchw) {
     if (i < 0 || i >= (int)layers.size()) fail("layer_output: no layer %d", i);
     const Layer &l = layers[i];
-    if (l.type == L_CONV && l.cw.loaded() && plan(batch).produced_by[i] < 0) (void)launch_conv(conv_args(i, batch), stream, l.variant);
+    if (l.type == L_CONV && l.cw.loaded() && plan(batch).produced_by[i] < 0) {
+        if (l.src < 0) materialise_input();
+        (void)launch_conv(conv_args(i, batch), stream, l.variant);
+    }
     if (l.type == L_YOLO) fail("layer_output: yolo layers are read through the forward output");
     if (l.fused_res >= 0) fail("layer_output: layer %d is fused with the following shortcut", i);
     nhwc_to_host(view(i, batch), nchw, stream);
 }
 
 void Darknet::get_input_host(int batch, float *nchw) {
+    materialise_input();
     View v = input_view(batch);
     v.c = in_channels;
     nhwc_to_host(v, nchw, stream);
@@ -867,6 +903,11 @@
     YDS_API_BEGIN
     n->d->get_input_host(batch, nchw_host);
     YDS_API_END
+}
+int yds_darknet_stem_resize_fused(yds_net *n, int64_t *resize_launches) {
+    if (!n) return 0;
+    if (resize_launches) *resize_launches = n->d->resize_launches;
+    return n->d->stem_resize_fused_last ? 1 : 0;
 }
 int yds_darknet_set_injection(yds_net *n, int image, const float *rows, int cnt, float logit) {
     YDS_API_BEGIN
diff --git a/yolo_deepsort_amd/csrc/engine.h b/yolo_deepsort_amd/csrc/engine.h
--- a/yolo_deepsort_amd/csrc/engine.h
+++ b/yolo_deepsort_amd/csrc/engine.h
@@ -74,13 +74,17 @@
     void forward_u8_host(const uint8_t *frames, int h, int w, int batch, float *out_host);
     void forward_u8_dev(const uint8_t *frames_dev, int h, int w, int batch);
     void forward_u8_frames_dev(const uint8_t *frames_dev, const std::vector<FrameGeom> &geom);
-    void forward_resized(int batch) { run_graph(batch); }
-    bool forward_resized_part(int batch, int part);
+    void forward_resized(int batch, const StemFrames *src = nullptr) { run_graph(batch, src); }
+    bool stem_takes_frames(int batch);
+    bool forward_resized_part(int batch, int part, const StemFrames *src = nullptr);
     int head_layers() const;
     void forward_tiles_host(const uint8_t *frame, int h, int w, const int *tiles_xyhw, int n_tiles);
     void forward_slots(const uint8_t *frames_dev, const SlotRec *slots, int n_slots, float *pred, bool bgr);
     void layer_output_host(int layer, int batch, float *nchw);
     void get_input_host(int batch, float *nchw);
+    bool stem_resize_fused_last = false;
+    int64_t resize_launches = 0;
+    void resize_into_input(const uint8_t *frames_dev, int h, int w, int batch, bool bgr);
     void set_injection(int image, const float *rows, int n, float logit);
     void load_injection_sets(const float *rows, const int *offsets, int n_sets, float logit);
     void select_injection_set(int set);
@@ -128,9 +132,12 @@
 private:
     void allocate_buffers();
     void check_pass(int batch) const;
-    void run_graph(int batch);
-    void run_lane(int first, int batch, hipStream_t st, int l0 = 0, int l1 = -1);
-    void enqueue_conv(const Step &st, int first, int batch, hipStream_t s);
+    void run_graph(int batch, const StemFrames *src = nullptr);
+    void run_lane(int first, int batch, hipStream_t st, int l0 = 0, int l1 = -1, const StemFrames *src = nullptr);
+    void enqueue_conv(const Step &st, int first, int batch, hipStream_t s, const StemFrames *src = nullptr);
+    void materialise_input();
+    StemFrames deferred_src;
+    int deferred_batch = 0;
     const LaunchPlan &plan(int batch);
     LaunchPlan plan_;
     int plan_epoch = 0;
diff --git a/yolo_deepsort_amd/csrc/layers.hip b/yolo_deepsort_amd/csrc/layers.hip
--- a/yolo_deepsort_amd/csrc/layers.hip
+++ b/yolo_deepsort_amd/csrc/layers.hip
@@ -1,6 +1,7 @@
 #include "common.h"
 
 #include <algorithm>
+#include <stdlib.h>
 #include "h16.h"
 #include "resize_dev.h"
 
@@ -191,8 +192,57 @@
     float s0, s1;
 };
 
+template <bool SMALL>
+__device__ __forceinline__ void yolo_decode_cell(const float *src, float *dst, int lane, int per_cell, int A, int attrs, int HW, float fgx,
+                                                 float fgy, const YoloParams yp) {
+    const int row = (HW - 1) * attrs;
+    const float aw0 = yp.aw[0], aw1 = yp.aw[1], aw2 = yp.aw[2], ah0 = yp.ah[0], ah1 = yp.ah[1], ah2 = yp.ah[2], s0 = yp.s0, s1 = yp.s1;
+    for (int i = lane; i < per_cell; i += 64) {
+        int t, off;
+        float aw, ah;
+        if (SMALL) {
+            const bool a1 = i >= attrs, a2 = i >= 2 * attrs;
+            t = i - (a2 ? 2 * attrs : a1 ? attrs : 0);
+            off = i + (a2 ? 2 * row : a1 ? row : 0);
+            aw = a2 ? aw2 : a1 ? aw1 : aw0;
+            ah = a2 ? ah2 : a1 ? ah1 : ah0;
+        } else {
+            int a = 0;
+            aw = aw0; ah = ah0;
+#pragma unroll
+            for (int k = 1; k < 8; ++k)
+                if (k < A && i >= k * attrs) { a = k; aw = yp.aw[k]; ah = yp.ah[k]; }
+            t = i - a * attrs;
+            off = i + a * row;
+        }
+        const float v = src[i];
+        const bool size = (unsigned)(t - 2) < 2u;
+        const float e = expf(size || v != v ? v : -v);
+        const float s = 1.f / (1.f + e);
+        const float sc = (t & 1) ? s1 : s0;
+        const float pos = __fmul_rn(__fadd_rn(s, t == 0 ? fgx : fgy), sc);
+        const float ext = __fmul_rn(__fmul_rn(e, t == 2 ? aw : ah), sc);
+        dst[off] = t < 2 ? pos : (size ? ext : s);
+    }
+}
 __global__ void yolo_decode_kernel(const float *head, float *out, int N, int H, int W, int ld, int A, int attrs, int total_boxes,
                                    int box_off, YoloParams yp) {
+    const int HW = H * W, n = blockIdx.y, per_cell = A * attrs;
+    (void)N;
+    const int lane = threadIdx.x & 63;
+    const int wave0 = __builtin_amdgcn_readfirstlane((int)((blockIdx.x * blockDim.x + threadIdx.x) >> 6));
+    const int nwaves = (int)((gridDim.x * blockDim.x) >> 6);
+    for (int cell = wave0; cell < HW; cell += nwaves) {
+        const int gy = cell / W, gx = cell - gy * W;
+        const float *src = head + ((size_t)(n * H + gy) * W + gx) * ld;
+        float *dst = out + ((size_t)n * total_boxes + box_off + cell) * attrs;
+        if (A <= 3) yolo_decode_cell<true>(src, dst, lane, per_cell, A, attrs, HW, (float)gx, (float)gy, yp);
+        else yolo_decode_cell<false>(src, dst, lane, per_cell, A, attrs, HW, (float)gx, (float)gy, yp);
+    }
+}
+
+__global__ void yolo_decode_ref_kernel(const float *head, float *out, int N, int H, int W, int ld, int A, int attrs, int total_boxes,
+                                       int box_off, YoloParams yp) {
     const int HW = H * W, n = blockIdx.y, per_cell = A * attrs;
     (void)N;
     const int lane = threadIdx.x & 63;
@@ -234,8 +284,9 @@
     const size_t per_img = (size_t)A * head.h * head.w * attrs;
     if (per_img >= (1ull << 31)) fail("yolo: head too large for 32-bit indexing");
     const unsigned cells = (unsigned)head.h * head.w;
-    hipLaunchKernelGGL(yolo_decode_kernel, dim3(std::min((cells + 3) / 4, 2048u), head.n), dim3(256), 0, s, head.p, out, head.n, head.h, head.w,
-                       head.ld, A, attrs, total_boxes, box_off, yp);
+    const bool ref = getenv("YDS_DECODE_REF") != nullptr;
+    hipLaunchKernelGGL(ref ? yolo_decode_ref_kernel : yolo_decode_kernel, dim3(std::min((cells + 3) / 4, 2048u), head.n), dim3(256), 0, s,
+                       head.p, out, head.n, head.h, head.w, head.ld, A, attrs, total_boxes, box_off, yp);
     YDS_HIP(hipGetLastError());
 }
 
diff --git a/yolo_deepsort_amd/csrc/pipeline.cpp b/yolo_deepsort_amd/csrc/pipeline.cpp
--- a/yolo_deepsort_amd/csrc/pipeline.cpp
+++ b/yolo_deepsort_amd/csrc/pipeline.cpp
@@ -61,6 +61,7 @@
     int slot = 0;
     enum { NOTHING, HEAD, WHOLE } done = NOTHING;
     bool split = false;
+    bool front_fused = false;
     bool open() const { return frames && done != WHOLE; }
     bool is_whole(const uint8_t *f, int n, const Geometry &g, const SlotPlan &pl) const {
         return frames == f && batch == n && geo == g && plan == pl && done == WHOLE;
@@ -193,12 +194,16 @@
             YDS_HIP(hipEventRecord(s.e1, net->stream));
             return;
         }
+        p.front_fused = !p.plan.direct() && net->stem_takes_frames(p.batch);
         if (p.plan.direct()) launch_slot_resize(p.frames, s.plan_slots(), p.batch, net->input_view(p.batch), net->stream, frames_bgr);
-        else launch_resize_u8(p.frames, p.batch, p.geo.h, p.geo.w, net->input_view(p.batch), net->stream, frames_bgr);
+        else if (!p.front_fused) net->resize_into_input(p.frames, p.geo.h, p.geo.w, p.batch, frames_bgr);
         YDS_HIP(hipEventRecord(s.e1, net->stream));
-        stager.mark_read(p.frames, net->stream, FrameStager::DET);
-        p.split = split && net->forward_resized_part(p.batch, 0);
-    }
+        if (!p.front_fused) stager.mark_read(p.frames, net->stream, FrameStager::DET);
+        const StemFrames src = stem_frames(p);
+        p.split = split && net->forward_resized_part(p.batch, 0, p.front_fused ? &src : nullptr);
+        if (p.front_fused && p.split) stager.mark_read(p.frames, net->stream, FrameStager::DET);
+    }
+    StemFrames stem_frames(const Pass &p) const { return StemFrames{p.frames, p.geo.h, p.geo.w, frames_bgr ? 1 : 0}; }
     void launch_detector_tail(Pass &p) {
         DetSlot &s = det[p.slot];
         const size_t per_slot = (size_t)net->total_boxes * net->attrs, n_slots = p.plan.slots.size();
@@ -212,6 +217,10 @@
             stager.mark_read(p.frames, net->stream, FrameStager::DET);
         } else if (p.split) {
             (void)net->forward_resized_part(p.batch, 1);
+        } else if (p.front_fused) {
+            const StemFrames src = stem_frames(p);
+            net->forward_resized(p.batch, &src);
+            stager.mark_read(p.frames, net->stream, FrameStager::DET);
         } else {
             net->forward_resized(p.batch);
         }
diff --git a/yolo_deepsort_amd/csrc/resize_dev.h b/yolo_deepsort_amd/csrc/resize_dev.h
--- a/yolo_deepsort_amd/csrc/resize_dev.h
+++ b/yolo_deepsort_amd/csrc/resize_dev.h
@@ -28,28 +28,60 @@
     if (src_h == 2 * dst_h && src_w == 2 * dst_w) return RESIZE_AREA2;
     return RESIZE_LINEAR;
 }
+struct PxSrc { unsigned rg[4], b[4]; unsigned ax, ay; };
+__device__ __forceinline__ unsigned load_u16(const uint8_t *p) {
+    uint16_t v;
+    __builtin_memcpy(&v, p, 2);
+    return v;
+}
+template <typename Off>
+__device__ __forceinline__ void resize_px_load(const uint8_t *base, Off row_bytes, int src_h, int src_w, int dst_h, int dst_w, int oy, int ox,
+                                               PxSrc &s) {
+    const int mode = resize_mode(src_h, src_w, dst_h, dst_w);
+    auto row = [&](int y) -> Off { return sizeof(Off) == 4 ? (Off)__umul24((unsigned)y, (unsigned)row_bytes) : (Off)y * row_bytes; };
+    Off o0, o1, o2, o3;
+    s.ax = s.ay = 0;
+    if (mode == RESIZE_LINEAR) {
+        const Tap tx = axis_tap<true>(ox, cv_scale(dst_w, src_w), src_w), ty = axis_tap<false>(oy, cv_scale(dst_h, src_h), src_h);
+        const Off r0 = row(ty.i0), r1 = row(ty.i1);
+        o0 = r0 + (Off)(tx.i0 * 3); o1 = r0 + (Off)(tx.i1 * 3); o2 = r1 + (Off)(tx.i0 * 3); o3 = r1 + (Off)(tx.i1 * 3);
+        s.ax = (unsigned)tx.a0 | (unsigned)tx.a1 << 16;
+        s.ay = (unsigned)ty.a0 | (unsigned)ty.a1 << 16;
+    } else if (mode == RESIZE_AREA2) {
+        o0 = row(2 * oy) + (Off)(2 * ox * 3);
+        o1 = o0 + 3; o2 = o0 + row_bytes; o3 = o2 + 3;
+    } else {
+        o0 = o1 = o2 = o3 = row(oy) + (Off)(ox * 3);
+    }
+    s.rg[0] = load_u16(base + o0); s.b[0] = base[o0 + 2];
+    s.rg[1] = load_u16(base + o1); s.b[1] = base[o1 + 2];
+    s.rg[2] = load_u16(base + o2); s.b[2] = base[o2 + 2];
+    s.rg[3] = load_u16(base + o3); s.b[3] = base[o3 + 2];
+}
+__device__ __forceinline__ void resize_px_value(const PxSrc &s, int src_h, int src_w, int dst_h, int dst_w, float o[3]) {
+    const int mode = resize_mode(src_h, src_w, dst_h, dst_w);
+    const int ax0 = s.ax & 0xffffu, ax1 = s.ax >> 16, ay0 = s.ay & 0xffffu, ay1 = s.ay >> 16;
+#pragma unroll
+    for (int c = 0; c < 3; ++c) {
+        int v[4];
+#pragma unroll
+        for (int k = 0; k < 4; ++k) v[k] = (int)(c == 0 ? s.rg[k] & 0xffu : c == 1 ? s.rg[k] >> 8 : s.b[k]);
+        if (mode == RESIZE_COPY) {
+            o[c] = (float)v[0];
+        } else if (mode == RESIZE_AREA2) {
+            o[c] = (float)((v[0] + v[1] + v[2] + v[3] + 2) >> 2);
+        } else {
+            const int h0 = v[0] * ax0 + v[1] * ax1;
+            const int h1 = v[2] * ax0 + v[3] * ax1;
+            o[c] = (float)(((((ay0 * (h0 >> 4)) >> 16) + ((ay1 * (h1 >> 4)) >> 16) + 2) >> 2) & 0xff);
+        }
+    }
+}
 __device__ __forceinline__ void resize_px(const uint8_t *base, size_t row_bytes, int src_h, int src_w, int dst_h, int dst_w, int oy, int ox,
                                           float o[3]) {
-    const int mode = resize_mode(src_h, src_w, dst_h, dst_w);
-    if (mode == RESIZE_COPY) {
-        const uint8_t *p = base + (size_t)oy * row_bytes + ox * 3;
-        o[0] = p[0]; o[1] = p[1]; o[2] = p[2];
-        return;
-    }
-    if (mode == RESIZE_AREA2) {
-        const uint8_t *p = base + (size_t)(2 * oy) * row_bytes + 2 * ox * 3, *q = p + row_bytes;
-#pragma unroll
-        for (int c = 0; c < 3; ++c) o[c] = (float)(((int)p[c] + (int)p[3 + c] + (int)q[c] + (int)q[3 + c] + 2) >> 2);
-        return;
-    }
-    const Tap tx = axis_tap<true>(ox, cv_scale(dst_w, src_w), src_w), ty = axis_tap<false>(oy, cv_scale(dst_h, src_h), src_h);
-    const uint8_t *r0 = base + (size_t)ty.i0 * row_bytes, *r1 = base + (size_t)ty.i1 * row_bytes;
-#pragma unroll
-    for (int c = 0; c < 3; ++c) {
-        const int h0 = (int)r0[tx.i0 * 3 + c] * tx.a0 + (int)r0[tx.i1 * 3 + c] * tx.a1;
-        const int h1 = (int)r1[tx.i0 * 3 + c] * tx.a0 + (int)r1[tx.i1 * 3 + c] * tx.a1;
-        o[c] = (float)(((((ty.a0 * (h0 >> 4)) >> 16) + ((ty.a1 * (h1 >> 4)) >> 16) + 2) >> 2) & 0xff);
-    }
+    PxSrc s;
+    resize_px_load<size_t>(base, row_bytes, src_h, src_w, dst_h, dst_w, oy, ox, s);
+    resize_px_value(s, src_h, src_w, dst_h, dst_w, o);
 }
 
 }
diff --git a/yolo_deepsort_amd/models.py b/yolo_deepsort_amd/models.py
--- a/yolo_deepsort_amd/models.py
+++ b/yolo_deepsort_amd/models.py
@@ -192,6 +192,11 @@
         _lib.check(_lib.load().yds_darknet_get_input(self._h, batch, _lib.ptr(out)))
         return out
 
+    def front_end(self):
+        n = C.c_int64(0)
+        fused = _lib.load().yds_darknet_stem_resize_fused(self._h, C.byref(n))
+        return bool(fused), int(n.value)
+
     def set_injection(self, image, rows, logit=6.0):
         rows = np.ascontiguousarray(rows, dtype=np.float32).reshape(-1, 9)
         _lib.check(_lib.load().yds_darknet_set_injection(self._h, image, _lib.ptr(rows), rows.shape[0], logit))
```
